# lucagem29/mcmc_clv_model

Measured on AMD Instinct MI355X. Metric: MCMC sweeps/sec x N_customers (customer-sweeps/s), higher is better.
Workload: dtype f64

## Files before the change

### include/clvmcmc.h

```cpp
#ifndef CLVMCMC_H
#define CLVMCMC_H

#include <stdint.h>

#ifdef __cplusplus
extern "C" {
#endif

#define CLV_ABI_VERSION 2

#define CLV_BLOCK 256
#define CLV_MAX_K 9
#define CLV_MAX_D 3

enum { CLV_OK = 0, CLV_EINVAL = -1, CLV_EHIP = -2, CLV_ESTATE = -3, CLV_ENOMEM = -4 };
enum { CLV_RNG_PHILOX = 0, CLV_RNG_REPLAY = 1 };
enum { CLV_SINK_FULL = 0, CLV_SINK_SUMMARY = 1, CLV_SINK_NONE = 2, CLV_SINK_SUMMARY_PCT = 3 };

#define CLV_SUMMARY_MU_CAP 0.05
enum {
  CLV_SUM_LAMBDA = 0, CLV_SUM_MU, CLV_SUM_Z, CLV_SUM_LOG_LAMBDA, CLV_SUM_LOG_MU,
  CLV_SUM_LAMBDA2, CLV_SUM_MU2, CLV_SUM_ETA, CLV_SUM_LOG_ETA, CLV_SUM_MU_CAPPED, CLV_SUM_TAU,
  CLV_N_SUM_STATS
};

typedef struct clv_config {
  int32_t abi_version;
  int32_t D;
  int32_t K;
  int32_t n_mh_steps;
  int32_t burnin, mcmc, thin;
  int32_t n_chains;
  int32_t chain_first;
  int32_t rng_mode;
  int32_t draw_sink;
  int32_t device;
  uint64_t seed;
  int64_t n_global;
  int64_t shard_begin;
  int32_t world_size;
  int32_t rank;
  int32_t blocks_per_rank;
  int32_t blocks_per_unit;
  uint64_t stream;
} clv_config;

typedef struct clv_data {
  int64_t n;
  const int32_t* x;
  const double* t_x;
  const double* T_cal;
  const double* covariates;
  const double* log_s;
} clv_data;

typedef struct clv_prior {
  double lam_init;
  double V[CLV_MAX_K * CLV_MAX_K];
  double chol_V[CLV_MAX_K * CLV_MAX_K];
  double A0B0[CLV_MAX_K * CLV_MAX_D];
  double S0_B0A0B0[CLV_MAX_D * CLV_MAX_D];
  double nu_n;
  double beta_init[CLV_MAX_K * CLV_MAX_D];
  double sigma_init[CLV_MAX_D * CLV_MAX_D];
  double omega2;
} clv_prior;

typedef struct clv_sampler clv_sampler;

int32_t clv_abi_version(void);
int32_t clv_default_blocks_per_unit(int64_t n_global);
int64_t clv_sizeof(int32_t which);
const char* clv_last_error(void);
int clv_device_count(int32_t* count);

int clv_create(const clv_config* cfg, const clv_data* data, const clv_prior* prior,
               clv_sampler** out);
void clv_destroy(clv_sampler* s);

int clv_set_replay_tape(clv_sampler* s, const double* tape, int64_t n_sweeps);
int64_t clv_replay_sweep_stride(const clv_sampler* s);

int clv_run(clv_sampler* s, int64_t n_sweeps);
int clv_rollback(clv_sampler* s);

int clv_sweep(clv_sampler* s);
int clv_hyper(clv_sampler* s, const double* gathered_device_ptr);
int clv_partials(clv_sampler* s, double** device_ptr, int64_t* n_doubles, int32_t* stride);
int clv_copy_partials(clv_sampler* s, void* dst_device_ptr);
int clv_synchronize(clv_sampler* s);
int64_t clv_sweeps_done(const clv_sampler* s);

int clv_clock_ghz(clv_sampler* s, double* ghz);
int clv_clock_probe(clv_sampler* s, double us, double* ghz);
int clv_launch_info(const clv_sampler* s, int64_t* out);
#define CLV_IPC_HANDLE_BYTES 64
int clv_p2p_info(const clv_sampler* s, int64_t* out);
int clv_p2p_export(clv_sampler* s, void* handle);
int clv_p2p_connect(clv_sampler* s, const void* handles, const uint64_t* ptrs);
int clv_p2p_disconnect(clv_sampler* s);
int clv_p2p_set_persistent(clv_sampler* s, int32_t on);
int clv_set_wait_timeout(clv_sampler* s, double ms);
int clv_set_stream(clv_sampler* s, uint64_t stream);
int clv_note_sweeps(clv_sampler* s, int64_t n);

int clv_read_draws(clv_sampler* s, double* level1, double* level2, double* loglik);
int clv_stream_draws(clv_sampler* s, double* level1);
int clv_read_summary(clv_sampler* s, double* sums, int64_t* n_stored);

int clv_get_state(clv_sampler* s, double* lambdas, double* mus, double* hyper);
int clv_set_state(clv_sampler* s, const double* lambdas, const double* mus, const double* hyper,
                  int64_t sweeps_done);

int clv_set_timing(clv_sampler* s, int32_t enable);
int clv_kernel_time(clv_sampler* s, double* sweep_kernel_ms_total, int64_t* sweep_launches,
                    double* hyper_kernel_ms_total, int64_t* hyper_launches);

int clv_debug_host_times(const clv_sampler* s, int64_t* out);
int clv_debug_philox(uint32_t k0, uint32_t k1, const uint32_t* ctr, int64_t n, uint32_t* out);
int clv_debug_variates(uint64_t seed, int32_t chain, uint32_t sweep, int64_t n, int32_t n_steps,
                       float* t_l, float* t_m, float* u_acc, double* u_z, double* u_tau,
                       double* e_alive, double* eta_z, float* log2_u_acc);
int clv_debug_log2u_scan(uint64_t w_begin, uint64_t w_end, double* out);
int clv_debug_t3(const uint32_t* words, int64_t n, int32_t packed, float* t_l, float* t_m);
int clv_debug_level2(int32_t D, int32_t K, const clv_prior* prior, const double* xty,
                     const double* yty, const double* iw_normal, const double* iw_chi2,
                     const double* z, double* beta, double* sigma);
int clv_debug_stamps(clv_sampler* s, uint64_t* out);
int clv_debug_wg_stamps(clv_sampler* s, uint64_t* out);
int clv_debug_hyper_variates(uint64_t seed, int32_t chain, uint32_t sweep, double df, int64_t n,
                             double* chi2, double* normals);
int clv_debug_exp(const double* x, int64_t n, double* out);
int clv_debug_log(const double* x, int64_t n, double* out);
int clv_debug_mh_step(int64_t n, const int32_t* x, const uint8_t* z, const double* T_cal, const double* tau,
                      const double* mean, const double* prec3, const double* cur_pt, const float* t3,
                      const double* scale2, const float* log_u, double* out);
int clv_debug_wg_map(int32_t n_chains, int32_t nb, int32_t n_cu, int32_t* out);
int clv_debug_persist_fits(int64_t grid_wgs, int32_t blocks_per_cu, int32_t n_cu);
int clv_debug_persist_choice(int32_t D, int32_t K, int32_t n_chains, int64_t grid_wgs, int32_t blocks_per_cu,
                             int32_t n_cu);

enum { CLV_EXCHANGE_AUTO = 0, CLV_EXCHANGE_P2P = 1, CLV_EXCHANGE_COPY = 2 };
typedef struct clv_group clv_group;
int clv_group_create(clv_sampler* const* shards, int32_t n, int32_t exchange, clv_group** out);
int clv_group_run(clv_group* g, int64_t n_sweeps);
int32_t clv_group_exchange(const clv_group* g);
void clv_group_destroy(clv_group* g);

enum {
  CLV_L1_MEAN_LAMBDA = 0, CLV_L1_LAMBDA_P025, CLV_L1_LAMBDA_P975, CLV_L1_MEAN_MU, CLV_L1_MEAN_MU_CAPPED,
  CLV_L1_MU_P025, CLV_L1_MU_P975, CLV_L1_MEAN_Z, CLV_L1_MEAN_TAU, CLV_L1_MEAN_ETA, CLV_N_L1_STATS
};
int clv_predict(int32_t device, const double* level1, int64_t n_draws, int64_t n, int32_t width,
                const double* T_cal, double T_star, uint64_t seed, int32_t simulate_spend, double sigma_s,
                int64_t* x_future, double* spend_future);
int clv_predict_sampler(clv_sampler* s, double T_star, uint64_t seed, int32_t simulate_spend,
                        double sigma_s, int64_t* x_future, double* spend_future);
int clv_track(int32_t device, const double* level1, int64_t n_draws, int64_t n, int32_t width,
              const double* birth_week, const double* times, int32_t n_times, uint64_t seed,
              double* inc_weekly);
int clv_track_sampler(clv_sampler* s, const double* birth_week, const double* times, int32_t n_times,
                      uint64_t seed, double* inc_weekly);
int clv_level1_summary(int32_t device, const double* level1, int64_t n_draws, int64_t n, int32_t width,
                       double mu_cap, double* out);
int clv_level1_summary_sampler(clv_sampler* s, double mu_cap, double* out);
int clv_chain_total_loglik(int32_t device, const double* level1, int64_t n_draws, int64_t n, int32_t width,
                           const int32_t* x, const double* T_cal, double* mean_total);
int clv_chain_total_loglik_sampler(clv_sampler* s, double* mean_total);

enum {
  CLV_LTV_VALUE_MEAN = 0, CLV_LTV_VALUE_SD, CLV_LTV_VALUE_P025, CLV_LTV_VALUE_P50, CLV_LTV_VALUE_P975,
  CLV_LTV_RESIDUAL_MEAN, CLV_LTV_RESIDUAL_SD, CLV_LTV_RESIDUAL_P025, CLV_LTV_RESIDUAL_P50, CLV_LTV_RESIDUAL_P975,
  CLV_LTV_P_ALIVE, CLV_LTV_LIFETIME_YRS, CLV_LTV_SURVIVAL_1YR, CLV_N_LTV_STATS
};
enum {
  CLV_LTV_DRAW_EQUITY = 0, CLV_LTV_DRAW_VALUE_TOTAL, CLV_LTV_DRAW_N_ALIVE, CLV_LTV_DRAW_MU_SHARE,
  CLV_N_LTV_DRAW_STATS
};
int clv_lifetime_value(int32_t device, const double* level1, int64_t n_draws, int64_t n, int32_t width,
                       const double* monetary , double delta, double horizon ,
                       double value_scale, double periods_per_year, double* out_customers, double* out_draws);
int clv_lifetime_value_sampler(clv_sampler* s, const double* monetary, double delta, double horizon,
                               double value_scale, double periods_per_year, double* out_customers,
                               double* out_draws);
int clv_ltv_info(int64_t* out);

enum {
  CLV_DIAG_MEAN = 0, CLV_DIAG_SD, CLV_DIAG_MCSE, CLV_DIAG_ESS, CLV_DIAG_RHAT, CLV_DIAG_LAG, CLV_N_DIAG_STATS
};
int clv_diagnostics(int32_t device, const double* series, int32_t n_chains, int64_t n_draws, int64_t n_series,
                    int32_t period, uint32_t log_mask, double* out);
int clv_diagnostics_sampler(clv_sampler* s, uint32_t log_mask, double* level1_out, double* level2_out);
int clv_autocorr(int32_t device, const double* series, int32_t n_chains, int64_t n_draws, int64_t n_series,
                 int32_t max_lag, double* out);

#define CLV_RANK_LDS_ELEMS 4080
enum {
  CLV_RANK_RHAT = 0, CLV_RANK_RHAT_BULK, CLV_RANK_RHAT_FOLDED, CLV_RANK_ESS_BULK, CLV_RANK_ESS_TAIL,
  CLV_RANK_ESS_Q05, CLV_RANK_ESS_Q95, CLV_RANK_ESS_SD, CLV_RANK_MCSE_SD, CLV_RANK_HDI_LO, CLV_RANK_HDI_HI,
  CLV_RANK_MEDIAN, CLV_RANK_LAG_BULK, CLV_N_RANK_STATS
};
int clv_rank_diagnostics(int32_t device, const double* series, int32_t n_chains, int64_t n_draws, int64_t n_series,
                         int32_t period, uint32_t log_mask, double hdi_prob, double* out);
int clv_rank_diagnostics_sampler(clv_sampler* s, uint32_t log_mask, double hdi_prob, double* level1_out,
                                 double* level2_out);
int clv_debug_zscale(int32_t device, const double* series, int32_t n_chains, int64_t n_draws, int64_t n_series,
                     int32_t folded, double* ranks_out, double* z_out);

int clv_elog2cbs(int32_t device, int64_t n_events, const int64_t* cust, const int64_t* date_ns, const double* sales,
                 int64_t unit_ns, int64_t T_cal_ns, int64_t T_tot_ns, int64_t* n_customers, int64_t* cust_out,
                 int64_t* x, double* t_x, double* litt, double* sales_out, double* sales_x, int64_t* first_ns,
                 double* T_cal, double* T_star, int64_t* x_star, double* sales_star);
int clv_generate_pareto_abe(int32_t device, int64_t n, int32_t K, const double* beta, const double* gamma,
                            const double* covars, const double* T_cal, int32_t n_star, const double* T_star,
                            uint64_t seed, int64_t* x, double* t_x, double* lambda_true, double* mu_true,
                            double* tau_true, uint8_t* alive_true, int64_t* x_star, double* covars_out,
                            int64_t* n_events, const int64_t* elog_offsets, int64_t elog_rows, int64_t* elog_cust,
                            double* elog_t);

typedef struct clv_pnbd clv_pnbd;
int clv_pnbd_create(int32_t device, int64_t n, const int32_t* x, const double* t_x, const double* T,
                    const double* weights, clv_pnbd** out);
void clv_pnbd_destroy(clv_pnbd* h);
int clv_pnbd_eval(clv_pnbd* h, const double* params, double* sums, int64_t* n_unconverged);
int clv_pnbd_customers(clv_pnbd* h, const double* params, double t_star, double* out);
int clv_pnbd_track(int32_t device, int64_t n, const double* birth_week, const double* times, int32_t n_times,
                   const double* params, double* cum);

#ifdef __cplusplus
}
#endif
#endif
```

### mcmc_clv_model_amd/csrc/capi.hip

```cpp
#include <hip/hip_runtime.h>

#include <algorithm>
#include <chrono>
#include <cstdlib>
#include <cstdio>
#include <cstring>
#include <string>
#include <vector>

#include "internal.h"
#include "kernels.h"
#include "philox.h"

using namespace clv;

namespace {

thread_local std::string g_err;

constexpr int PRIOR_DOUBLES = 81 + 81 + 27 + 9;
constexpr int GRAPH_CHUNK = 64;
constexpr int TIMING_EVENTS = 256;

}
// ... 135 lines not shown
    s->ev.resize(4 * TIMING_EVENTS);
    for (auto& e : s->ev) CLV_HIP(hipEventCreate(&e));
  }
  return CLV_OK;
}

int build_graph(clv_sampler* s, int n) {
  if (s->graph_exec && s->graph_sweeps == n) return CLV_OK;
  if (s->graph_exec) {
    CLV_HIP(hipGraphExecDestroy(s->graph_exec));
    s->graph_exec = nullptr;
  }
  hipGraph_t graph;
  CLV_HIP(hipStreamBeginCapture(s->stream, hipStreamCaptureModeThreadLocal));
  for (int k = 0; k < n; ++k) {
    int rc = enqueue_fused(s, nullptr, nullptr);
    if (rc != CLV_OK) {
      hipGraph_t dummy;
      (void)hipStreamEndCapture(s->stream, &dummy);
      return rc;
    }
  }
  CLV_HIP(hipStreamEndCapture(s->stream, &graph));
  CLV_HIP(hipGraphInstantiate(&s->graph_exec, graph, nullptr, nullptr, 0));
  CLV_HIP(hipGraphDestroy(graph));
  s->graph_sweeps = n;
  return CLV_OK;
}

bool is_pow2(int v) { return v > 0 && (v & (v - 1)) == 0; }

int64_t stored_count(const clv_sampler* s, int64_t sweeps) {
  const Geometry& g = s->g;
  if (sweeps <= g.burnin || g.n_draws <= 0) return 0;
  return std::min<int64_t>((sweeps - 1 - g.burnin) / g.thin + 1, g.n_draws);
}

void stream_enqueue(clv_sampler* s) {
  if (!s->ds_dest || !s->d_level1) return;
  const Geometry& g = s->g;
  const int64_t k = stored_count(s, s->sweeps_done);
  if (k <= s->ds_next) return;
  const int64_t row = g.n * (g.D + 2);
  for (int c = 0; c < g.n_chains; ++c) {
    const int64_t off = ((int64_t)c * g.n_draws + s->ds_next) * row;
    stream_copy(s->ds, s->device, s->d_level1 + off, s->ds_dest + off, sizeof(double) * (size_t)((k - s->ds_next) * row));
  }
  s->ds_next = k;
}

void stream_rewind(clv_sampler* s) {
  if (!s->ds_dest) return;
  stream_wait(s->ds);
  s->ds_next = std::min(s->ds_next, stored_count(s, s->sweeps_done));
}

std::string take_wait_diag(clv_sampler* s) {
  if (!s->d_diag) return "";
  unsigned long long d[DIAG_WORDS] = {};
  if (hipMemcpy(d, s->d_diag, sizeof(d), hipMemcpyDeviceToHost) != hipSuccess) return "";
  (void)hipMemset(s->d_diag, 0, sizeof(d));
  if (!d[0]) return "";
  const Geometry& g = s->g;
  const char* what = d[1] == WAIT_HYPER ? "(beta, Sigma) hand-off slot"
                     : d[1] == WAIT_BLOCKS ? "block partial"
                     : d[1] == WAIT_P2P_MAIL ? "peer unit partial (persistent)" : "peer unit partial (fused)";
  std::string m = std::string(" [wait record: sweep ") + std::to_string((long long)d[2]) + ", chain " +
                  std::to_string(d[3]) + ", rank " + std::to_string(d[4]) + ": " + what + " ";
  const long long unit = (long long)d[5];
  if ((d[1] == WAIT_P2P_MAIL || d[1] == WAIT_FX_MAIL) && g.units_per_rank > 0 && unit >= 0)
    m += "unit " + std::to_string(unit) + " (rank " + std::to_string(unit / g.units_per_rank) + ", local unit " +
         std::to_string(unit % g.units_per_rank) + ")";
  else
    m += (d[1] == WAIT_HYPER ? "of block " : "") + std::to_string(unit);
  char bits[32];
  std::snprintf(bits, sizeof(bits), "%016llx", d[7]);
  m += " statistic " + std::to_string((long long)d[6]) + " still empty (bits " + bits + ") after " +
       std::to_string(d[8]) + " polls, " + std::to_string(d[9] / 100000.0) + " ms; " + std::to_string(d[10]) +
       " lanes of the wave missing";
  if (d[1] == WAIT_P2P_MAIL || d[1] == WAIT_FX_MAIL) {
    m += "; progress (sweep each rank's level-2 side last polled for):";
    for (int q = 0; q < std::min(g.world_size, 5); ++q)
      m += " " + std::to_string(q) + ":" + (d[11 + q] == ~0ull ? std::string("none") : std::to_string((long long)d[11 + q]));
  }
  return m + "]";
}

bool parse_wait_ms(const char* txt, double* ms) {
  for (const char* c = txt; *c; ++c)
    if (*c == 'x' || *c == 'X' || *c == 'n' || *c == 'N' || *c == 'i' || *c == 'I') return false;
  char* end = nullptr;
  const double v = std::strtod(txt, &end);
  if (end == txt) return false;
  while (*end == ' ' || *end == '\t' || *end == '\n') ++end;
  if (*end || !(v == v) || v > 1e300 || v < -1e300) return false;
  *ms = std::min(3.6e6, std::max(1.0, v));
  return true;
}

}

extern "C" {

int32_t clv_abi_version(void) { return CLV_ABI_VERSION; }

int32_t clv_default_blocks_per_unit(int64_t n_global) {
  const int64_t nb = (n_global + BLOCK - 1) / BLOCK;
  int32_t g = 1;
  while ((nb + g - 1) / g > 512) g *= 2;
  return g;
}

const char* clv_last_error(void) { return g_err.c_str(); }

int64_t clv_sizeof(int32_t which) {
  switch (which) {
    case 0: return (int64_t)sizeof(clv_config);
    case 1: return (int64_t)sizeof(clv_data);
    case 2: return (int64_t)sizeof(clv_prior);
    default: return -1;
  }
}

int clv_device_count(int32_t* count) {
  int n = 0;
  CLV_HIP(hipGetDeviceCount(&n));
  *count = n;
  return CLV_OK;
}

int64_t clv_replay_sweep_stride(const clv_sampler* s) {
  const int64_t n = s->g.n;
  return n * (2 + 3 * (int64_t)s->g.S + (s->g.D == 3 ? 1 : 0)) + TAPE_HYPER;
}

}

bool clv::persist_grid_fits(int64_t grid_wgs, int blocks_per_cu, int n_cu) {
  constexpr int SGPR_MAX = 102;
  const int sgpr_term = 800 / (((SGPR_MAX + 15) / 16) * 16 + 16);
  const int64_t per_cu = std::min({blocks_per_cu, 8, sgpr_term});
  const int64_t slots = per_cu * n_cu;
  const int64_t margin = std::max(1, n_cu / 32);
  return grid_wgs > 0 && slots > 0 && grid_wgs <= slots - margin;
}

constexpr size_t PERSIST_SCRATCH_MAX = 64;

bool clv::persist_worth(int D, int K, int n_chains, int64_t grid_wgs, int n_cu) {
  (void)D, (void)K, (void)n_chains;
  return n_cu > 0 && grid_wgs > 0;
}

namespace {

#ifndef CLV_L2_ALONE_MIN_NB
#define CLV_L2_ALONE_MIN_NB 256
#endif
std::vector<int32_t> persist_wg_map(int C, int nb, int n_cu) {
  const int per = nb + 1;
  const int T = C * per;
  std::vector<int32_t> map(T);
  for (int c = 0; c < C; ++c)
    for (int b = 0; b < per; ++b) map[c * per + b] = (c << 16) | b;
  const int P = T - n_cu;
  if (P <= 0 || T > 2 * n_cu) return map;
  std::vector<std::vector<int>> todo(C);
  for (int c = 0; c < C; ++c)
    for (int b = nb - 1; b >= 0; --b) todo[c].push_back(b);
  std::vector<int32_t> first, second, single;
  int p = 0;
  const bool l2_alone = nb >= CLV_L2_ALONE_MIN_NB;
  for (int c = 0; !l2_alone && c < C && p < P; ++c, ++p) {
    first.push_back((c << 16) | nb);
    if (todo[c].empty()) return map;
    second.push_back((c << 16) | todo[c].back());
    todo[c].pop_back();
  }
  const int n_l2_paired = (int)first.size();
  const bool l2_paired = n_l2_paired == C;
  for (int c = 0; p < P; c = (c + 1) % C) {
    bool any = false;
    for (int k = 0; k < C && !any; ++k) any = todo[(c + k) % C].size() >= 2;
    if (!any) return map;
    if (todo[c].size() < 2) continue;
    first.push_back((c << 16) | todo[c].back());
    todo[c].pop_back();
    second.push_back((c << 16) | todo[c].back());
    todo[c].pop_back();
    ++p;
  }
  for (int c = 0; c < C; ++c) {
    if (!l2_paired && c >= n_l2_paired) single.push_back((c << 16) | nb);
    while (!todo[c].empty()) {
      single.push_back((c << 16) | todo[c].back());
      todo[c].pop_back();
    }
  }
  std::vector<int32_t> sorted_single;
  for (size_t k = 0; sorted_single.size() < single.size(); ++k)
    for (int c = 0; c < C; ++c) {
      size_t seen = 0;
      for (int32_t v : single)
        if ((v >> 16) == c && seen++ == k) sorted_single.push_back(v);
    }
  if ((int)first.size() != P || (int)sorted_single.size() != n_cu - P) return map;
  for (int i = 0; i < P; ++i) {
    map[i] = first[i];
    map[n_cu + i] = second[i];
  }
  for (int i = 0; i < n_cu - P; ++i) map[P + i] = sorted_single[i];
  return map;
}

}

extern "C" {

int clv_create(const clv_config* cfg, const clv_data* data, const clv_prior* prior, clv_sampler** out) {
  if (!cfg || !data || !prior || !out) return fail(CLV_EINVAL, "null argument");
  *out = nullptr;
  if (cfg->abi_version != CLV_ABI_VERSION) return fail(CLV_EINVAL, "ABI version mismatch");
  if (cfg->D != 2 && cfg->D != 3) return fail(CLV_EINVAL, "D must be 2 or 3");
  if (cfg->K < 1 || cfg->K > CLV_MAX_K) return fail(CLV_EINVAL, "K must be in 1..9");
  if (cfg->n_mh_steps < 0) return fail(CLV_EINVAL, "n_mh_steps must be >= 0");
  if (cfg->thin < 1) return fail(CLV_EINVAL, "thin must be >= 1");
  if (cfg->burnin < 0 || cfg->mcmc < 0) return fail(CLV_EINVAL, "burnin/mcmc must be >= 0");
  if (cfg->n_chains < 1) return fail(CLV_EINVAL, "n_chains must be >= 1");
  if (cfg->rng_mode != CLV_RNG_PHILOX && cfg->rng_mode != CLV_RNG_REPLAY) return fail(CLV_EINVAL, "bad rng_mode");
  if (cfg->draw_sink < CLV_SINK_FULL || cfg->draw_sink > CLV_SINK_SUMMARY_PCT) return fail(CLV_EINVAL, "bad draw_sink");
  if (data->n < 0) return fail(CLV_EINVAL, "n must be >= 0");
  if (cfg->n_global > 0xffffffffLL) return fail(CLV_EINVAL, "n_global must fit the 32-bit Philox customer counter");
  if (cfg->n_global < data->n || cfg->n_global < 1) return fail(CLV_EINVAL, "n_global must be >= n >= 0 and > 0");
  if (cfg->world_size < 1 || cfg->rank < 0 || cfg->rank >= cfg->world_size) return fail(CLV_EINVAL, "bad rank/world_size");
  if (cfg->D == 3 && data->n > 0 && !data->log_s) return fail(CLV_EINVAL, "D == 3 needs log_s");
  if (cfg->K > 1 && data->n > 0 && !data->covariates) return fail(CLV_EINVAL, "K > 1 needs covariates");
  if (data->n > 0 && (!data->x || !data->t_x || !data->T_cal)) return fail(CLV_EINVAL, "missing CBS column");
  if (cfg->rng_mode == CLV_RNG_REPLAY && cfg->world_size != 1) return fail(CLV_EINVAL, "replay needs world_size 1");

  const int32_t bpu = cfg->blocks_per_unit ? cfg->blocks_per_unit : clv_default_blocks_per_unit(cfg->n_global);
  if (!is_pow2(bpu)) return fail(CLV_EINVAL, "blocks_per_unit must be a power of two");
  const int nb_local = (int)((data->n + BLOCK - 1) / BLOCK);
  int32_t bpr = cfg->blocks_per_rank;
  if (bpr == 0) {
    if (cfg->world_size != 1) return fail(CLV_EINVAL, "blocks_per_rank required when sharded");
    bpr = ((std::max(nb_local, 1) + bpu - 1) / bpu) * bpu;
  }
  if (bpr % bpu) return fail(CLV_EINVAL, "blocks_per_rank must be a multiple of blocks_per_unit");
  if (nb_local > bpr) return fail(CLV_EINVAL, "shard larger than blocks_per_rank * CLV_BLOCK");
  if (cfg->shard_begin != (int64_t)cfg->rank * bpr * BLOCK) return fail(CLV_EINVAL, "shard_begin != rank * blocks_per_rank * CLV_BLOCK");
  const int64_t nb_global = (cfg->n_global + BLOCK - 1) / BLOCK;
  if ((int64_t)bpr * cfg->world_size < nb_global) return fail(CLV_EINVAL, "shards do not cover n_global");

  auto* s = new clv_sampler();
  s->cfg = *cfg;
  s->cfg.blocks_per_rank = bpr;
  s->cfg.blocks_per_unit = bpu;
  s->prior = *prior;
  s->replay = cfg->rng_mode == CLV_RNG_REPLAY;

  Geometry& g = s->g;
  g.D = cfg->D;
  g.K = cfg->K;
  g.S = cfg->n_mh_steps;
  g.n_chains = cfg->n_chains;
  g.n = data->n;
  g.n_global = cfg->n_global;
  g.shard_begin = cfg->shard_begin;
  g.nb_local = nb_local;
  g.blocks_per_rank = bpr;
  g.blocks_per_unit = bpu;
  g.units_per_rank = bpr / bpu;
  g.n_units_global = (nb_global + bpu - 1) / bpu;
  g.world_size = cfg->world_size;
  g.stride = cfg->K * cfg->D + cfg->D * (cfg->D + 1) / 2 + 1;
  g.burnin = cfg->burnin;
  g.mcmc = cfg->mcmc;
  g.thin = cfg->thin;
  g.n_draws = cfg->mcmc >= 1 ? (cfg->mcmc - 1) / cfg->thin + 1 : 0;
  g.l2w = cfg->D * cfg->K + cfg->D * (cfg->D + 1) / 2;

  auto cleanup_fail = [&](int rc) {
    clv_destroy(s);
    return rc;
  };
#define CLV_HIPC(expr)                                                                            \
  do {                                                                                            \
    hipError_t e_ = (expr);                                                                       \
    if (e_ != hipSuccess)                                                                         \
      return cleanup_fail(fail(CLV_EHIP, std::string(#expr) + ": " + hipGetErrorString(e_)));    \
  } while (0)

  if (cfg->device >= 0) CLV_HIPC(hipSetDevice(cfg->device));
  CLV_HIPC(hipGetDevice(&s->device));
  if (cfg->stream) {
    s->stream = (hipStream_t)(uintptr_t)cfg->stream;
  } else {
    CLV_HIPC(hipStreamCreateWithFlags(&s->stream, hipStreamNonBlocking));
    s->own = s->stream;
    s->own_stream = true;
  }

  const int64_t n = g.n, C = g.n_chains;
  CLV_HIPC(dalloc(&s->d_x, std::max<int64_t>(n, 1)));
  CLV_HIPC(dalloc(&s->d_tx, std::max<int64_t>(n, 1)));
  CLV_HIPC(dalloc(&s->d_T, std::max<int64_t>(n, 1)));
  if (g.K > 1) CLV_HIPC(dalloc(&s->d_cov, (size_t)(g.K - 1) * std::max<int64_t>(n, 1)));
  if (g.D == 3) CLV_HIPC(dalloc(&s->d_logs, std::max<int64_t>(n, 1)));
  CLV_HIPC(dalloc(&s->d_clk, 2 * CLK_RING));
  CLV_HIPC(hipMemsetAsync(s->d_clk, 0, sizeof(unsigned long long) * 2 * CLK_RING, s->stream));
  CLV_HIPC(dalloc(&s->d_lam, C * std::max<int64_t>(n, 1)));
  CLV_HIPC(dalloc(&s->d_mu, C * std::max<int64_t>(n, 1)));
  CLV_HIPC(dalloc(&s->d_hyper, C * HS));
  CLV_HIPC(dalloc(&s->d_block, (size_t)C * bpr * g.stride));
  if (bpu > 1) CLV_HIPC(dalloc(&s->d_unit, (size_t)C * g.units_per_rank * g.stride));
  else s->d_unit = s->d_block;
  CLV_HIPC(dalloc(&s->d_prior, PRIOR_DOUBLES));
  CLV_HIPC(dalloc(&s->d_ctrl, 1));
  CLV_HIPC(dalloc(&s->d_arrive, C + C * (int64_t)g.units_per_rank));
  CLV_HIPC(dalloc(&s->d_hvar, 2 * C * HV));
  CLV_HIPC(dalloc(&s->d_hyp2, 2 * C * HS));
  if (!s->replay && cfg->world_size == 1 && nb_local > 0 && bpu == 1 && nb_local <= 2 * BLOCK) {
    const char* env = std::getenv("CLV_PERSISTENT");
    hipDeviceProp_t prop{};
    size_t scratch = SIZE_MAX;
    if (persist_occupancy(g.D, g.K, false, &s->persist_bpc) == hipSuccess &&
        persist_scratch_bytes(g.D, g.K, false, &scratch) == hipSuccess &&
        hipGetDeviceProperties(&prop, s->device) == hipSuccess)
      s->n_cu = prop.multiProcessorCount;
    const int64_t grid = (int64_t)(nb_local + 1) * C;
    const bool force = env && std::string(env) == "1";
    if ((!env || std::string(env) != "0") && (force || scratch <= PERSIST_SCRATCH_MAX) && persist_grid_fits(grid, s->persist_bpc, s->n_cu) &&
        (force || persist_worth(g.D, g.K, (int)C, grid, s->n_cu)))
      s->persistent = true;
  }
  if (!s->replay && cfg->world_size > 1 && cfg->world_size <= MAX_WORLD && nb_local > 0 && nb_local <= 2 * BLOCK && g.n_units_global <= 2 * BLOCK &&
      bpu <= 64 && (int64_t)g.stride * ((nb_local + bpu - 1) / bpu) <= UMAIL) {
    hipDeviceProp_t prop{};
    size_t scratch = SIZE_MAX;
    if (persist_occupancy(g.D, g.K, true, &s->persist_bpc) == hipSuccess &&
        persist_scratch_bytes(g.D, g.K, true, &scratch) == hipSuccess &&
        hipGetDeviceProperties(&prop, s->device) == hipSuccess)
      s->n_cu = prop.multiProcessorCount;
    const char* env = std::getenv("CLV_PERSISTENT");
    const int64_t grid = (int64_t)(nb_local + 1) * C;
    const bool force = env && std::string(env) == "1";
    if ((!env || std::string(env) != "0") && (force || scratch <= PERSIST_SCRATCH_MAX) && persist_grid_fits(grid, s->persist_bpc, s->n_cu) &&
        (force || persist_worth(g.D, g.K, (int)C, grid, s->n_cu)))
      s->p2p_capable = s->p2p_persist_fits = true;
  }
  if (!s->replay && cfg->world_size > 1 && cfg->world_size <= MAX_WORLD && g.n_units_global <= 2 * BLOCK)
    s->fx_capable = true;
  if (s->p2p_capable || s->fx_capable) {
    const int64_t nm = mail_slots(g.world_size, (int)C, g.stride, g.units_per_rank) + MAIL_TAIL;
    {
      const char* env = std::getenv("CLV_MAIL_ALLOC");
      const std::string want = env ? env : "uncached";
      const unsigned flags[3] = {hipDeviceMallocUncached, hipDeviceMallocFinegrained, hipDeviceMallocDefault};
      const int first = want == "fine" ? 1 : want == "default" ? 2 : 0;
      for (int k = first; k < 3 && !s->d_mail; ++k) {
        void* p = nullptr;
        if (hipExtMallocWithFlags(&p, sizeof(double) * (size_t)nm, flags[k]) == hipSuccess && p) {
          s->d_mail = (double*)p;
          s->mail_kind = k;
        } else {
          (void)hipGetLastError();
        }
      }
      if (!s->d_mail) return cleanup_fail(fail(CLV_ENOMEM, "peer mail buffer"));
    }
    CLV_HIPC(hipMemsetAsync(s->d_mail, 0xFF, sizeof(double) * nm, s->stream));
    CLV_HIPC(dalloc(&s->d_peers, g.world_size));
  }
  if (s->persistent || s->p2p_capable || s->fx_capable) {
    CLV_HIPC(dalloc(&s->d_pblock, (size_t)C * std::max(nb_local, 1) * g.stride));
    if (s->persistent) {
      const char* env = std::getenv("CLV_DEFER");
      s->defer = !(env && std::string(env) == "0");
      if (s->defer) CLV_HIPC(dalloc(&s->d_pend, (size_t)2 * C * g.stride));
    }
    CLV_HIPC(dalloc(&s->d_lam_alt, C * std::max<int64_t>(n, 1)));
    CLV_HIPC(dalloc(&s->d_mu_alt, C * std::max<int64_t>(n, 1)));
    CLV_HIPC(dalloc(&s->d_hyper_alt, C * HS));
    if ((cfg->draw_sink == CLV_SINK_SUMMARY || cfg->draw_sink == CLV_SINK_SUMMARY_PCT) && n > 0)
      CLV_HIPC(dalloc(&s->d_sums_prev, (size_t)C * CLV_N_SUM_STATS * n));
    CLV_HIPC(dalloc(&s->d_diag, DIAG_WORDS));
    CLV_HIPC(hipMemsetAsync(s->d_diag, 0, sizeof(unsigned long long) * DIAG_WORDS, s->stream));
    CLV_HIPC(hipHostMalloc((void**)&s->h_abort, sizeof(uint32_t), hipHostMallocMapped));
    *s->h_abort = 0;
    CLV_HIPC(hipHostGetDevicePointer((void**)&s->d_h_abort, s->h_abort, 0));
    double ms = cfg->world_size > 1 ? 10000.0 : 2000.0;
    if (const char* env = std::getenv("CLV_WAIT_TIMEOUT_MS")) {
      if (!parse_wait_ms(env, &ms))
        return cleanup_fail(fail(CLV_EINVAL, "CLV_WAIT_TIMEOUT_MS must be a finite decimal number of ms"));
    }
    s->wait_ticks = (uint64_t)(ms * 1e5);
  }
  if ((s->persistent || s->p2p_capable) && s->n_cu > 0) {
    {
      std::vector<int32_t> map = persist_wg_map((int)C, (int)nb_local, s->n_cu);
      CLV_HIPC(dalloc(&s->d_wgmap, map.size()));
      CLV_HIPC(hipMemcpy(s->d_wgmap, map.data(), sizeof(int32_t) * map.size(), hipMemcpyHostToDevice));
    }
  }
#ifdef CLV_STAMPS
  {
    std::vector<unsigned long long> st(1024 * 8 + 12 * (size_t)C * (std::max(nb_local, 1) + 1), 0ull);
    for (int i = 0; i < 1024; ++i) st[i * 8 + 0] = st[i * 8 + 4] = ~0ull;
    CLV_HIPC(dalloc(&s->d_stamps, st.size()));
    CLV_HIPC(hipMemcpy(s->d_stamps, st.data(), st.size() * sizeof(unsigned long long), hipMemcpyHostToDevice));
  }
#endif
  CLV_HIPC(hipMemsetAsync(s->d_hvar, 0, sizeof(double) * 2 * C * HV, s->stream));
  CLV_HIPC(hipMemsetAsync(s->d_arrive, 0, sizeof(uint32_t) * (C + C * (int64_t)g.units_per_rank), s->stream));
  CLV_HIPC(dalloc(&s->d_bs, C * (CLV_MAX_K * CLV_MAX_D + CLV_MAX_D * CLV_MAX_D)));
  if (g.n_draws > 0) {
    CLV_HIPC(dalloc(&s->d_level2, (size_t)C * g.n_draws * g.l2w));
    CLV_HIPC(dalloc(&s->d_loglik, (size_t)C * g.n_draws));
    CLV_HIPC(hipMemsetAsync(s->d_level2, 0, sizeof(double) * C * g.n_draws * g.l2w, s->stream));
    CLV_HIPC(hipMemsetAsync(s->d_loglik, 0, sizeof(double) * C * g.n_draws, s->stream));
    if (cfg->draw_sink == CLV_SINK_FULL && n > 0) {
      const size_t bytes = sizeof(double) * (size_t)C * g.n_draws * n * (g.D + 2);
      CLV_HIPC(dalloc(&s->d_level1, bytes / sizeof(double)));
      CLV_HIPC(hipMemsetAsync(s->d_level1, 0, bytes, s->stream));
    }
  }
  if ((cfg->draw_sink == CLV_SINK_SUMMARY || cfg->draw_sink == CLV_SINK_SUMMARY_PCT) && n > 0) {
    CLV_HIPC(dalloc(&s->d_sums, (size_t)C * CLV_N_SUM_STATS * n));
    CLV_HIPC(hipMemsetAsync(s->d_sums, 0, sizeof(double) * C * CLV_N_SUM_STATS * n, s->stream));
  }
  if (cfg->draw_sink == CLV_SINK_SUMMARY_PCT && n > 0 && g.n_draws > 0) {
    const size_t nq = (size_t)C * g.n_draws * n;
    if (hipMalloc((void**)&s->d_qstore, sizeof(float2) * nq) != hipSuccess) {
      (void)hipGetLastError();
      s->d_qstore = nullptr;
      return cleanup_fail(fail(CLV_ENOMEM, "percentile store: " + std::to_string(sizeof(float2) * nq) +
                                               " bytes of device memory not available"));
    }
    CLV_HIPC(hipMemsetAsync(s->d_qstore, 0, sizeof(float2) * nq, s->stream));
  }
  CLV_HIPC(hipMemsetAsync(s->d_block, 0, sizeof(double) * C * bpr * g.stride, s->stream));
  if (bpu > 1) CLV_HIPC(hipMemsetAsync(s->d_unit, 0, sizeof(double) * C * g.units_per_rank * g.stride, s->stream));
  CLV_HIPC(hipMemsetAsync(s->d_ctrl, 0, sizeof(Ctrl), s->stream));
  CLV_HIPC(hipMemsetAsync(s->d_hyper, 0, sizeof(double) * C * HS, s->stream));

  if (n > 0) {
    CLV_HIPC(hipMemcpyAsync(s->d_x, data->x, sizeof(int32_t) * n, hipMemcpyHostToDevice, s->stream));
    CLV_HIPC(hipMemcpyAsync(s->d_tx, data->t_x, sizeof(double) * n, hipMemcpyHostToDevice, s->stream));
    CLV_HIPC(hipMemcpyAsync(s->d_T, data->T_cal, sizeof(double) * n, hipMemcpyHostToDevice, s->stream));
    if (g.K > 1)
      CLV_HIPC(hipMemcpyAsync(s->d_cov, data->covariates, sizeof(double) * (g.K - 1) * n, hipMemcpyHostToDevice, s->stream));
    if (g.D == 3)
      CLV_HIPC(hipMemcpyAsync(s->d_logs, data->log_s, sizeof(double) * n, hipMemcpyHostToDevice, s->stream));
  }
  {
    std::vector<double> pr(PRIOR_DOUBLES, 0.0);
    const int K = g.K, D = g.D;
    for (int i = 0; i < K * K; ++i) {
      pr[i] = prior->V[i];
      pr[81 + i] = prior->chol_V[i];
    }
    for (int i = 0; i < K * D; ++i) pr[162 + i] = prior->A0B0[i];
    for (int i = 0; i < D * D; ++i) pr[189 + i] = prior->S0_B0A0B0[i];
    CLV_HIPC(hipMemcpyAsync(s->d_prior, pr.data(), sizeof(double) * PRIOR_DOUBLES, hipMemcpyHostToDevice, s->stream));
    CLV_HIPC(hipStreamSynchronize(s->stream));
  }

  if (n > 0) CLV_HIPC(launch_sweep(sweep_args(s, 1), false, s->stream));
  else CLV_HIPC(hipMemsetAsync(s->d_block, 0, sizeof(double) * C * bpr * g.stride, s->stream));
  if (bpu > 1) {
    GroupArgs ga{};
    ga.g = g;
    ga.blockpart = s->d_block;
    ga.unitpart = s->d_unit;
    if (n > 0) CLV_HIPC(launch_group(ga, s->stream));
  }
  if (g.D == 3) {
    std::vector<double> bs(C * (g.K * g.D + g.D * g.D));
    for (int c = 0; c < C; ++c) {
      double* o = bs.data() + c * (g.K * g.D + g.D * g.D);
      for (int i = 0; i < g.K * g.D; ++i) o[i] = prior->beta_init[i];
      for (int i = 0; i < g.D * g.D; ++i) o[g.K * g.D + i] = prior->sigma_init[i];
    }
    CLV_HIPC(hipMemcpyAsync(s->d_bs, bs.data(), sizeof(double) * bs.size(), hipMemcpyHostToDevice, s->stream));
    CLV_HIPC(launch_set_hyper(g.D, g.K, (int)C, s->d_hyper, s->d_bs, prior->omega2, s->replay, s->stream));
  } else {
    s->pending_init_hyper = true;
  }
  CLV_HIPC(hipStreamSynchronize(s->stream));
#undef CLV_HIPC
  *out = s;
  return CLV_OK;
}

void clv_destroy(clv_sampler* s) {
  if (!s) return;
  (void)hipSetDevice(s->device);
  if (s->stream) (void)hipStreamSynchronize(s->stream);
  if (s->ds) {
    stream_wait(s->ds);
    delete s->ds;
  }
  if (s->graph_exec) (void)hipGraphExecDestroy(s->graph_exec);
  for (auto e : s->ev) (void)hipEventDestroy(e);
  if (s->done_ev) (void)hipEventDestroy(s->done_ev);
  void* ptrs[] = {s->d_x, s->d_tx, s->d_T, s->d_cov, s->d_logs, s->d_lam, s->d_mu, s->d_hyper,
                  s->d_block, s->d_prior, s->d_ctrl, s->d_level1, s->d_level2, s->d_loglik,
                  s->d_sums, s->d_tape, s->d_bs, s->d_arrive, s->d_hvar, s->d_stamps};
  for (void* p : ptrs)
    if (p) (void)hipFree(p);
  if (s->d_unit && s->d_unit != s->d_block) (void)hipFree(s->d_unit);
  if (s->d_hyp2) (void)hipFree(s->d_hyp2);
  for (void* p : {(void*)s->d_lam_alt, (void*)s->d_mu_alt, (void*)s->d_hyper_alt, (void*)s->d_sums_prev,
                  (void*)s->d_pblock, (void*)s->d_qstore, (void*)s->d_pend, (void*)s->d_diag,
                  (void*)s->d_clk})
    if (p) (void)hipFree(p);
  if (s->h_abort) (void)hipHostFree(s->h_abort);
  for (void* p : s->ipc_opened) (void)hipIpcCloseMemHandle(p);
  if (s->d_mail) (void)hipFree(s->d_mail);
  if (s->d_peers) (void)hipFree(s->d_peers);
  if (s->d_wgmap) (void)hipFree(s->d_wgmap);
  if (s->own_stream && s->own) (void)hipStreamDestroy(s->own);
  delete s;
}

int clv_set_replay_tape(clv_sampler* s, const double* tape, int64_t n_sweeps) {
  if (!s || !tape || n_sweeps < 1) return fail(CLV_EINVAL, "bad replay tape arguments");
  if (!s->replay) return fail(CLV_ESTATE, "sampler not created in replay mode");
  CLV_HIP(hipSetDevice(s->device));
  if (s->d_tape) CLV_HIP(hipFree(s->d_tape));
  s->d_tape = nullptr;
  const size_t count = (size_t)s->g.n_chains * n_sweeps * clv_replay_sweep_stride(s);
  CLV_HIP(dalloc(&s->d_tape, count));
  CLV_HIP(hipMemcpy(s->d_tape, tape, count * sizeof(double), hipMemcpyHostToDevice));
  s->tape_sweeps = n_sweeps;
  if (s->graph_exec) {
    CLV_HIP(hipGraphExecDestroy(s->graph_exec));
    s->graph_exec = nullptr;
  }
  return CLV_OK;
}

int clv_hyper(clv_sampler* s, const double* gathered) {
  if (!s) return fail(CLV_EINVAL, "null sampler");
  if (s->g.world_size > 1 && !gathered) return fail(CLV_EINVAL, "sharded hyper needs the gathered buffer");
  CLV_HIP(hipSetDevice(s->device));
  {
    int rc = persist_flush(s);
    if (rc) return rc;
  }
  if (s->pending_init_hyper) {
    int rc = check_replay_range(s, 0);
    if (rc) return rc;
    rc = enqueue_hyper(s, gathered, 1, nullptr, nullptr);
    if (rc) return rc;
    s->pending_init_hyper = false;
    return CLV_OK;
  }
  return enqueue_hyper(s, gathered, 0, nullptr, nullptr);
}

int clv_sweep(clv_sampler* s) {
  if (!s) return fail(CLV_EINVAL, "null sampler");
  if (s->pending_init_hyper) return fail(CLV_ESTATE, "bivariate: call clv_hyper once before the first sweep");
  CLV_HIP(hipSetDevice(s->device));
  int rc = persist_flush(s);
  if (rc) return rc;
  rc = check_replay_range(s, 1);
  if (rc) return rc;
  hipEvent_t e0 = nullptr, e1 = nullptr;
  if (s->timing) {
    rc = ensure_events(s);
    if (rc) return rc;
    e0 = s->ev[4 * s->ev_used];
    e1 = s->ev[4 * s->ev_used + 1];
  }
  rc = enqueue_sweep(s, e0, e1);
  if (rc) return rc;
  if (s->timing && ++s->ev_used == TIMING_EVENTS) {
    rc = harvest_timing(s);
    if (rc) return rc;
  }
  s->sweeps_done++;
  return CLV_OK;
}

int clv_partials(clv_sampler* s, double** ptr, int64_t* n_doubles, int32_t* stride) {
  if (!s) return fail(CLV_EINVAL, "null sampler");
  if (ptr) *ptr = s->d_unit;
  if (n_doubles) *n_doubles = (int64_t)s->g.n_chains * s->g.units_per_rank * s->g.stride;
  if (stride) *stride = s->g.stride;
  return CLV_OK;
}

int clv_copy_partials(clv_sampler* s, void* dst) {
  if (!s || !dst) return fail(CLV_EINVAL, "null argument");
  CLV_HIP(hipSetDevice(s->device));
  const size_t bytes = sizeof(double) * (size_t)s->g.n_chains * s->g.units_per_rank * s->g.stride;
  CLV_HIP(hipMemcpyAsync(dst, s->d_unit, bytes, hipMemcpyDeviceToDevice, s->stream));
  return CLV_OK;
}

int clv_synchronize(clv_sampler* s) {
  if (!s) return fail(CLV_EINVAL, "null sampler");
  CLV_HIP(hipSetDevice(s->device));
  CLV_HIP(hipStreamSynchronize(s->stream));
  return CLV_OK;
}

int64_t clv_sweeps_done(const clv_sampler* s) { return s ? s->sweeps_done : -1; }

int clv_clock_ghz(clv_sampler* s, double* ghz) {
  if (!s || !ghz) return fail(CLV_EINVAL, "null argument");
  *ghz = 0.0;
  const int64_t end = s->sweeps_done - 1;
  const int64_t first = std::max<int64_t>(s->clk_first, end - (CLK_RING - 1));
  if (!s->d_clk || s->clk_first < 1 || end < first) return CLV_OK;
  CLV_HIP(hipSetDevice(s->device));
  CLV_HIP(hipStreamSynchronize(s->stream));
  std::vector<unsigned long long> ring(2 * CLK_RING);
  CLV_HIP(hipMemcpy(ring.data(), s->d_clk, sizeof(unsigned long long) * ring.size(), hipMemcpyDeviceToHost));
  double dm = 0.0, dr = 0.0;
  for (int64_t q = first; q <= end; ++q) {
    dm += (double)ring[2 * (q % CLK_RING)];
    dr += (double)ring[2 * (q % CLK_RING) + 1];
  }
  if (dr > 0.0) *ghz = 0.1 * dm / dr;
  return CLV_OK;
}

int clv_launch_info(const clv_sampler* s, int64_t* out) {
  if (!s || !out) return fail(CLV_EINVAL, "null argument");
  out[0] = s->persistent ? 1 : 0;
  out[1] = s->persist_bpc;
  out[2] = s->n_cu;
  out[3] = (int64_t)(s->g.nb_local + (s->persistent ? 1 : 0)) * s->g.n_chains;
  out[4] = 0;
  out[5] = 0;
  return CLV_OK;
}

int clv_p2p_info(const clv_sampler* s, int64_t* out) {
  if (!s || !out) return fail(CLV_EINVAL, "null argument");
  out[0] = (s->p2p_capable || s->fx_capable) ? 1 : 0;
  out[4] = s->p2p_capable ? 1 : 0;
  out[1] = s->p2p_ready ? 1 : 0;
  out[2] = s->d_mail ? (int64_t)sizeof(double) * 2 * s->g.world_size * s->g.n_chains * s->g.stride * s->g.units_per_rank : 0;
  out[3] = (int64_t)(uintptr_t)s->d_mail;
  out[5] = s->d_mail ? s->mail_kind : -1;
  return CLV_OK;
}

int clv_p2p_export(clv_sampler* s, void* handle) {
  if (!s || !handle) return fail(CLV_EINVAL, "null argument");
  if (!s->p2p_capable && !s->fx_capable) return fail(CLV_ESTATE, "no peer exchange for this sampler (world size 1 or replay mode)");
  CLV_HIP(hipSetDevice(s->device));
  hipIpcMemHandle_t h;
  CLV_HIP(hipIpcGetMemHandle(&h, s->d_mail));
  std::memcpy(handle, &h, sizeof(h));
  return CLV_OK;
}

int clv_p2p_connect(clv_sampler* s, const void* handles, const uint64_t* ptrs) {
  if (!s || (!handles && !ptrs)) return fail(CLV_EINVAL, "null argument");
  if (!s->p2p_capable && !s->fx_capable) return fail(CLV_ESTATE, "no peer exchange for this sampler (world size 1 or replay mode)");
  CLV_HIP(hipSetDevice(s->device));
  CLV_HIP(hipStreamSynchronize(s->stream));
  if (s->p2p_ready || !s->ipc_opened.empty()) {
    s->p2p_ready = false;
    for (void* p : s->ipc_opened) (void)hipIpcCloseMemHandle(p);
    s->ipc_opened.clear();
  }
  {
    const int64_t nm = mail_slots(s->g.world_size, s->g.n_chains, s->g.stride, s->g.units_per_rank) + MAIL_TAIL;
    CLV_HIP(hipMemsetAsync(s->d_mail, 0xFF, sizeof(double) * nm, s->stream));
  }
  const int W = s->g.world_size, r = s->cfg.rank;
  std::vector<double*> peers(W, nullptr);
  for (int q = 0; q < W; ++q) {
    if (q == r) {
      peers[q] = s->d_mail;
    } else if (handles) {
      hipIpcMemHandle_t h;
      std::memcpy(&h, (const char*)handles + (size_t)q * sizeof(h), sizeof(h));
      void* p = nullptr;
      CLV_HIP(hipIpcOpenMemHandle(&p, h, hipIpcMemLazyEnablePeerAccess));
      s->ipc_opened.push_back(p);
      peers[q] = (double*)p;
    } else {
      peers[q] = (double*)(uintptr_t)ptrs[q];
    }
    if (!peers[q]) return fail(CLV_EINVAL, "null peer mail pointer");
  }
  CLV_HIP(hipMemcpy(s->d_peers, peers.data(), sizeof(double*) * W, hipMemcpyHostToDevice));
  CLV_HIP(hipStreamSynchronize(s->stream));
  s->p2p_ready = true;
  return CLV_OK;
}

int clv_p2p_set_persistent(clv_sampler* s, int32_t on) {
  if (!s) return fail(CLV_EINVAL, "null sampler");
  if (on && !s->p2p_persist_fits) return fail(CLV_ESTATE, "the persistent peer exchange does not fit this shard's grid");
  if (!on && !s->fx_capable) return fail(CLV_ESTATE, "no fused peer exchange for this sampler");
  CLV_HIP(hipSetDevice(s->device));
  CLV_HIP(hipStreamSynchronize(s->stream));
  s->p2p_capable = on != 0;
  s->last_persist_n = 0;
  return CLV_OK;
}

int clv_p2p_disconnect(clv_sampler* s) {
  if (!s) return fail(CLV_EINVAL, "null sampler");
  CLV_HIP(hipSetDevice(s->device));
  CLV_HIP(hipStreamSynchronize(s->stream));
  s->p2p_ready = false;
  for (void* p : s->ipc_opened) (void)hipIpcCloseMemHandle(p);
  s->ipc_opened.clear();
  if (s->d_peers) CLV_HIP(hipMemset(s->d_peers, 0, sizeof(double*) * s->g.world_size));
  return CLV_OK;
}

int clv_set_wait_timeout(clv_sampler* s, double ms) {
  if (!s || !(ms >= 1.0) || ms > 3.6e6) return fail(CLV_EINVAL, "wait timeout must be in [1 ms, 1 h]");
  s->wait_ticks = (uint64_t)(ms * 1e5);
  if (s->graph_exec) {
    CLV_HIP(hipGraphExecDestroy(s->graph_exec));
    s->graph_exec = nullptr;
  }
  return CLV_OK;
}

int clv_set_stream(clv_sampler* s, uint64_t stream) {
  if (!s || !stream) return fail(CLV_EINVAL, "bad arguments");
  if (s->graph_exec) {
    CLV_HIP(hipGraphExecDestroy(s->graph_exec));
    s->graph_exec = nullptr;
  }
  s->stream = (hipStream_t)(uintptr_t)stream;
  return CLV_OK;
}

int clv_note_sweeps(clv_sampler* s, int64_t n) {
  if (!s || s->sweeps_done + n < 0) return fail(CLV_EINVAL, "bad arguments");
  s->sweeps_done += n;
  s->last_persist_n = 0;
  return CLV_OK;
}

}

static inline int64_t host_now_ns() {
  return std::chrono::duration_cast<std::chrono::nanoseconds>(std::chrono::steady_clock::now().time_since_epoch())
      .count();
}

int clv::persist_launch(clv_sampler* s, int64_t n_sweeps) {
  const Geometry& g = s->g;
  s->last_persist_n = 0;
  s->inflight_n = 0;
  if (n_sweeps == 0) return CLV_OK;
  if (s->slots_dirty) {
    CLV_HIP(hipMemsetAsync(s->d_hyp2, 0xFF, sizeof(double) * 2 * g.n_chains * HS, s->stream));
    CLV_HIP(hipMemsetAsync(s->d_pblock, 0xFF, sizeof(double) * g.n_chains * g.nb_local * g.stride, s->stream));
    s->slots_dirty = false;
  }
  const size_t sums_bytes = sizeof(double) * (size_t)g.n_chains * CLV_N_SUM_STATS * g.n;
  if (s->d_sums_prev)
    CLV_HIP(hipMemcpyAsync(s->d_sums_prev, s->d_sums, sums_bytes, hipMemcpyDeviceToDevice, s->stream));
  SweepArgs a = sweep_args(s, 0, 1);
  const int64_t stride_c = (int64_t)g.n_chains * g.stride;
  a.pend_in = s->pend ? s->d_pend + s->pend_buf * stride_c : nullptr;
  a.pend_out = s->defer ? s->d_pend + (s->pend_buf ^ 1) * stride_c : nullptr;
  hipEvent_t e0 = nullptr, e1 = nullptr;
  if (s->timing) {
    int rc = ensure_events(s);
    if (rc) return rc;
    e0 = s->ev[4 * s->ev_used];
    e1 = s->ev[4 * s->ev_used + 1];
    if (s->ev_sweeps.size() < TIMING_EVENTS) s->ev_sweeps.assign(TIMING_EVENTS, 1);
    s->ev_sweeps[s->ev_used] = n_sweeps;
  }
  if (e0) CLV_HIP(hipEventRecord(e0, s->stream));
  s->host_ns[2] = host_now_ns();
  CLV_HIP(launch_persist(a, s->sweeps_done + 1, n_sweeps, s->stream, nullptr, nullptr));
  s->host_ns[3] = host_now_ns();
  if (e1) CLV_HIP(hipEventRecord(e1, s->stream));
  s->inflight_done = e1;
  if (s->timing) {
    if (++s->ev_used == TIMING_EVENTS) {
      int rc = harvest_timing(s);
      if (rc) return rc;
    }
  } else {
    if (!s->done_ev) CLV_HIP(hipEventCreateWithFlags(&s->done_ev, hipEventDisableTiming));
    CLV_HIP(hipEventRecord(s->done_ev, s->stream));
    s->inflight_done = s->done_ev;
  }
  s->inflight_n = n_sweeps;
  s->host_ns[4] = host_now_ns();
  return CLV_OK;
}

int clv::persist_wait(clv_sampler* s) {
  const int64_t n_sweeps = s->inflight_n;
  if (n_sweeps == 0) return CLV_OK;
  s->inflight_n = 0;
  const Geometry& g = s->g;
  const hipEvent_t done = s->inflight_done;
  if (!done) {
    CLV_HIP(hipStreamSynchronize(s->stream));
  } else {
    hipError_t q;
    while ((q = hipEventQuery(done)) == hipErrorNotReady) {
    }
    CLV_HIP(q);
  }
  s->host_ns[5] = host_now_ns();
  if (__atomic_load_n(s->h_abort, __ATOMIC_ACQUIRE)) {
    *s->h_abort = 0;
    Ctrl c{};
    c.cur = s->sweeps_done;
    CLV_HIP(hipMemcpy(s->d_ctrl, &c, sizeof(Ctrl), hipMemcpyHostToDevice));
    const size_t sums_bytes = sizeof(double) * (size_t)g.n_chains * CLV_N_SUM_STATS * g.n;
    if (s->d_sums_prev) CLV_HIP(hipMemcpy(s->d_sums, s->d_sums_prev, sums_bytes, hipMemcpyDeviceToDevice));
    s->slots_dirty = true;
    if (g.world_size > 1) s->p2p_ready = false;
    const std::string diag = take_wait_diag(s);
    return fail(CLV_EHIP, std::string(g.world_size > 1
                                          ? "persistent sweep kernel: a wait timed out (a peer rank not running, or not all "
                                            "resident?); state unchanged"
                                          : "persistent sweep kernel: a workgroup timed out waiting for its chain (not all "
                                            "resident?); state unchanged") + diag);
  }
  std::swap(s->d_lam, s->d_lam_alt);
  std::swap(s->d_mu, s->d_mu_alt);
  s->rb_pend = s->pend;
  s->rb_pend_buf = s->pend_buf;
  s->rb_hyper_swaps = 0;
  if (s->defer) {
    s->pend = true;
    s->pend_buf ^= 1;
  } else {
    std::swap(s->d_hyper, s->d_hyper_alt);
    s->rb_hyper_swaps = 1;
    s->pend = false;
  }
  if (s->graph_exec) {
    CLV_HIP(hipGraphExecDestroy(s->graph_exec));
    s->graph_exec = nullptr;
  }
  s->sweeps_done += n_sweeps;
  s->last_persist_n = n_sweeps;
  return CLV_OK;
}

int clv::persist_flush(clv_sampler* s) {
  if (!s->pend) return CLV_OK;
  CLV_HIP(hipSetDevice(s->device));
  SweepArgs a = sweep_args(s, 0, 1);
  a.pend_in = s->d_pend + s->pend_buf * (int64_t)s->g.n_chains * s->g.stride;
  a.pend_out = nullptr;
  CLV_HIP(launch_persist_flush(a, s->sweeps_done + 1, s->stream));
  CLV_HIP(hipStreamSynchronize(s->stream));
  std::swap(s->d_hyper, s->d_hyper_alt);
  s->rb_hyper_swaps++;
  s->pend = false;
  if (s->graph_exec) {
    CLV_HIP(hipGraphExecDestroy(s->graph_exec));
    s->graph_exec = nullptr;
  }
  return CLV_OK;
}

namespace {
int run_persistent(clv_sampler* s, int64_t n_sweeps) {
  int rc = persist_launch(s, n_sweeps);
  if (rc) return rc;
  return persist_wait(s);
}

int enqueue_fused_sweeps(clv_sampler* s, int64_t n_sweeps) {
  int rc = CLV_OK;
  int64_t left = n_sweeps;
  if (s->timing) {
    rc = ensure_events(s);
    if (rc) return rc;
    while (left > 0) {
      const int k = s->ev_used;
      rc = enqueue_fused(s, s->ev[4 * k], s->ev[4 * k + 1]);
      if (rc) return rc;
      s->ev_used++;
      s->sweeps_done++;
      left--;
      if (s->ev_used == TIMING_EVENTS) {
        rc = harvest_timing(s);
        if (rc) return rc;
      }
    }
    return harvest_timing(s);
  }
  if (left >= GRAPH_CHUNK) {
    rc = build_graph(s, GRAPH_CHUNK);
    if (rc) return rc;
    while (left >= GRAPH_CHUNK) {
      CLV_HIP(hipGraphLaunch(s->graph_exec, s->stream));
      s->sweeps_done += GRAPH_CHUNK;
      left -= GRAPH_CHUNK;
    }
  }
  while (left > 0) {
    rc = enqueue_fused(s, nullptr, nullptr);
    if (rc) return rc;
    s->sweeps_done++;
    left--;
  }
  return CLV_OK;
}

int run_fused_exchange(clv_sampler* s, int64_t n_sweeps) {
  s->last_persist_n = 0;
  if (n_sweeps == 0) return CLV_OK;
  const Geometry& g = s->g;
  const size_t nl = sizeof(double) * (size_t)g.n_chains * std::max<int64_t>(g.n, 1);
  const size_t sums_bytes = sizeof(double) * (size_t)g.n_chains * CLV_N_SUM_STATS * g.n;
  CLV_HIP(hipMemcpyAsync(s->d_lam_alt, s->d_lam, nl, hipMemcpyDeviceToDevice, s->stream));
  CLV_HIP(hipMemcpyAsync(s->d_mu_alt, s->d_mu, nl, hipMemcpyDeviceToDevice, s->stream));
  CLV_HIP(hipMemcpyAsync(s->d_hyper_alt, s->d_hyper, sizeof(double) * g.n_chains * HS, hipMemcpyDeviceToDevice,
                         s->stream));
  if (s->d_sums_prev) CLV_HIP(hipMemcpyAsync(s->d_sums_prev, s->d_sums, sums_bytes, hipMemcpyDeviceToDevice, s->stream));
  const int64_t before = s->sweeps_done;
  const int rc = enqueue_fused_sweeps(s, n_sweeps);
  CLV_HIP(hipStreamSynchronize(s->stream));
  const bool aborted = __atomic_load_n(s->h_abort, __ATOMIC_ACQUIRE) != 0;
  if (rc == CLV_OK && !aborted) {
    s->last_persist_n = n_sweeps;
    s->rb_pend = false;
    s->rb_hyper_swaps = 1;
    return CLV_OK;
  }
  CLV_HIP(hipMemcpy(s->d_lam, s->d_lam_alt, nl, hipMemcpyDeviceToDevice));
  CLV_HIP(hipMemcpy(s->d_mu, s->d_mu_alt, nl, hipMemcpyDeviceToDevice));
  CLV_HIP(hipMemcpy(s->d_hyper, s->d_hyper_alt, sizeof(double) * g.n_chains * HS, hipMemcpyDeviceToDevice));
  if (s->d_sums_prev) CLV_HIP(hipMemcpy(s->d_sums, s->d_sums_prev, sums_bytes, hipMemcpyDeviceToDevice));
  *s->h_abort = 0;
  s->sweeps_done = before;
  Ctrl c{};
  c.cur = before;
  CLV_HIP(hipMemcpy(s->d_ctrl, &c, sizeof(Ctrl), hipMemcpyHostToDevice));
  CLV_HIP(hipMemset(s->d_arrive, 0, sizeof(uint32_t) * (g.n_chains + (int64_t)g.n_chains * g.units_per_rank)));
  s->p2p_ready = false;
  if (rc) return rc;
  return fail(CLV_EHIP, "fused peer exchange: a wait timed out (a peer rank not running?); state unchanged" +
                            take_wait_diag(s));
}

int run_streaming(clv_sampler* s, int64_t n_sweeps) {
  const Geometry& g = s->g;
  const int64_t per_draw = (int64_t)g.n_chains * g.n * (g.D + 2) * (int64_t)sizeof(double);
  const int64_t chunk = std::max<int64_t>(256, std::max<int64_t>(1, (64LL << 20) / std::max<int64_t>(per_draw, 1)) * g.thin);
  int64_t left = n_sweeps;
  while (left > 0) {
    const int64_t k = s->sweeps_done < g.burnin ? std::min<int64_t>(left, g.burnin - s->sweeps_done)
                                                : std::min<int64_t>(left, chunk);
    int rc;
    if (s->persistent) {
      rc = run_persistent(s, k);
    } else {
      rc = enqueue_fused_sweeps(s, k);
      if (rc == CLV_OK && hipStreamSynchronize(s->stream) != hipSuccess) rc = fail(CLV_EHIP, "hipStreamSynchronize");
    }
    if (rc) return rc;
    stream_enqueue(s);
    left -= k;
  }
  return CLV_OK;
}
}

extern "C" {

// ... 224 lines not shown

int clv_debug_wg_stamps(clv_sampler* s, uint64_t* out) {
  if (!s || !out) return fail(CLV_EINVAL, "null argument");
  if (!s->d_stamps) return fail(CLV_ESTATE, "library not built with CLV_STAMPS (make STAMPS=1)");
  CLV_HIP(hipStreamSynchronize(s->stream));
  CLV_HIP(hipMemcpy(out, s->d_stamps + 1024 * 8, sizeof(uint64_t) * 12 * s->g.n_chains * (s->g.nb_local + 1),
                    hipMemcpyDeviceToHost));
  return CLV_OK;
}

int clv_debug_host_times(const clv_sampler* s, int64_t* out) {
  if (!s || !out) return fail(CLV_EINVAL, "bad arguments");
  for (int k = 0; k < 8; ++k) out[k] = s->host_ns[k];
  return CLV_OK;
}

int clv_debug_philox(uint32_t k0, uint32_t k1, const uint32_t* ctr, int64_t n, uint32_t* out) {
  if (!ctr || !out || n < 0) return fail(CLV_EINVAL, "bad arguments");
  uint32_t *dc = nullptr, *dout = nullptr;
  CLV_HIP(dalloc(&dc, 4 * std::max<int64_t>(n, 1)));
  CLV_HIP(dalloc(&dout, 4 * std::max<int64_t>(n, 1)));
  CLV_HIP(hipMemcpy(dc, ctr, 16 * n, hipMemcpyHostToDevice));
  CLV_HIP(launch_debug_philox(k0, k1, dc, n, dout, nullptr));
  CLV_HIP(hipMemcpy(out, dout, 16 * n, hipMemcpyDeviceToHost));
  CLV_HIP(hipFree(dc));
  CLV_HIP(hipFree(dout));
  return CLV_OK;
}

int clv_debug_variates(uint64_t seed, int32_t chain, uint32_t sweep, int64_t n, int32_t S, float* tl, float* tm,
                       float* ua, double* uz, double* ut, double* ea, double* ez, float* l2u) {
  if (n < 1 || S < 0) return fail(CLV_EINVAL, "bad arguments");
  const int64_t nS = std::max<int64_t>(n * S, 1);
  float *dtl, *dtm, *dua, *dl2u;
  double *duz, *dut, *dea, *dez;
  CLV_HIP(dalloc(&dtl, nS));
  CLV_HIP(dalloc(&dtm, nS));
  CLV_HIP(dalloc(&dua, nS));
  CLV_HIP(dalloc(&dl2u, nS));
  CLV_HIP(dalloc(&duz, n));
  CLV_HIP(dalloc(&dut, n));
  CLV_HIP(dalloc(&dea, n));
  CLV_HIP(dalloc(&dez, n));
  CLV_HIP(launch_debug_variates(seed, chain, sweep, n, S, dtl, dtm, dua, dl2u, duz, dut, dea, dez, nullptr));
  if (S > 0) {
    CLV_HIP(hipMemcpy(tl, dtl, sizeof(float) * n * S, hipMemcpyDeviceToHost));
    CLV_HIP(hipMemcpy(tm, dtm, sizeof(float) * n * S, hipMemcpyDeviceToHost));
    CLV_HIP(hipMemcpy(ua, dua, sizeof(float) * n * S, hipMemcpyDeviceToHost));
    if (l2u) CLV_HIP(hipMemcpy(l2u, dl2u, sizeof(float) * n * S, hipMemcpyDeviceToHost));
  }
  CLV_HIP(hipMemcpy(uz, duz, sizeof(double) * n, hipMemcpyDeviceToHost));
  CLV_HIP(hipMemcpy(ut, dut, sizeof(double) * n, hipMemcpyDeviceToHost));
  CLV_HIP(hipMemcpy(ea, dea, sizeof(double) * n, hipMemcpyDeviceToHost));
  CLV_HIP(hipMemcpy(ez, dez, sizeof(double) * n, hipMemcpyDeviceToHost));
  for (void* p : {(void*)dtl, (void*)dtm, (void*)dua, (void*)dl2u, (void*)duz, (void*)dut, (void*)dea, (void*)dez})
    CLV_HIP(hipFree(p));
  return CLV_OK;
}

int clv_debug_log2u_scan(uint64_t w_begin, uint64_t w_end, double* out) {
  if (!out || w_end > (1ull << 32) || w_begin >= w_end) return fail(CLV_EINVAL, "bad arguments");
  constexpr int NB = 4096;
  double* dres = nullptr;
  CLV_HIP(dalloc(&dres, 4 * NB));
  CLV_HIP(launch_debug_log2u_scan(w_begin, w_end, NB, dres, nullptr));
  std::vector<double> r(4 * NB);
  CLV_HIP(hipMemcpy(r.data(), dres, sizeof(double) * r.size(), hipMemcpyDeviceToHost));
  CLV_HIP(hipFree(dres));
  double mu = 0.0, ma = 0.0, wu = 0.0, mu_far = 0.0;
  for (int b = 0; b < NB; ++b) {
    if (r[4 * b] > mu) {
      mu = r[4 * b];
      wu = r[4 * b + 2];
    }
    ma = std::max(ma, r[4 * b + 1]);
    mu_far = std::max(mu_far, r[4 * b + 3]);
  }
  out[0] = mu;
  out[1] = ma;
  out[2] = wu;
  out[3] = mu_far;
  return CLV_OK;
}

int clv_debug_t3(const uint32_t* words, int64_t n, int32_t packed, float* tl, float* tm) {
  if (!words || !tl || !tm || n < 1 || (packed != 0 && packed != 1)) return fail(CLV_EINVAL, "bad arguments");
  uint32_t* dw = nullptr;
  float *dl = nullptr, *dm = nullptr;
  CLV_HIP(dalloc(&dw, 3 * n));
  CLV_HIP(dalloc(&dl, n));
  CLV_HIP(dalloc(&dm, n));
  CLV_HIP(hipMemcpy(dw, words, 12 * n, hipMemcpyHostToDevice));
  CLV_HIP(launch_debug_t3(dw, n, packed, dl, dm, nullptr));
  CLV_HIP(hipMemcpy(tl, dl, sizeof(float) * n, hipMemcpyDeviceToHost));
  CLV_HIP(hipMemcpy(tm, dm, sizeof(float) * n, hipMemcpyDeviceToHost));
  for (void* p : {(void*)dw, (void*)dl, (void*)dm}) CLV_HIP(hipFree(p));
  return CLV_OK;
}

int clv_debug_level2(int32_t D, int32_t K, const clv_prior* prior, const double* xty, const double* yty,
                     const double* iwn, const double* chi2, const double* z, double* beta, double* sigma) {
  if ((D != 2 && D != 3) || K < 1 || K > CLV_MAX_K || !prior) return fail(CLV_EINVAL, "bad arguments");
  std::vector<double> pr(PRIOR_DOUBLES, 0.0);
  for (int i = 0; i < K * K; ++i) {
    pr[i] = prior->V[i];
    pr[81 + i] = prior->chol_V[i];
  }
  for (int i = 0; i < K * D; ++i) pr[162 + i] = prior->A0B0[i];
  for (int i = 0; i < D * D; ++i) pr[189 + i] = prior->S0_B0A0B0[i];
  std::vector<double> in(K * D + D * D + 6 + D * K, 0.0);
  for (int i = 0; i < K * D; ++i) in[i] = xty[i];
  for (int i = 0; i < D * D; ++i) in[K * D + i] = yty[i];
  for (int i = 0; i < D * (D - 1) / 2; ++i) in[K * D + D * D + i] = iwn[i];
  for (int i = 0; i < D; ++i) in[K * D + D * D + 3 + i] = chi2[i];
  for (int i = 0; i < D * K; ++i) in[K * D + D * D + 6 + i] = z[i];
  double *dpr, *din, *dout;
  CLV_HIP(dalloc(&dpr, pr.size()));
  CLV_HIP(dalloc(&din, in.size()));
  CLV_HIP(dalloc(&dout, K * D + D * D));
  CLV_HIP(hipMemcpy(dpr, pr.data(), sizeof(double) * pr.size(), hipMemcpyHostToDevice));
  CLV_HIP(hipMemcpy(din, in.data(), sizeof(double) * in.size(), hipMemcpyHostToDevice));
  CLV_HIP(launch_debug_level2(D, K, dpr, din, dout, nullptr));
  std::vector<double> o(K * D + D * D);
  CLV_HIP(hipMemcpy(o.data(), dout, sizeof(double) * o.size(), hipMemcpyDeviceToHost));
  for (int i = 0; i < K * D; ++i) beta[i] = o[i];
  for (int i = 0; i < D * D; ++i) sigma[i] = o[K * D + i];
  CLV_HIP(hipFree(dpr));
  CLV_HIP(hipFree(din));
  CLV_HIP(hipFree(dout));
  return CLV_OK;
}

int clv_debug_hyper_variates(uint64_t seed, int32_t chain, uint32_t sweep, double df, int64_t n, double* chi2,
                             double* normals) {
  if (n < 1 || df < 2.0) return fail(CLV_EINVAL, "bad arguments");
  double *dc, *dn;
  CLV_HIP(dalloc(&dc, n));
  CLV_HIP(dalloc(&dn, n));
  CLV_HIP(launch_debug_hyper_variates(seed, chain, sweep, df, n, dc, dn, nullptr));
  CLV_HIP(hipMemcpy(chi2, dc, sizeof(double) * n, hipMemcpyDeviceToHost));
  CLV_HIP(hipMemcpy(normals, dn, sizeof(double) * n, hipMemcpyDeviceToHost));
  CLV_HIP(hipFree(dc));
  CLV_HIP(hipFree(dn));
  return CLV_OK;
}

int clv_debug_persist_choice(int32_t D, int32_t K, int32_t n_chains, int64_t grid_wgs, int32_t blocks_per_cu,
                             int32_t n_cu) {
  return persist_grid_fits(grid_wgs, blocks_per_cu, n_cu) && persist_worth(D, K, n_chains, grid_wgs, n_cu) ? 1 : 0;
}

int clv_debug_persist_fits(int64_t grid_wgs, int32_t blocks_per_cu, int32_t n_cu) {
  return persist_grid_fits(grid_wgs, blocks_per_cu, n_cu) ? 1 : 0;
}

int clv_debug_wg_map(int32_t n_chains, int32_t nb, int32_t n_cu, int32_t* out) {
  if (!out || n_chains < 1 || nb < 0 || n_cu < 1 || n_chains >= (1 << 15) || nb >= (1 << 16))
    return fail(CLV_EINVAL, "bad arguments");
  const std::vector<int32_t> m = persist_wg_map(n_chains, nb, n_cu);
  std::copy(m.begin(), m.end(), out);
  return CLV_OK;
}

int clv_debug_mh_step(int64_t n, const int32_t* x, const uint8_t* z, const double* T_cal, const double* tau,
                      const double* mean, const double* prec3, const double* cur_pt, const float* t3,
                      const double* scale2, const float* log_u, double* out) {
  if (!x || !z || !T_cal || !tau || !mean || !prec3 || !cur_pt || !t3 || !scale2 || !log_u || !out || n < 1)
    return fail(CLV_EINVAL, "bad arguments");
  int32_t *dx;
  uint8_t* dz;
  double *dT, *dtau, *dm, *dp, *dc, *ds, *dout;
  float *dt3, *dlu;
  CLV_HIP(hipMalloc(&dx, sizeof(int32_t) * n));
  CLV_HIP(hipMalloc(&dz, n));
  CLV_HIP(dalloc(&dT, n));
  CLV_HIP(dalloc(&dtau, n));
  CLV_HIP(dalloc(&dm, 2 * n));
  CLV_HIP(dalloc(&dp, 3));
  CLV_HIP(dalloc(&dc, 2 * n));
  CLV_HIP(dalloc(&ds, 2));
  CLV_HIP(dalloc(&dout, 7 * n));
  CLV_HIP(hipMalloc(&dt3, sizeof(float) * 2 * n));
  CLV_HIP(hipMalloc(&dlu, sizeof(float) * n));
  CLV_HIP(hipMemcpy(dx, x, sizeof(int32_t) * n, hipMemcpyHostToDevice));
  CLV_HIP(hipMemcpy(dz, z, n, hipMemcpyHostToDevice));
  CLV_HIP(hipMemcpy(dT, T_cal, sizeof(double) * n, hipMemcpyHostToDevice));
  CLV_HIP(hipMemcpy(dtau, tau, sizeof(double) * n, hipMemcpyHostToDevice));
  CLV_HIP(hipMemcpy(dm, mean, sizeof(double) * 2 * n, hipMemcpyHostToDevice));
  CLV_HIP(hipMemcpy(dp, prec3, sizeof(double) * 3, hipMemcpyHostToDevice));
  CLV_HIP(hipMemcpy(dc, cur_pt, sizeof(double) * 2 * n, hipMemcpyHostToDevice));
  CLV_HIP(hipMemcpy(ds, scale2, sizeof(double) * 2, hipMemcpyHostToDevice));
  CLV_HIP(hipMemcpy(dt3, t3, sizeof(float) * 2 * n, hipMemcpyHostToDevice));
  CLV_HIP(hipMemcpy(dlu, log_u, sizeof(float) * n, hipMemcpyHostToDevice));
  CLV_HIP(launch_debug_mh(dx, dz, dT, dtau, dm, dp, dc, dt3, ds, dlu, n, dout, nullptr));
  CLV_HIP(hipMemcpy(out, dout, sizeof(double) * 7 * n, hipMemcpyDeviceToHost));
  for (void* p : {(void*)dx, (void*)dz, (void*)dT, (void*)dtau, (void*)dm, (void*)dp, (void*)dc, (void*)ds,
                  (void*)dout, (void*)dt3, (void*)dlu})
    CLV_HIP(hipFree(p));
  return CLV_OK;
}

}
static int debug_fast_fn(const double* x, int64_t n, double* out, bool log_fn) {
  if (!x || !out || n < 1) return fail(CLV_EINVAL, "bad arguments");
  double *dx, *dout;
  CLV_HIP(dalloc(&dx, n));
  CLV_HIP(dalloc(&dout, n));
  CLV_HIP(hipMemcpy(dx, x, sizeof(double) * n, hipMemcpyHostToDevice));
  CLV_HIP(launch_debug_exp(dx, n, dout, nullptr, log_fn));
  CLV_HIP(hipMemcpy(out, dout, sizeof(double) * n, hipMemcpyDeviceToHost));
  CLV_HIP(hipFree(dx));
  CLV_HIP(hipFree(dout));
  return CLV_OK;
}
extern "C" {
int clv_debug_exp(const double* x, int64_t n, double* out) { return debug_fast_fn(x, n, out, false); }

int clv_debug_log(const double* x, int64_t n, double* out) { return debug_fast_fn(x, n, out, true); }

}
```

### mcmc_clv_model_amd/csrc/internal.h

```cpp
#pragma once
#include <hip/hip_runtime.h>

#include <atomic>
#include <condition_variable>
#include <mutex>
#include <string>
#include <vector>

#include "kernels.h"

namespace clv {

int fail(int code, const std::string& msg);

int persist_launch(clv_sampler* s, int64_t n_sweeps);
int persist_wait(clv_sampler* s);
int persist_flush(clv_sampler* s);
bool persist_grid_fits(int64_t grid_wgs, int blocks_per_cu, int n_cu);
bool persist_worth(int D, int K, int n_chains, int64_t grid_wgs, int n_cu);

struct DrawStreamState {
  std::mutex m;
  std::condition_variable cv;
  int64_t pending = 0;
  std::atomic<int> failed{0};
};
void stream_prefault(DrawStreamState* st, int device, void* dst, size_t bytes);
void stream_copy(DrawStreamState* st, int device, const void* src, void* dst, size_t bytes);
bool stream_wait(DrawStreamState* st);
void stream_clear_failed(DrawStreamState* st);

int sampler_l1(clv_sampler* s, const double** l1, int64_t* n_draws, int32_t* width);

template <class T>
hipError_t dalloc(T** p, size_t count) {
  *p = nullptr;
  if (count == 0) return hipSuccess;
  return hipMalloc((void**)p, count * sizeof(T));
}

struct DevBuf {
  void* p = nullptr;
  DevBuf() = default;
  DevBuf(const DevBuf&) = delete;
  DevBuf& operator=(const DevBuf&) = delete;
  ~DevBuf() {
    if (p) (void)hipFree(p);
  }
  template <class T>
  T* as() const {
    return (T*)p;
  }
};

struct DeviceScope {
  int prev = -1;
  explicit DeviceScope(int dev) {
    (void)hipGetDevice(&prev);
    if (dev >= 0) (void)hipSetDevice(dev);
  }
  ~DeviceScope() {
    if (prev >= 0) (void)hipSetDevice(prev);
  }
};

}

#define CLV_HIP(expr)                                                                           \
  do {                                                                                          \
    hipError_t e_ = (expr);                                                                     \
    if (e_ != hipSuccess)                                                                       \
      return ::clv::fail(CLV_EHIP, std::string(#expr) + ": " + hipGetErrorString(e_));          \
  } while (0)

struct clv_sampler {
  clv_config cfg{};
  clv_prior prior{};
  clv::Geometry g{};
  bool replay = false;
  int device = 0;
  hipStream_t stream = nullptr;
  hipStream_t own = nullptr;
  bool own_stream = false;

  int32_t* d_x = nullptr;
  double *d_tx = nullptr, *d_T = nullptr, *d_cov = nullptr, *d_logs = nullptr;
  double *d_lam = nullptr, *d_mu = nullptr, *d_hyper = nullptr;
  double *d_block = nullptr, *d_unit = nullptr;
  double* d_prior = nullptr;
  clv::Ctrl* d_ctrl = nullptr;
  uint32_t* d_arrive = nullptr;
  double* d_hyp2 = nullptr;
  double* d_pblock = nullptr;
  double *d_lam_alt = nullptr, *d_mu_alt = nullptr, *d_hyper_alt = nullptr;
  double* d_sums_prev = nullptr;
  uint32_t* h_abort = nullptr;
  uint32_t* d_h_abort = nullptr;
  unsigned long long* d_diag = nullptr;
  unsigned long long* d_clk = nullptr;
  int64_t clk_first = 0;
  uint64_t wait_ticks = 0;
  bool slots_dirty = true;
  int64_t last_persist_n = 0;
  bool defer = false;
  bool pend = false;
  int pend_buf = 0;
  double* d_pend = nullptr;
  bool rb_pend = false;
  int rb_pend_buf = 0;
  int rb_hyper_swaps = 0;
  bool persistent = false;
  int persist_bpc = 0, n_cu = 0;
  bool p2p_capable = false;
  bool p2p_persist_fits = false;
  bool fx_capable = false;
  bool p2p_ready = false;
  double* d_mail = nullptr;
  int mail_kind = -1;
  double** d_peers = nullptr;
  int32_t* d_wgmap = nullptr;
  std::vector<void*> ipc_opened;
  double* d_hvar = nullptr;
  unsigned long long* d_stamps = nullptr;
  double *d_level1 = nullptr, *d_level2 = nullptr, *d_loglik = nullptr, *d_sums = nullptr;
  float2* d_qstore = nullptr;
  double* d_tape = nullptr;
  double* d_bs = nullptr;
  int64_t tape_sweeps = 0;

  bool pending_init_hyper = false;
  int64_t sweeps_done = 0;

  hipGraphExec_t graph_exec = nullptr;
  int graph_sweeps = 0;

  hipEvent_t done_ev = nullptr;
  int64_t inflight_n = 0;
  hipEvent_t inflight_done = nullptr;

  int64_t host_ns[8] = {0, 0, 0, 0, 0, 0, 0, 0};

  clv::DrawStreamState* ds = nullptr;
  double* ds_dest = nullptr;
  int64_t ds_next = 0;

  bool timing = false;
  std::vector<hipEvent_t> ev;
  std::vector<int64_t> ev_sweeps;
  int ev_used = 0;
  double t_sweep_ms = 0.0, t_hyper_ms = 0.0;
  int64_t n_sweep_timed = 0, n_hyper_timed = 0;
};
```

### mcmc_clv_model_amd/csrc/kernels.h

```cpp
#pragma once
#include <hip/hip_runtime.h>
#include <stdint.h>

#include "../../include/clvmcmc.h"

namespace clv {

constexpr int BLOCK = CLV_BLOCK;
constexpr int HS = 64;
constexpr int H_TAG = 63;
constexpr int TAPE_HYPER = 40;
constexpr int MAX_WORLD = 64;
constexpr int UMAIL = 2048;
constexpr int HV = 40;
constexpr int MAIL_TAIL = MAX_WORLD;
constexpr int CLK_RING = 1024;
constexpr int DIAG_WORDS = 16;
enum : int { WAIT_HYPER = 1, WAIT_BLOCKS = 2, WAIT_P2P_MAIL = 3, WAIT_FX_MAIL = 4 };

__host__ __device__ inline int64_t mail_slots(int world, int chains, int stride, int units_per_rank) {
  return 2LL * world * chains * stride * units_per_rank;
}

enum : int {
  H_BETA = 0,
  H_SIGMA = 27,
  H_P00 = 36, H_P01 = 37, H_P11 = 38,
  H_S00 = 39, H_S11 = 40,
  H_S22 = 41, H_POSTVAR = 42, H_SQRT_POSTVAR = 43, H_OMEGA2 = 44,
  H_INV_OMEGA2 = 45, H_INV_S22 = 46,
};

struct Ctrl {
  int64_t cur;
  uint32_t arrive;
  uint32_t abort;
};

struct Geometry {
  int D, K, S;
  int n_chains;
  int64_t n;
  int64_t n_global;
  int64_t shard_begin;
  int nb_local;
  int blocks_per_rank;
  int blocks_per_unit;
  int units_per_rank;
  int64_t n_units_global;
  int world_size;
  int stride;
  int burnin, mcmc, thin, n_draws;
  int l2w;
};

struct Rng {
  uint64_t seed;
  int chain_first;
  const double* tape;
  int64_t tape_sweep_stride;
  int64_t tape_sweeps;
};

struct HyperArgs {
  Geometry g;
  Rng r;
  const double* units;
  double* hyper;
  Ctrl* ctrl;
  double* level2;
  double* loglik;
  const double* V;
  const double* cholV;
  const double* A0B0;
  const double* S0B;
  double nu_n;
  double omega2;
  int mode;
  const double* hvar;
  unsigned long long* stamps;
};

struct SweepArgs {
  Geometry g;
  Rng r;
  const int32_t* x;
  const double* tx;
  const double* T;
  const double* cov;
  const double* log_s;
  double* lam;
  double* mu;
  const double* hyper;
  double* blockpart;
  double* pblock;
  const Ctrl* ctrl;
  Ctrl* ctrl_rw;
  double* hyp2;
  double* level1;
  double* sums;
  float2* qstore;
  int64_t* n_stored;
  double lam_init;
  int init;
  int fuse;
  uint32_t* chain_arrive;
  uint32_t* unit_arrive;
  double* unitpart;
  double* hvar_out;
  double* mail;
  double* const* peers;
  int rank;
  const int32_t* wg_map;
  double* lam_out;
  double* mu_out;
  double* hyper_out;
  const double* pend_in;
  double* pend_out;
  uint64_t wait_ticks;
  uint32_t* abort_host;
  unsigned long long* diag;
  unsigned long long* clk;
  HyperArgs h;
  unsigned long long* stamps;
};

struct GroupArgs {
  Geometry g;
  const double* blockpart;
  double* unitpart;
};


hipError_t launch_sweep(const SweepArgs& a, bool replay, hipStream_t st, hipEvent_t e0 = nullptr,
                        hipEvent_t e1 = nullptr);
hipError_t launch_group(const GroupArgs& a, hipStream_t st);
hipError_t launch_persist(const SweepArgs& a, int64_t s_first, int64_t n_sweeps, hipStream_t st,
                          hipEvent_t e0 = nullptr, hipEvent_t e1 = nullptr);
hipError_t persist_occupancy(int D, int K, bool p2p, int* blocks_per_cu);
hipError_t persist_scratch_bytes(int D, int K, bool p2p, size_t* bytes);
hipError_t launch_persist_flush(const SweepArgs& a, int64_t s_first, hipStream_t st);
hipError_t launch_hyper(const HyperArgs& a, bool replay, hipStream_t st);
hipError_t launch_set_hyper(int D, int K, int n_chains, double* hyper, const double* beta_sigma,
                            double omega2, bool replay, hipStream_t st);
hipError_t launch_debug_philox(uint32_t k0, uint32_t k1, const uint32_t* ctr, int64_t n, uint32_t* out,
                               hipStream_t st);
hipError_t launch_debug_variates(uint64_t seed, int chain, uint32_t sweep, int64_t n, int S, float* tl,
                                 float* tm, float* ua, float* l2u, double* uz, double* ut, double* ea, double* ez,
                                 hipStream_t st);
hipError_t launch_debug_log2u_scan(uint64_t w_begin, uint64_t w_end, int n_blocks, double* out, hipStream_t st);
hipError_t launch_debug_t3(const uint32_t* w, int64_t n, int packed, float* tl, float* tm, hipStream_t st);
hipError_t launch_debug_level2(int D, int K, const double* prior_dev, const double* in, double* out,
                               hipStream_t st);
hipError_t launch_debug_hyper_variates(uint64_t seed, int chain, uint32_t sweep, double df, int64_t n,
                                       double* chi2, double* normals, hipStream_t st);
hipError_t launch_debug_exp(const double* x, int64_t n, double* out, hipStream_t st, bool log_fn = false);
hipError_t launch_debug_mh(const int32_t* x, const uint8_t* z, const double* T, const double* tau, const double* m,
                           const double* prec, const double* cur_pt, const float* t3, const double* scale,
                           const float* log_u, int64_t n, double* out, hipStream_t st);

}
```

### mcmc_clv_model_amd/csrc/kernels.hip

```cpp
#include <hip/hip_ext.h>

#include "fastmath.h"
#include "kernels.h"
#include "philox.h"

#ifndef SWEEP_MH_PIPELINE
#define SWEEP_MH_PIPELINE 1
#endif
#ifndef CLV_OPAQUE_GI
#define CLV_OPAQUE_GI(D) ((D) == 3)
#endif
#ifndef CLV_L2_OPAQUE
#define CLV_L2_OPAQUE(P) (P)
#endif
#ifndef CLV_L2_LANE0_MAX
#define CLV_L2_LANE0_MAX 6
#endif
#ifndef PERSIST_REDUCE_GEN
#define PERSIST_REDUCE_GEN 1
#endif
#ifndef SWEEP_REDUCE_CHUNK
#define SWEEP_REDUCE_CHUNK 8
#endif
template <int D, int K>
struct SweepOcc;

#ifndef SWEEP_COV_LDS_MIN_K
#define SWEEP_COV_LDS_MIN_K 6
#endif
template <int D, int K>
struct CovLds {
  static constexpr bool value = K >= SWEEP_COV_LDS_MIN_K;
};

template <int D, int K>
struct SweepOcc {
#ifdef SWEEP_MIN_BLOCKS
  static constexpr int value = SWEEP_MIN_BLOCKS;
#else
  static constexpr int value = (D == 2 && K != 6) ? 4 : 1;
#endif
};

namespace clv {


__device__ __forceinline__ double clip70(double v) {
  return __builtin_fmin(__builtin_fmax(v, -70.0), 70.0);
}
__device__ __forceinline__ double min700(double v) {
  return v > 700.0 ? 700.0 : v;
}

struct LPConst {
  double xm, omz, w, m0, m1, p00, p01, p11;
};

__device__ __forceinline__ double log_post(const LPConst& c, double ll, double lm) {
  const double dl = ll - c.m0;
  const double dm = lm - c.m1;
  const double lik = (c.xm * ll + c.omz * lm) - (exp(ll) + exp(lm)) * c.w;
  const double prior = -0.5 * ((dl * dl * c.p00 + 2.0 * dl * dm * c.p01) + dm * dm * c.p11);
  const double res = lik + prior;
  return lm > 5.0 ? -__builtin_inf() : res;
}

struct LPFast {
  double A, B, C, Dl, El, w;
};
__device__ __forceinline__ double log_post_fast(const LPFast& c, double ll, double lm, const double* tab) {
  const double t1 = __builtin_fma(c.A, ll, __builtin_fma(c.B, lm, c.Dl));
  const double t2 = __builtin_fma(c.C, lm, c.El);
  const double q = __builtin_fma(ll, t1, lm * t2);
  double el, em;
  exp_fast2(ll, lm, tab, el, em);
  return __builtin_fma(-c.w, el + em, q);
}

__device__ __forceinline__ uint64_t dbits(double x) { return __builtin_bit_cast(uint64_t, x); }
__device__ __forceinline__ double bitsd(uint64_t x) { return __builtin_bit_cast(double, x); }

__device__ __forceinline__ void swap_halves(double& a, double& b) {
  const uint64_t ua = dbits(a), ub = dbits(b);
  const auto lo = __builtin_amdgcn_permlane32_swap((uint32_t)ua, (uint32_t)ub, false, false);
  const auto hi = __builtin_amdgcn_permlane32_swap((uint32_t)(ua >> 32), (uint32_t)(ub >> 32), false, false);
  a = bitsd(((uint64_t)hi[0] << 32) | lo[0]);
  b = bitsd(((uint64_t)hi[1] << 32) | lo[1]);
}
__device__ __forceinline__ void swap_rows(double& a, double& b) {
  const uint64_t ua = dbits(a), ub = dbits(b);
  const auto lo = __builtin_amdgcn_permlane16_swap((uint32_t)ua, (uint32_t)ub, false, false);
  const auto hi = __builtin_amdgcn_permlane16_swap((uint32_t)(ua >> 32), (uint32_t)(ub >> 32), false, false);
  a = bitsd(((uint64_t)hi[0] << 32) | lo[0]);
  b = bitsd(((uint64_t)hi[1] << 32) | lo[1]);
}
template <int R>
__device__ __forceinline__ double add_row_ror(double x) {
  const uint64_t u = dbits(x);
  const uint32_t lo = __builtin_amdgcn_mov_dpp((uint32_t)u, 0x120 + R, 0xf, 0xf, true);
  const uint32_t hi = __builtin_amdgcn_mov_dpp((uint32_t)(u >> 32), 0x120 + R, 0xf, 0xf, true);
  return x + bitsd(((uint64_t)hi << 32) | lo);
}

__device__ __forceinline__ void lds_barrier() {
  __builtin_amdgcn_fence(__ATOMIC_RELEASE, "workgroup", "local");
  __builtin_amdgcn_s_barrier();
  __builtin_amdgcn_fence(__ATOMIC_ACQUIRE, "workgroup", "local");
}

template <int NS, int NT = BLOCK, bool LDS_ONLY = false>
__device__ __forceinline__ void block_reduce(double (&v)[NS], double (*red)[NS], double* out) {
  constexpr int H1 = (NS + 1) / 2;
  constexpr int H2 = (H1 + 1) / 2;
  const int lane = threadIdx.x & 63;
  const int wave = threadIdx.x >> 6;
  constexpr int NW = NT / 64;
  double w1[H1];
#pragma unroll
  for (int j = 0; j < H1; ++j) {
    double a = v[j];
    double b = (j + H1 < NS) ? v[j + H1] : 0.0;
    swap_halves(a, b);
    w1[j] = a + b;
  }
  double w2[H2];
#pragma unroll
  for (int j = 0; j < H2; ++j) {
    double a = w1[j];
    double b = (j + H2 < H1) ? w1[j + H2] : 0.0;
    swap_rows(a, b);
    w2[j] = a + b;
  }
#pragma unroll
  for (int j = 0; j < H2; ++j) {
    double x = w2[j];
    x = add_row_ror<8>(x);
    x = add_row_ror<4>(x);
    x = add_row_ror<2>(x);
    x = add_row_ror<1>(x);
    w2[j] = x;
  }
  if ((lane & 15) == 0) {
    const int row = lane >> 4;
#pragma unroll
    for (int j = 0; j < H2; ++j) {
      const int i1 = j + ((row & 1) ? H2 : 0);
      const int idx = i1 + ((row >> 1) ? H1 : 0);
      if (i1 < H1 && idx < NS) red[wave][idx] = w2[j];
    }
  }
  if constexpr (LDS_ONLY) lds_barrier(); else __syncthreads();
  if (threadIdx.x < NS) {
    double t = red[0][threadIdx.x];
#pragma unroll
    for (int w = 1; w < NW; ++w) t += red[w][threadIdx.x];
    out[threadIdx.x] = t;
  }
  if constexpr (LDS_ONLY) lds_barrier(); else __syncthreads();
}

template <int NS, int G, int NT = BLOCK, class Gen>
__device__ __forceinline__ void block_reduce_gen(const Gen& gen, double (*red)[NS], double* out) {
  const int lane = threadIdx.x & 63;
  const int wave = threadIdx.x >> 6;
  constexpr int NW = NT / 64;
#pragma unroll
  for (int base = 0; base < NS; base += G) {
    constexpr int GG = G;
    const int n = NS - base < GG ? NS - base : GG;
    const int h1 = (n + 1) / 2;
    const int h2 = (h1 + 1) / 2;
    double w1[(G + 1) / 2];
#pragma unroll
    for (int j = 0; j < (G + 1) / 2; ++j) {
      if (j < h1) {
        double a = gen(base + j);
        double b = (j + h1 < n) ? gen(base + j + h1) : 0.0;
        swap_halves(a, b);
        w1[j] = a + b;
      }
    }
    double w2[(G + 3) / 4];
#pragma unroll
    for (int j = 0; j < (G + 3) / 4; ++j) {
      if (j < h2) {
        double a = w1[j];
        double b = (j + h2 < h1) ? w1[j + h2] : 0.0;
        swap_rows(a, b);
        double x = a + b;
        x = add_row_ror<8>(x);
        x = add_row_ror<4>(x);
        x = add_row_ror<2>(x);
        x = add_row_ror<1>(x);
        w2[j] = x;
      }
    }
    if ((lane & 15) == 0) {
      const int row = lane >> 4;
#pragma unroll
      for (int j = 0; j < (G + 3) / 4; ++j) {
        const int i1 = j + ((row & 1) ? h2 : 0);
        const int idx = i1 + ((row >> 1) ? h1 : 0);
        if (j < h2 && i1 < h1 && idx < n) red[wave][base + idx] = w2[j];
      }
    }
  }
  __syncthreads();
  if (threadIdx.x < NS) {
    double t = red[0][threadIdx.x];
#pragma unroll
    for (int w = 1; w < NW; ++w) t += red[w][threadIdx.x];
    out[threadIdx.x] = t;
  }
  __syncthreads();
}

template <int D, int K>
struct StatGen {
  double xr[K];
  double Y[D];
  double lik;
  bool on;
  __device__ __forceinline__ double operator()(int j) const {
    double v;
    if (j < K * D) {
      v = xr[j / D] * Y[j % D];
    } else if (j < K * D + D * (D + 1) / 2) {
      v = 0.0;
      int t = K * D;
#pragma unroll
      for (int p = 0; p < D; ++p)
#pragma unroll
        for (int q = p; q < D; ++q, ++t)
          if (t == j) v = Y[p] * Y[q];
    } else {
      v = lik;
    }
    return v;
  }
};

#ifdef CLV_STAMPS
__device__ __forceinline__ void stamp(unsigned long long* st, int64_t s, int k, bool is_min) {
  if (!st) return;
  const unsigned long long t = __builtin_amdgcn_s_memrealtime();
  unsigned long long* p = st + (s & 1023) * 8 + k;
  if (is_min) __hip_atomic_fetch_min(p, t, __ATOMIC_RELAXED, __HIP_MEMORY_SCOPE_AGENT);
  else __hip_atomic_fetch_max(p, t, __ATOMIC_RELAXED, __HIP_MEMORY_SCOPE_AGENT);
}
#define CLV_STAMP(st, s, k, is_min) stamp(st, s, k, is_min)
__device__ __forceinline__ void wg_stamp(unsigned long long* st, int64_t wg, int k) {
  if (!st) return;
  unsigned long long v;
  if (k < 2) v = __builtin_amdgcn_s_memrealtime();
  else if (k == 2) v = __builtin_amdgcn_s_getreg((4 << 0) | (0 << 6) | (31 << 11));
  else if (k == 3) v = __builtin_amdgcn_s_getreg((20 << 0) | (0 << 6) | (15 << 11));
  else v = __builtin_amdgcn_s_memtime();
  st[1024 * 8 + wg * 12 + k] = v;
}
#define CLV_WG_STAMP(st, wg, k) wg_stamp(st, wg, k)
#define CLV_P_STAMP(st, wg, k, on) \
  do {                             \
    if ((on) && (st)) (st)[1024 * 8 + (wg) * 12 + (k)] = (k) == 8 ? __builtin_amdgcn_s_getreg((4 << 0) | (0 << 6) | (31 << 11)) : (k) == 9 ? __builtin_amdgcn_s_getreg((20 << 0) | (0 << 6) | (15 << 11)) : __builtin_amdgcn_s_memrealtime(); \
  } while (0)
#else
#define CLV_P_STAMP(st, wg, k, on) ((void)0)
#define CLV_WG_STAMP(st, wg, k) ((void)0)
#define CLV_STAMP(st, s, k, is_min) ((void)0)
#endif

__device__ __forceinline__ int64_t uniform_i64(int64_t v) {
  const uint32_t lo = __builtin_amdgcn_readfirstlane((uint32_t)v);
  const uint32_t hi = __builtin_amdgcn_readfirstlane((uint32_t)((uint64_t)v >> 32));
  return (int64_t)(((uint64_t)hi << 32) | lo);
}

__device__ __forceinline__ int64_t uniform64(int64_t x) {
  const uint32_t lo = __builtin_amdgcn_readfirstlane((uint32_t)x);
  const uint32_t hi = __builtin_amdgcn_readfirstlane((uint32_t)((uint64_t)x >> 32));
  return (int64_t)(((uint64_t)hi << 32) | lo);
}
__device__ __forceinline__ uint32_t stored_offset(int64_t s, const Geometry& g) {
  return (uint32_t)__builtin_amdgcn_readfirstlane((int32_t)(s - 1 - g.burnin));
}
__device__ __forceinline__ bool is_stored(int64_t s, const Geometry& g) {
  return s > g.burnin && s <= (int64_t)g.burnin + g.mcmc && stored_offset(s, g) % (uint32_t)g.thin == 0u;
}
__device__ __forceinline__ int64_t draw_index(int64_t s, const Geometry& g) {
  return (int64_t)(stored_offset(s, g) / (uint32_t)g.thin);
}

__global__ __launch_bounds__(64) void group_kernel(GroupArgs a) {
  const Geometry& g = a.g;
  const int u = blockIdx.x;
  const int c = blockIdx.y;
  const int j = threadIdx.x;
  if (j >= g.stride) return;
  const double* p = a.blockpart + ((int64_t)c * g.stride + j) * g.blocks_per_rank + (int64_t)u * g.blocks_per_unit;
  double t = 0.0;
  for (int bb = 0; bb < g.blocks_per_unit; ++bb) t += p[bb];
  a.unitpart[((int64_t)c * g.stride + j) * g.units_per_rank + u] = t;
}

#ifndef CLV_L2_NR
#define CLV_L2_NR 1
#endif
__device__ __forceinline__ double rsq_nr(double x) {
  double y = __builtin_amdgcn_rsq(x);
#pragma unroll
  for (int i = 0; i < 2; ++i) {
    const double h = x * y;
    const double e = __builtin_fma(-h, y, 1.0);
    y = __builtin_fma(0.5 * y, e, y);
  }
  return y;
}
__device__ __forceinline__ double rcp_nr(double x) {
  double y = __builtin_amdgcn_rcp(x);
#pragma unroll
  for (int i = 0; i < 2; ++i) y = __builtin_fma(y, __builtin_fma(-x, y, 1.0), y);
  return y;
}

template <int D, bool NR = false>
__device__ void cholesky(const double (&A)[D][D], double (&L)[D][D]) {
#pragma unroll
  for (int r = 0; r < D; ++r)
#pragma unroll
    for (int q = 0; q < D; ++q) L[r][q] = 0.0;
#pragma unroll
  for (int j = 0; j < D; ++j) {
    double sdiag = A[j][j];
#pragma unroll
    for (int k = 0; k < j; ++k) sdiag -= L[j][k] * L[j][k];
    const double rj = NR ? rsq_nr(sdiag) : 0.0;
    L[j][j] = NR ? sdiag * rj : sqrt(sdiag);
#pragma unroll
    for (int r = j + 1; r < D; ++r) {
      double sv = A[r][j];
#pragma unroll
      for (int k = 0; k < j; ++k) sv -= L[r][k] * L[j][k];
      L[r][j] = NR ? sv * rj : sv / L[j][j];
    }
  }
}

__device__ __forceinline__ void hstore(double* H, int idx, double v) {
  __hip_atomic_store(H + idx, v, __ATOMIC_RELAXED, __HIP_MEMORY_SCOPE_AGENT);
}

template <bool TO_LDS>
__device__ __forceinline__ void hput(double* H, int idx, double v) {
  if constexpr (TO_LDS) H[idx] = v;
  else hstore(H, idx, v);
}

template <int D, int K, bool TO_LDS = false, bool NR = false>
__device__ void finalize_hyper(const double* beta_flat, const double (&Sig)[D][D], double omega2, double* H) {
#pragma unroll
// ... 739 lines not shown
  const double ml = mu + lam;
  const double zz = ml * (T - tx);
  const double e = REPLAY ? exp(-zz) : exp_fast(-min700(zz), exp_tab);
  bool z;
  if constexpr (REPLAY) {
    const double p = (ml * e) / (ml * e + mu * (1.0 - e));
    z = u_z < p;
  } else {
    const double ae = ml * e;
    z = u_z * (ae + mu * (1.0 - e)) < ae;
  }
  u.z = z;

  double tau;
  if constexpr (REPLAY) {
    if (z) {
      tau = T + (1.0 / mu) * v_tau;
    } else {
      const double uu = v_tau;
      const double e_tx = exp(-min700(ml * tx));
      const double e_T = exp(-min700(ml * T));
      tau = -log((1 - uu) * e_tx + uu * e_T) / ml;
    }
  } else {
    const double uu = u53(rz, rw);
    double e_tx, e_T;
    exp_fast2(-min700(ml * tx), -min700(ml * T), exp_tab, e_tx, e_T);
    const double L = log_fast(z ? u53_open0(rz, rw) : (1 - uu) * e_tx + uu * e_T, exp_tab);
    const double q = L / (z ? mu : ml);
    tau = z ? T - q : -q;
  }
  u.tau = tau;
  u.lc.xm = u.xm;
  u.lc.omz = z ? 0.0 : 1.0;
  u.lc.w = z ? T : tau;
  if constexpr (REPLAY) {
    u.ll = log(lam);
    u.lm = log(mu);
  } else {
    u.ll = log_fast(lam, exp_tab);
    u.lm = log_fast(mu, exp_tab);
  }
}

template <int D, int K, bool REPLAY, bool CL>
__device__ __forceinline__ void cust_coeffs(Cust<D, K, CL>& u, const double* H, const double* exp_tab) {
  double m0 = 0.0, m1 = 0.0;
#pragma unroll
  for (int k = 0; k < K; ++k) {
    m0 += u.x(k) * H[H_BETA + k * D + 0];
    m1 += u.x(k) * H[H_BETA + k * D + 1];
  }
  LPConst& lc = u.lc;
  lc.m0 = m0;
  lc.m1 = m1;
  lc.p00 = H[H_P00];
  lc.p01 = H[H_P01];
  lc.p11 = H[H_P11];
  if constexpr (REPLAY) {
    u.cur = log_post(lc, u.ll, u.lm);
  } else {
    LPFast& fc = u.fc;
    fc.A = -0.5 * lc.p00;
    fc.B = -lc.p01;
    fc.C = -0.5 * lc.p11;
    fc.Dl = lc.xm + lc.p00 * lc.m0 + lc.p01 * lc.m1;
    fc.El = lc.omz + lc.p01 * lc.m0 + lc.p11 * lc.m1;
    fc.w = lc.w;
    u.cur = u.lm > 5.0 ? -__builtin_inf() : log_post_fast(fc, u.ll, u.lm, exp_tab);
  }
}

template <int D, int K, bool REPLAY, bool CL>
__device__ __forceinline__ void cust_prepare(Cust<D, K, CL>& u, const SweepArgs& a, int c, int64_t s, const double* H,
                                             uint32_t k0, uint32_t k1, const double* tape, const double* exp_tab) {
  (void)c;
  cust_ztau<D, K, REPLAY>(u, a, s, k0, k1, tape, exp_tab);
  cust_coeffs<D, K, REPLAY>(u, H, exp_tab);
}

__device__ __forceinline__ double clip70_fma(double a, double b, double c) {
  double r, lo = -70.0, hi = 70.0;
  asm("v_fma_f64 %0, %1, %2, %3" : "=v"(r) : "v"(a), "v"(b), "v"(c));
  asm("v_max_f64 %0, %1, %2" : "=v"(r) : "v"(r), "s"(lo));
  asm("v_min_f64 %0, %1, %2" : "=v"(r) : "v"(r), "s"(hi));
  return r;
}

__device__ __forceinline__ double prop_lm(double a, double b, double c) {
  double r, lo = -70.0;
  asm("v_fma_f64 %0, %1, %2, %3" : "=v"(r) : "v"(a), "v"(b), "v"(c));
  asm("v_max_f64 %0, %1, %2" : "=v"(r) : "v"(r), "s"(lo));
  return r;
}

template <int D, int K, bool CL>
__device__ __forceinline__ void mh_step(Cust<D, K, CL>& u, double s00, double s11, float t_l, float t_m, float l2u,
                                        const double* exp_tab) {
  const double thr = __builtin_fma((double)l2u, 0x1.62e42fefa39efp-1, u.cur);
  const double pl = clip70_fma(s00, (double)t_l, u.ll);
  const double pm = prop_lm(s11, (double)t_m, u.lm);
  const double plp = log_post_fast(u.fc, pl, pm, exp_tab);
  uint64_t m0, m1, sv;
  const double five = 5.0;
  asm volatile(
      "v_cmp_ge_f64_e64 %[m0], %[five], %[pm]\n\t"
      "v_cmp_gt_f64_e64 %[m1], %[plp], %[thr]\n\t"
      "s_and_saveexec_b64 %[sv], %[m0]\n\t"
      "s_and_b64 exec, exec, %[m1]\n\t"
      "v_mov_b64 %[ll], %[pl]\n\t"
      "v_mov_b64 %[lm], %[pm]\n\t"
      "v_mov_b64 %[cur], %[plp]\n\t"
      "s_mov_b64 exec, %[sv]"
      : [ll] "+v"(u.ll), [lm] "+v"(u.lm), [cur] "+v"(u.cur), [m0] "=&s"(m0), [m1] "=&s"(m1), [sv] "=&s"(sv)
      : [pl] "v"(pl), [pm] "v"(pm), [plp] "v"(plp), [thr] "v"(thr), [five] "s"(five)
      : "scc");
}

template <bool PIPE = (SWEEP_MH_PIPELINE != 0), int D, int K, bool CL>
__device__ __forceinline__ void mh_run(Cust<D, K, CL>& cu, const SlotPhilox& ph, double s00, double s11, int S,
                                       const double* exp_tab, int q0 = 0) {
  constexpr int MC = MH_CHUNK_STEPS;
  const int n_chunks = (S + MC - 1) / MC;
  if (n_chunks <= q0) return;
  float tl[MC], tm[MC], lu[MC];
  constexpr bool PK = D == 3;
  if constexpr (!PIPE) {
  for (int ch = q0; ch < n_chunks; ++ch) {
    mh_chunk_variates<PK>(ph, (uint32_t)ch, tl, tm, lu);
    const int rem = S - ch * MC;
#pragma unroll
    for (int st = 0; st < MC; ++st) mh_step(cu, s00, s11, tl[st], tm[st], st < rem ? lu[st] : __builtin_inff(), exp_tab);
  }
  return;
  }
  mh_chunk_variates<PK>(ph, (uint32_t)q0, tl, tm, lu);
  for (int ch = q0; ch + 1 < n_chunks; ++ch) {
    float ntl[MC], ntm[MC], nlu[MC];
    mh_chunk_variates<PK>(ph, (uint32_t)(ch + 1), ntl, ntm, nlu);
#pragma unroll
    for (int st = 0; st < MC; ++st) mh_step(cu, s00, s11, tl[st], tm[st], lu[st], exp_tab);
#pragma unroll
    for (int st = 0; st < MC; ++st) {
      tl[st] = ntl[st];
      tm[st] = ntm[st];
      lu[st] = nlu[st];
    }
  }
  const int rem = S - (n_chunks - 1) * MC;
#pragma unroll
  for (int st = 0; st < MC; ++st) mh_step(cu, s00, s11, tl[st], tm[st], st < rem ? lu[st] : __builtin_inff(), exp_tab);
}

constexpr int PRE_STEPS = 20;
constexpr int PRE_LDS_BYTES = PRE_STEPS * BLOCK * 12;
struct PreVariates {
  float2* t;
  float* u;
  int lane;
};

__device__ __forceinline__ int opaque_uniform(int x) {
  x = __builtin_amdgcn_readfirstlane(x);
  asm volatile("" : "+s"(x));
  return x;
}

template <int NQ = PRE_STEPS / MH_CHUNK_STEPS>
__device__ __forceinline__ void mh_pre_variates(const SlotPhilox& ph, int S_, const PreVariates& v) {
  constexpr int MC = MH_CHUNK_STEPS;
  const int S = opaque_uniform(S_);
#pragma unroll
  for (int q = 0; q < NQ; ++q) {
    if (q * MC < S) {
      float tl[MC], tm[MC], lu[MC];
      mh_chunk_variates(ph, (uint32_t)q, tl, tm, lu);
      if (q * MC + MC <= S) {
#pragma unroll
        for (int st = 0; st < MC; ++st) {
          const int k = q * MC + st;
          v.t[k * BLOCK + v.lane] = make_float2(tl[st], tm[st]);
          v.u[k * BLOCK + v.lane] = lu[st];
        }
      } else {
#pragma unroll
        for (int st = 0; st < MC; ++st) {
          const int k = q * MC + st;
          v.t[k * BLOCK + v.lane] = make_float2(tl[st], tm[st]);
          v.u[k * BLOCK + v.lane] = k < S ? lu[st] : __builtin_inff();
        }
      }
    }
  }
}

template <int NQ = PRE_STEPS / MH_CHUNK_STEPS, int D, int K, bool CL>
__device__ __forceinline__ void mh_run_pre(Cust<D, K, CL>& cu, const PreVariates& v, double s00, double s11, int S,
                                           const double* exp_tab) {
  constexpr int MC = MH_CHUNK_STEPS;
  S = opaque_uniform(S);
#pragma unroll
  for (int q = 0; q < NQ; ++q) {
    if (q * MC < S) {
      float2 t[MC];
      float u[MC];
#pragma unroll
      for (int st = 0; st < MC; ++st) {
        t[st] = v.t[(q * MC + st) * BLOCK + v.lane];
        u[st] = v.u[(q * MC + st) * BLOCK + v.lane];
      }
#pragma unroll
      for (int st = 0; st < MC; ++st) mh_step(cu, s00, s11, t[st].x, t[st].y, u[st], exp_tab);
    }
  }
}

template <int D>
struct CustOut {
  double lam, mu, eta, lgl, lgm, leta;
};

__device__ __forceinline__ double eta_normal(uint32_t k0, uint32_t k1, uint32_t gi, int64_t s, const double* tab) {
  const u32x4 r = customer_block(k0, k1, gi, (uint32_t)s, SLOT_ETA);
  return sqrt(-2.0 * log_fast(u53_open0(r.x, r.y), tab)) * cos2pi_u53(r.z, r.w, tab);
}

template <int D, int K, bool REPLAY, bool CL>
__device__ __forceinline__ CustOut<D> cust_finish(Cust<D, K, CL>& u, const SweepArgs& a, int64_t s, bool stored,
                                                  const double* H, uint32_t k0, uint32_t k1, const double* tape,
                                                  const double* exp_tab, StatGen<D, K>& st,
                                                  const double* zeta_pre = nullptr) {
  const Geometry& g = a.g;
  const int64_t i = u.i;
  double lam, mu;
  if constexpr (REPLAY) {
    lam = exp(u.ll);
    mu = exp(u.lm);
  } else {
    exp_fast2(u.ll, u.lm, exp_tab, lam, mu);
  }
  double eta = 1.0, leta = 0.0, Y[D];
  if constexpr (D == 3) {
    double m2 = 0.0;
#pragma unroll
    for (int k = 0; k < K; ++k) m2 += u.x(k) * H[H_BETA + k * D + 2];
    const double post_var = H[H_POSTVAR];
    const double post_mean = REPLAY ? post_var * (a.log_s[i] / H[H_OMEGA2] + m2 / H[H_S22])
                                    : post_var * __builtin_fma(a.log_s[i], H[H_INV_OMEGA2], m2 * H[H_INV_S22]);
    double zeta;
    if constexpr (REPLAY) {
      zeta = tape[(int64_t)(2 + 3 * g.S) * g.n + i];
    } else {
      zeta = zeta_pre ? *zeta_pre : eta_normal(k0, k1, u.gi, s, exp_tab);
    }
    const double xe = post_mean + H[H_SQRT_POSTVAR] * zeta;
    if constexpr (REPLAY) {
      eta = exp(xe);
      leta = log(eta);
    } else {
      if (__builtin_fabs(xe) <= 700.0) eta = exp_fast(xe, exp_tab);
      else eta = exp(xe);
      leta = xe;
    }
    Y[0] = REPLAY ? log(lam) : u.ll;
    Y[1] = REPLAY ? log(mu) : u.lm;
    Y[2] = leta;
  }
  double lik = 0.0, lgl = 0.0, lgm = 0.0;
  if (stored) {
    if constexpr (REPLAY) {
      lam = exp(log(lam));
      mu = exp(log(mu));
    }
    lgl = REPLAY ? log(lam) : u.ll;
    lgm = REPLAY ? log(mu) : u.lm;
    lik = (u.xm * lgl + u.lc.omz * lgm) - (lam + mu) * u.lc.w;
  }
  if constexpr (D == 2) {
    Y[0] = REPLAY ? log(lam) : u.ll;
    Y[1] = REPLAY ? log(mu) : u.lm;
  }
  u.lam = lam;
  u.mu = mu;
#pragma unroll
  for (int k = 0; k < K; ++k) st.xr[k] = u.x(k);
#pragma unroll
  for (int d = 0; d < D; ++d) st.Y[d] = Y[d];
  st.lik = lik;
  st.on = true;
  return CustOut<D>{lam, mu, eta, lgl, lgm, leta};
}

template <int D>
struct SumsPre {
  static constexpr int N = D == 3 ? CLV_N_SUM_STATS : CLV_N_SUM_STATS - 2;
  static __device__ __forceinline__ constexpr int slot(int k) { return (D == 3 || k < CLV_SUM_ETA) ? k : k - 2; }
  double v[N];
};
template <int D>
__device__ __forceinline__ void prefetch_sums(const SweepArgs& a, int c, int64_t i, SumsPre<D>& p) {
  const double* sm = a.sums + (int64_t)c * CLV_N_SUM_STATS * a.g.n + i;
#pragma unroll
  for (int k = 0; k < CLV_N_SUM_STATS; ++k) {
    if (D == 2 && (k == CLV_SUM_ETA || k == CLV_SUM_LOG_ETA)) continue;
    p.v[SumsPre<D>::slot(k)] = sm[(int64_t)k * a.g.n];
  }
}

template <int D, int K, bool CL>
__device__ __forceinline__ void cust_store(const Cust<D, K, CL>& u, const CustOut<D>& o, const SweepArgs& a, int c,
                                           int64_t s, bool stored, bool store_state,
                                           const SumsPre<D>* pre = nullptr) {
  const Geometry& g = a.g;
  const int64_t i = u.i;
  if (stored) {
    const int64_t dr = draw_index(s, g);
    if (a.level1) {
      double* w = a.level1 + (((int64_t)c * g.n_draws + dr) * g.n + i) * (D + 2);
      w[0] = o.lam;
      w[1] = o.mu;
      w[2] = u.tau;
      w[3] = u.z ? 1.0 : 0.0;
      if constexpr (D == 3) w[4] = o.eta;
    }
    if (a.sums) {
      double* sm = a.sums + (int64_t)c * CLV_N_SUM_STATS * g.n + i;
      auto acc = [&](int k, double v) {
        if (pre) sm[k * g.n] = pre->v[SumsPre<D>::slot(k)] + v;
        else sm[k * g.n] += v;
      };
      acc(CLV_SUM_LAMBDA, o.lam);
      acc(CLV_SUM_MU, o.mu);
      acc(CLV_SUM_Z, u.z ? 1.0 : 0.0);
      acc(CLV_SUM_LOG_LAMBDA, o.lgl);
      acc(CLV_SUM_LOG_MU, o.lgm);
      acc(CLV_SUM_LAMBDA2, o.lam * o.lam);
      acc(CLV_SUM_MU2, o.mu * o.mu);
      if constexpr (D == 3) {
        acc(CLV_SUM_ETA, o.eta);
        acc(CLV_SUM_LOG_ETA, o.leta);
      }
      acc(CLV_SUM_MU_CAPPED, fmin(o.mu, CLV_SUMMARY_MU_CAP));
      acc(CLV_SUM_TAU, u.tau);
    }
    if (a.qstore)
      a.qstore[((int64_t)c * g.n_draws + dr) * g.n + i] = make_float2((float)o.lam, (float)o.mu);
  }
  if (store_state) {
    const int64_t ci = (int64_t)c * g.n + i;
    a.lam[ci] = o.lam;
    a.mu[ci] = o.mu;
  }
}

static_assert(BLOCK == EXP_TAB_N, "the sweep kernel stages the exp table with one entry per lane");

template <int D, int K, bool REPLAY, bool FX>
__device__ __forceinline__ void sweep_body(const SweepArgs& a) {
  constexpr int NT = BLOCK;
  constexpr int NXY = K * D;
  constexpr int NYY = D * (D + 1) / 2;
  constexpr int NS = NXY + NYY + 1;
// ... 177 lines not shown
      __syncthreads();
      __builtin_amdgcn_fence(__ATOMIC_ACQUIRE, "wavefront");
      if (!s_last) {
        finish_store();
        return;
      }
      if (threadIdx.x < NS) {
        const double* p = a.blockpart + ((int64_t)c * g.stride + threadIdx.x) * g.blocks_per_rank + (int64_t)u * bpu;
        double t = 0.0;
        int bb = 0;
        for (; bb + 8 <= bpu; bb += 8) {
          double v[8];
#pragma unroll
          for (int q = 0; q < 8; ++q) v[q] = __hip_atomic_load(p + bb + q, __ATOMIC_RELAXED, __HIP_MEMORY_SCOPE_AGENT);
#pragma unroll
          for (int q = 0; q < 8; ++q) t += v[q];
        }
        for (; bb < bpu; ++bb) t += __hip_atomic_load(p + bb, __ATOMIC_RELAXED, __HIP_MEMORY_SCOPE_AGENT);
        if (fx) {
          for (int q = 0; q < g.world_size; ++q) st_sys(a.peers[q] + mail_off + (int64_t)u * NS + threadIdx.x, t);
        } else {
          __hip_atomic_store(a.unitpart + ((int64_t)c * g.stride + threadIdx.x) * g.units_per_rank + u, t,
                             __ATOMIC_RELAXED, __HIP_MEMORY_SCOPE_AGENT);
        }
      }
      units = a.unitpart;
    }
    if (bpu > 1 || fx) {
      asm volatile("s_waitcnt vmcnt(0)" ::: "memory");
      __syncthreads();
    }
    if (threadIdx.x == 0) {
      CLV_STAMP(a.stamps, s, 1, false);
      CLV_STAMP(a.stamps, s, 4, true);
      CLV_WG_STAMP(a.stamps, (int64_t)c * g.nb_local + b, 1);
      CLV_WG_STAMP(a.stamps, (int64_t)c * g.nb_local + b, 7);
      const uint32_t n_arrivals = (uint32_t)((g.nb_local + bpu - 1) / bpu);
      const uint32_t old = __hip_atomic_fetch_add(a.chain_arrive + c, 1u, __ATOMIC_RELAXED, __HIP_MEMORY_SCOPE_AGENT);
      const uint32_t last = old == n_arrivals - 1 ? 1u : 0u;
      if (last) __hip_atomic_store(a.chain_arrive + c, 0u, __ATOMIC_RELAXED, __HIP_MEMORY_SCOPE_AGENT);
      s_last = last;
    }
    __syncthreads();
    __builtin_amdgcn_fence(__ATOMIC_ACQUIRE, "wavefront");
    finish_store();
    if (s_last) {
      if (threadIdx.x == 0) CLV_STAMP(a.stamps, s, 2, false);
      if (!fx) {
        hyper_body<D, K, REPLAY, NS, NT>(a.h, c, s, 0, units, red, tot, var_iw, var_chi, var_noise, &l2);
      } else {
        hyper_variates<D, K, REPLAY>(a.h, c, s, var_iw, var_chi, var_noise, &l2);
        const int64_t u0 = threadIdx.x, u1 = threadIdx.x + NT;
        const bool h0 = u0 < g.n_units_global, h1 = u1 < g.n_units_global;
        const double* mb = a.mail + (int64_t)(s & 1) * g.world_size * mail_rank + (int64_t)c * g.units_per_rank * NS;
        double* p0 = (double*)mb + (u0 / g.units_per_rank) * mail_rank + (u0 % g.units_per_rank) * NS;
        double* p1 = (double*)mb + (u1 / g.units_per_rank) * mail_rank + (u1 % g.units_per_rank) * NS;
        const double* q0 = h0 ? p0 : mb;
        const double* q1 = h1 ? p1 : mb;
        __shared__ uint32_t s_fx_abort;
        if (threadIdx.x == 0) {
          s_fx_abort = 0;
          post_progress(a, a.peers, s);
        }
        __syncthreads();
        constexpr int FXC = NS <= 16 ? NS : 12;
        double acc[NS];
        bool timed_out = false;
#pragma unroll
        for (int j0 = 0; j0 < NS; j0 += FXC) {
          double v0[FXC], v1[FXC];
          const uint64_t t0 = __builtin_amdgcn_s_memrealtime();
          for (uint32_t poll = 0; !timed_out; ++poll) {
            bool ok = true;
#pragma unroll
            for (int q = 0; q < FXC; ++q) {
              if (j0 + q < NS) {
                v0[q] = ld_sys(q0 + j0 + q);
                v1[q] = ld_sys(q1 + j0 + q);
                ok = ok & (!h0 | slot_full(v0[q])) & (!h1 | slot_full(v1[q]));
              }
            }
            if (__all(ok)) break;
            const int ws = wait_state(a, t0, poll, a.wait_ticks);
            if (ws == WAIT_OBSERVED) {
              timed_out = true;
            } else if (ws == WAIT_EXPIRED) {
              timed_out = true;
              int64_t mu_ = -1;
              int mj = -1;
              uint64_t mb = 0;
#pragma unroll
              for (int q = FXC - 1; q >= 0; --q) {
                if (j0 + q < NS) {
                  if (h1 && !slot_full(v1[q])) { mu_ = u1; mj = j0 + q; mb = dbits(v1[q]); }
                  if (h0 && !slot_full(v0[q])) { mu_ = u0; mj = j0 + q; mb = dbits(v0[q]); }
                }
              }
              report_wait(a, WAIT_FX_MAIL, s, c, ok, mu_, mj, mb, poll, t0);
              raise_abort(a);
            } else {
              __builtin_amdgcn_s_sleep(1);
            }
          }
#pragma unroll
          for (int q = 0; q < FXC; ++q) {
            if (j0 + q < NS) {
              acc[j0 + q] = 0.0;
              if (h0) acc[j0 + q] += v0[q];
              if (h1) acc[j0 + q] += v1[q];
            }
          }
        }
        if (timed_out) s_fx_abort = 1;
        __syncthreads();
        if (!s_fx_abort) {
          const int nrun = g.units_per_rank * NS;
          hyper_finish<D, K, REPLAY, NS, NT>(a.h, c, s, 0, acc, red, tot, var_iw, var_chi, var_noise, &l2, [&] {
            for (int e = (int)threadIdx.x - 64; e >= 0 && e < g.world_size * nrun; e += NT - 64) {
              const int q = e / nrun;
              st_sys((double*)mb + (int64_t)q * mail_rank + (e - q * nrun), slot_empty());
            }
          });
        }
      }
      if (threadIdx.x == 0) CLV_STAMP(a.stamps, s, 3, false);
    }
  }
}


template <int D, int K, bool REPLAY, bool FX>
__global__ __launch_bounds__(BLOCK) void sweep_kernel(SweepArgs a) {
  sweep_body<D, K, REPLAY, FX>(a);
}
template <int D, int K, bool REPLAY, bool FX>
__global__ __launch_bounds__(BLOCK, 4) void sweep_kernel_occ4(SweepArgs a) {
  sweep_body<D, K, REPLAY, FX>(a);
}

template <int D, int K, bool REPLAY, bool FX>
hipError_t launch_sweep_t(const SweepArgs& a, hipStream_t st, hipEvent_t e0, hipEvent_t e1) {
  const dim3 grid(a.g.nb_local, a.g.n_chains);
  const dim3 block(BLOCK);
  if constexpr (SweepOcc<D, K>::value >= 4) {
    if (e0) hipExtLaunchKernelGGL((sweep_kernel_occ4<D, K, REPLAY, FX>), grid, block, 0, st, e0, e1, 0, a);
    else hipLaunchKernelGGL((sweep_kernel_occ4<D, K, REPLAY, FX>), grid, block, 0, st, a);
  } else {
    if (e0) hipExtLaunchKernelGGL((sweep_kernel<D, K, REPLAY, FX>), grid, block, 0, st, e0, e1, 0, a);
    else hipLaunchKernelGGL((sweep_kernel<D, K, REPLAY, FX>), grid, block, 0, st, a);
  }
  return hipGetLastError();
}

template <int D, int K, bool P2P>
__device__ __forceinline__ void persist_level2(const SweepArgs& a, int64_t s_first, int64_t n_sweeps, int c, uint32_t k0,
                                            uint32_t k1, int64_t wgi, int64_t it_stamp, double* pool) {
  constexpr int NT = BLOCK;
  constexpr int NXY = K * D;
  constexpr int NYY = D * (D + 1) / 2;
  constexpr int NS = NXY + NYY + 1;
  constexpr int NTRIL = D * (D - 1) / 2;
  (void)NXY;
  __shared__ double red[BLOCK / 64][NS];
  __shared__ double tot[NS];
  __shared__ double Hs[HS];
  __shared__ uint32_t s_abort;
  __shared__ double var_iw[4], var_chi[4], var_noise[32];
  __shared__ L2Scratch l2;
  __shared__ double* s_peers[P2P ? MAX_WORLD : 1];
  const Geometry& g = a.g;
  const int tid0 = threadIdx.x;
  (void)wgi;
  double* parts0 = a.pblock + (int64_t)c * g.nb_local * NS;
  if (tid0 == 0) s_abort = 0;
  if constexpr (P2P) {
    if (tid0 < g.world_size) s_peers[tid0] = a.peers[tid0];
  }
  __syncthreads();
  __builtin_amdgcn_s_setprio(3);
  stage_prior(a.h.V, &l2);
  const double* pin = P2P ? nullptr : a.pend_in;
  double* pout = P2P ? nullptr : a.pend_out;
  ClockMark clk_prev = CLV_CLOCK_RECORD && a.clk && c == 0 ? ClockMark::now() : ClockMark{0, 0};
  for (int64_t it = pin ? -1 : 0; it < n_sweeps; ++it) {
    int tid = tid0;
    double* parts = parts0;
    if constexpr (CLV_L2_OPAQUE(P2P)) {
      asm volatile("" : "+v"(tid));
      asm volatile("" : "+s"(parts));
    }
    const int64_t s = s_first + it;
    const bool stp = tid == 0 && it == it_stamp;
    (void)stp;
    const int64_t hs = (D == 2) ? s + 1 : s;
    const bool from_pend = it < 0;
    const bool defer_now = pout && it == n_sweeps - 1;
    CLV_P_STAMP(a.stamps, wgi, 0, stp);
    if (!defer_now) {
      if (tid < NTRIL) var_iw[tid] = hyper_normal(k0, k1, HSLOT_NORMAL0 + tid, (uint32_t)hs);
      if (tid >= 32 && tid < 32 + D * K) var_noise[tid - 32] = hyper_normal(k0, k1, HSLOT_BETA_NORMAL0 + (tid - 32), (uint32_t)hs);
      if (tid >= 64 && tid < 64 + D) var_chi[tid - 64] = chi2_draw(k0, k1, (uint32_t)hs, tid - 64, a.h.nu_n - D + 1 + (tid - 64));
    }
    if (from_pend && tid < NS) tot[tid] = pin[(int64_t)c * NS + tid];
    __syncthreads();
    if (!defer_now && tid == 0) bartlett_inverse<D>(var_iw, var_chi, l2.Ai);
    CLV_P_STAMP(a.stamps, wgi, 1, stp);
    if (!from_pend) {
    double v0[NS], v1[NS];
    const int b0 = tid, b1 = tid + NT;
    const bool hb0 = b0 < g.nb_local, hb1 = b1 < g.nb_local;
    double* pb0 = parts + (int64_t)b0 * NS;
    double* pb1 = parts + (int64_t)b1 * NS;
    const double* qb0 = hb0 ? pb0 : parts;
    const double* qb1 = hb1 ? pb1 : parts;
    const int64_t per_rank = (int64_t)g.n_chains * NS * g.units_per_rank;
    const double* mb = a.mail + (int64_t)(s & 1) * g.world_size * per_rank + (int64_t)c * NS * g.units_per_rank;
    const int64_t u0 = tid, u1 = tid + NT;
    const int r0 = (int)(u0 / g.units_per_rank), r1 = (int)(u1 / g.units_per_rank);
    const int l0 = (int)(u0 % g.units_per_rank), l1 = (int)(u1 % g.units_per_rank);
    const double* p0 = mb + r0 * per_rank + (int64_t)l0 * NS;
    const double* p1 = mb + r1 * per_rank + (int64_t)l1 * NS;
    const bool h0 = u0 < g.n_units_global, h1 = u1 < g.n_units_global;
    const bool m0 = P2P && h0 && r0 != a.rank, m1 = P2P && h1 && r1 != a.rank;
    const double* q0 = m0 ? p0 : mb;
    const double* q1 = m1 ? p1 : mb;
    double w0[NS], w1[NS];
    bool mdone = !(m0 || m1);
    if constexpr (P2P) {
      if (tid == 0) post_progress(a, s_peers, s);
    }
    const uint64_t t0 = __builtin_amdgcn_s_memrealtime();
    {
      bool done = false;
      for (uint32_t poll = 0;; ++poll) {
        if (!done) {
          bool ok = true;
#pragma unroll
          for (int j = 0; j < NS; ++j) {
            v0[j] = ld_wt(qb0 + j);
            v1[j] = ld_wt(qb1 + j);
          }
#pragma unroll
          for (int j = 0; j < NS; ++j) ok = ok & (!hb0 | slot_full(v0[j])) & (!hb1 | slot_full(v1[j]));
          done = ok;
        }
        if constexpr (P2P) {
          if (!mdone) {
            bool ok = true;
#pragma unroll
            for (int j = 0; j < NS; ++j) {
              w0[j] = ld_sys(q0 + j);
              w1[j] = ld_sys(q1 + j);
            }
#pragma unroll
            for (int j = 0; j < NS; ++j) ok = ok & (!m0 | slot_full(w0[j])) & (!m1 | slot_full(w1[j]));
            mdone = ok;
          }
        }
        if (__all(done)) break;
        const int ws = wait_state(a, t0, poll, a.wait_ticks);
        if (ws == WAIT_OBSERVED) {
          s_abort = 1;
          break;
        }
        if (ws == WAIT_EXPIRED) {
          int64_t mb_ = -1;
          int mj = -1;
          uint64_t mbits = 0;
#pragma unroll
          for (int j = NS - 1; j >= 0; --j) {
            if (hb1 && !slot_full(v1[j])) { mb_ = b1; mj = j; mbits = dbits(v1[j]); }
            if (hb0 && !slot_full(v0[j])) { mb_ = b0; mj = j; mbits = dbits(v0[j]); }
          }
          report_wait(a, WAIT_BLOCKS, s, c, done, mb_, mj, mbits, poll, t0);
          raise_abort(a);
          s_abort = 1;
          break;
        }
        __builtin_amdgcn_s_sleep(1);
      }
    }
    __syncthreads();
    if (s_abort) return;
#pragma unroll
    for (int j = 0; j < NS; ++j) {
      v0[j] = hb0 ? v0[j] : 0.0;
      v1[j] = hb1 ? v1[j] : 0.0;
    }
    CLV_P_STAMP(a.stamps, wgi, 2, stp);
    double acc[NS];
    if constexpr (!P2P) {
#pragma unroll
      for (int j = 0; j < NS; ++j) {
        acc[j] = 0.0;
        if (hb0) acc[j] += v0[j];
        if (hb1) acc[j] += v1[j];
      }
    } else {
      double* umail = pool;
      const int bpu = g.blocks_per_unit;
      const int ul = (g.nb_local + bpu - 1) / bpu;
      const int lane = tid & 63;
#pragma unroll
      for (int half = 0; half < 2; ++half) {
        const double* v = half ? v1 : v0;
        const int ub = (tid + half * NT) / bpu;
        double t[NS];
        if (bpu == 1) {
#pragma unroll
          for (int j = 0; j < NS; ++j) t[j] = v[j];
        } else {
#pragma unroll
          for (int j = 0; j < NS; ++j) t[j] = 0.0 + v[j];
          for (int k = 1; k < bpu; ++k) {
#pragma unroll
            for (int j = 0; j < NS; ++j) t[j] += __shfl(v[j], lane + k, 64);
          }
        }
        if (tid % bpu == 0 && ub < ul) {
#pragma unroll
          for (int j = 0; j < NS; ++j) umail[ub * NS + j] = t[j];
        }
      }
      lds_barrier();
      CLV_P_STAMP(a.stamps, wgi, 10, stp);
      const int64_t dst = ((int64_t)(s & 1) * g.world_size + a.rank) * per_rank + (int64_t)c * NS * g.units_per_rank;
      for (int e = tid; e < NS * ul; e += NT) {
        const double v = umail[e];
        for (int q = 0; q < g.world_size; ++q)
          if (q != a.rank) st_sys(s_peers[q] + dst + e, v);
      }
      const uint64_t tw = t0;
      for (uint32_t poll = 0; !__all(mdone); ++poll) {
        if (!mdone) {
          bool ok = true;
#pragma unroll
          for (int j = 0; j < NS; ++j) {
            w0[j] = ld_sys(q0 + j);
            w1[j] = ld_sys(q1 + j);
          }
#pragma unroll
          for (int j = 0; j < NS; ++j) ok = ok & (!m0 | slot_full(w0[j])) & (!m1 | slot_full(w1[j]));
          mdone = ok;
        }
        if (__all(mdone)) break;
        const int ws = wait_state(a, tw, poll, a.wait_ticks);
        if (ws == WAIT_OBSERVED) {
          s_abort = 1;
          break;
        }
        if (ws == WAIT_EXPIRED) {
          int64_t mu_ = -1;
          int mj = -1;
          uint64_t mbits = 0;
#pragma unroll
          for (int j = NS - 1; j >= 0; --j) {
            if (m1 && !slot_full(w1[j])) { mu_ = u1; mj = j; mbits = dbits(w1[j]); }
            if (m0 && !slot_full(w0[j])) { mu_ = u0; mj = j; mbits = dbits(w0[j]); }
          }
          report_wait(a, WAIT_P2P_MAIL, s, c, mdone, mu_, mj, mbits, poll, tw);
          raise_abort(a);
          s_abort = 1;
          break;
        }
        __builtin_amdgcn_s_sleep(1);
      }
      CLV_P_STAMP(a.stamps, wgi, 11, stp);
      lds_barrier();
      if (s_abort) return;
#pragma unroll
      for (int j = 0; j < NS; ++j) {
        const double x0 = m0 ? w0[j] : (h0 ? umail[l0 * NS + j] : 0.0);
        const double x1 = m1 ? w1[j] : (h1 ? umail[l1 * NS + j] : 0.0);
        acc[j] = 0.0;
        if (h0) acc[j] += x0;
        if (h1) acc[j] += x1;
      }
    }
    block_reduce<NS, NT, P2P>(acc, red, tot);
    CLV_P_STAMP(a.stamps, wgi, 6, stp);
    const int rt = tid - 64;
    if (rt >= 0) {
      const int nrec = g.nb_local * NS;
      for (int e = rt; e < nrec; e += NT - 64) st_wt(parts + e, slot_empty());
      if ((it > 0 || pin) && rt < HS) st_wt(a.hyp2 + ((int64_t)(s & 1) * g.n_chains + c) * HS + rt, slot_empty());
    }
    if constexpr (P2P) {
      const int nrun = g.units_per_rank * NS;
      for (int e = rt; rt >= 0 && e < g.world_size * nrun; e += NT - 64) {
        const int q = e / nrun;
        if (q != a.rank) st_sys((double*)mb + (int64_t)q * per_rank + (e - q * nrun), slot_empty());
      }
    }
    }
    if (defer_now) {
      if (tid < NS) pout[(int64_t)c * NS + tid] = tot[tid];
      if (tid == 0) {
        if (is_stored(s, g)) a.h.loglik[(int64_t)c * g.n_draws + draw_index(s, g)] = tot[NS - 1] / (double)g.n_global;
        a.ctrl_rw->cur = s;
      }
      return;
    }
    if (tid < HS) Hs[tid] = 0.0;
    level2_draw<D, K, P2P ? 6 : CLV_L2_LANE0_MAX>(tot, var_iw, var_chi, var_noise, false, &l2, l2.Ai);
    CLV_P_STAMP(a.stamps, wgi, 7, stp);
    if (tid == 0) {
      double Sig[D][D];
#pragma unroll
      for (int p = 0; p < D; ++p)
#pragma unroll
        for (int q = 0; q < D; ++q) Sig[p][q] = l2.Sig[p * D + q];
      finalize_hyper<D, K, true, CLV_L2_NR != 0>(l2.beta, Sig, a.h.omega2, Hs);
    }
    CLV_P_STAMP(a.stamps, wgi, 3, stp);
    asm volatile("s_waitcnt vmcnt(0)" ::: "memory");
    __syncthreads();
    const bool last = it == n_sweeps - 1;
    if (tid < HS) {
      if (last) a.hyper_out[(int64_t)c * HS + tid] = Hs[tid];
      else st_wt(a.hyp2 + ((int64_t)((s + 1) & 1) * g.n_chains + c) * HS + tid, Hs[tid]);
    }
    CLV_P_STAMP(a.stamps, wgi, 4, stp);
    CLV_P_STAMP(a.stamps, wgi, 5, tid == 0 && it + 1 == it_stamp);
    if (CLV_CLOCK_RECORD && a.clk && c == 0 && tid == 0) clk_prev = clock_mark(a.clk, s, clk_prev);
#ifdef CLV_STAMPS
    if (tid == 0 && a.stamps && c < 8 && it % 4 == 0 && it / 4 < 1024)
      a.stamps[(it / 4) * 8 + c] = __builtin_amdgcn_s_memrealtime();
#endif
    const bool store_l2 = hs >= 1 && is_stored(hs, g);
    double* o = store_l2 ? a.h.level2 + ((int64_t)c * g.n_draws + draw_index(hs, g)) * g.l2w : nullptr;
    if (tid < K * D && store_l2) o[(tid % D) * K + tid / D] = l2.beta[tid];
    if (tid == 0) {
      if (store_l2) {
        int q = K * D;
#pragma unroll
        for (int p = 0; p < D; ++p)
#pragma unroll
          for (int r = p; r < D; ++r) o[q++] = l2.Sig[p * D + r];
      }
      if (!from_pend && is_stored(s, g)) a.h.loglik[(int64_t)c * g.n_draws + draw_index(s, g)] = tot[NS - 1] / (double)g.n_global;
      if (last) a.ctrl_rw->cur = s;
    }
    __syncthreads();
  }
  return;
}

__device__ __forceinline__ const SweepArgs& kernargs_fresh() {
  auto p4 = (const __attribute__((address_space(4))) SweepArgs*)__builtin_amdgcn_kernarg_segment_ptr();
  asm volatile("" : "+s"(p4));
  return *(const SweepArgs*)p4;
}

#ifndef CLV_PERSIST_FRESH_ARGS
#define CLV_PERSIST_FRESH_ARGS 1
#endif
template <bool FRESH>
__device__ __forceinline__ const SweepArgs& loop_args(const SweepArgs& a) {
  if constexpr (FRESH) return kernargs_fresh();
  else return a;
}

template <int D, int K, bool P2P>
__global__ __launch_bounds__(BLOCK, 2) void persist_kernel(SweepArgs a, int64_t s_first, int64_t n_sweeps) {
  constexpr int NXY = K * D;
  constexpr int NYY = D * (D + 1) / 2;
  constexpr int NS = NXY + NYY + 1;
  __shared__ double red[BLOCK / 64][NS];
  __shared__ double tot[NS];
  __shared__ __attribute__((aligned(16))) double exp_tab[D == 3 ? FAST_TAB_N3 : FAST_TAB_N];
  __shared__ double Hs[HS];
  __shared__ uint32_t s_abort;
  __shared__ __attribute__((aligned(16))) char pool[PRE_LDS_BYTES];
  static_assert(UMAIL * sizeof(double) <= PRE_LDS_BYTES, "the level-2 unit partials share the variates' LDS");
  __shared__ double zeta_lds[D == 3 ? BLOCK : 1];
  const Geometry& g = a.g;
  int c = blockIdx.y, b = blockIdx.x;
  if (a.wg_map) {
    const int32_t m = a.wg_map[blockIdx.y * gridDim.x + blockIdx.x];
    c = m >> 16;
    b = m & 0xFFFF;
  }
  const int tid = threadIdx.x;
  const int64_t wgi = (int64_t)c * (g.nb_local + 1) + b;
  const int64_t it_stamp = n_sweeps >= 2 ? n_sweeps - 2 : 0;
  (void)wgi;
  (void)it_stamp;
  uint32_t k0, k1;
  chain_key(a.r.seed, (int64_t)a.r.chain_first + c, &k0, &k1);
  double* parts = a.pblock + (int64_t)c * g.nb_local * NS;
  if (tid == 0) s_abort = 0;

  if (b == g.nb_local) {
    persist_level2<D, K, P2P>(a, s_first, n_sweeps, c, k0, k1, wgi, it_stamp, (double*)pool);
    return;
  }

  CLV_P_STAMP(a.stamps, wgi, 7, tid == 0);
  Cust<D, K> cu;
  {
    const int64_t i = (int64_t)b * BLOCK + tid;
    cu.active = i < g.n;
    cu.i = cu.active ? i : (g.n > 0 ? g.n - 1 : 0);
  }
  cust_load(cu, a, c);
  fast_tab_fill(exp_tab, tid, BLOCK, D == 3);
  if (tid < HS) Hs[tid] = a.hyper[(int64_t)c * HS + tid];
  __syncthreads();
  if (cu.active) cust_ztau<D, K, false>(cu, a, s_first, k0, k1, nullptr, exp_tab);
  const bool pre = g.S <= PRE_STEPS;
  const PreVariates pv{(float2*)pool, (float*)(pool + PRE_STEPS * BLOCK * 8), tid};
  if (cu.active && pre) mh_pre_variates(SlotPhilox(k0, k1, cu.gi, (uint32_t)s_first), g.S, pv);
  if constexpr (D == 3) {
    if (cu.active && pre) zeta_lds[tid] = eta_normal(k0, k1, cu.gi, s_first, exp_tab);
  }
  CLV_P_STAMP(a.stamps, wgi, 10, tid == 0);
  const SweepArgs& a_launch = a;
  for (int64_t it = 0; it < n_sweeps; ++it) {
    const SweepArgs& a = loop_args<CLV_PERSIST_FRESH_ARGS && D == 2>(a_launch);
    const Geometry& g = a.g;
    const double* hyp_c = a.hyp2 + (int64_t)c * HS;
    if constexpr (CLV_OPAQUE_GI(D)) asm volatile("" : "+v"(cu.gi));
    const int64_t s = uniform64(s_first + it);
    const bool stored = is_stored(s, g);
    const bool stp = tid == 0 && it == it_stamp;
    (void)stp;
    CLV_P_STAMP(a.stamps, wgi, 0, stp);
    if (it > 0 || (!P2P && a.pend_in)) {
      if (tid < 64) {
        const double* src = hyp_c + (int64_t)(s & 1) * g.n_chains * HS;
        const uint64_t t0 = __builtin_amdgcn_s_memrealtime();
        for (uint32_t poll = 0;; ++poll) {
          const double v = ld_wt(src + tid);
          if (__all(slot_full(v))) {
            Hs[tid] = v;
            break;
          }
          const int ws = wait_state(a, t0, poll, hyper_wait_ticks(a));
          if (ws != WAIT_GOING) {
            if (ws == WAIT_EXPIRED) {
              report_wait(a, WAIT_HYPER, s, c, slot_full(v), b, tid, dbits(v), poll, t0);
              raise_abort(a);
            }
            if (tid == 0) s_abort = 1;
            break;
          }
          __builtin_amdgcn_s_sleep(1);
        }
      }
      __syncthreads();
      if (s_abort) return;
    }
    CLV_P_STAMP(a.stamps, wgi, 1, stp);
    StatGen<D, K> st{};
    CustOut<D> out{};
    __builtin_amdgcn_s_setprio(2);
    if (cu.active) {
      cust_coeffs<D, K, false>(cu, Hs, exp_tab);
      CLV_P_STAMP(a.stamps, wgi, 2, stp);
      const double s00 = Hs[H_S00];
      const double s11 = Hs[H_S11];
      if (pre) mh_run_pre(cu, pv, s00, s11, g.S, exp_tab);
      else mh_run(cu, SlotPhilox(k0, k1, cu.gi, (uint32_t)s), s00, s11, g.S, exp_tab);
      CLV_P_STAMP(a.stamps, wgi, 3, stp);
      if constexpr (D == 3) {
        if (!pre) zeta_lds[tid] = eta_normal(k0, k1, cu.gi, s, exp_tab);
      }
      out = cust_finish<D, K, false>(cu, a, s, stored, Hs, k0, k1, nullptr, exp_tab, st,
                                     D == 3 ? &zeta_lds[tid] : nullptr);
    }
    CLV_P_STAMP(a.stamps, wgi, 4, stp);
#if PERSIST_REDUCE_GEN
    block_reduce_gen<NS, SWEEP_REDUCE_CHUNK>(st, red, tot);
#else
    {
      double acc[NS];
#pragma unroll
      for (int j = 0; j < NS; ++j) acc[j] = st(j);
      block_reduce<NS>(acc, red, tot);
    }
#endif
    if (tid < NS) st_wt(parts + (int64_t)b * NS + tid, tot[tid]);
    __builtin_amdgcn_s_setprio(0);
    CLV_P_STAMP(a.stamps, wgi, 5, stp);
    CLV_P_STAMP(a.stamps, wgi, 8, stp);
    CLV_P_STAMP(a.stamps, wgi, 9, stp);
#ifdef CLV_STAMPS
    if (stp && a.stamps) a.stamps[1024 * 8 + wgi * 12 + 11] = blockIdx.y * gridDim.x + blockIdx.x;
#endif
    if (cu.active) {
      cust_store<D, K>(cu, out, a, c, s, stored, false);
      if (it + 1 < n_sweeps) {
        cust_ztau<D, K, false>(cu, a, s + 1, k0, k1, nullptr, exp_tab);
        if (pre) mh_pre_variates(SlotPhilox(k0, k1, cu.gi, (uint32_t)(s + 1)), g.S, pv);
        if constexpr (D == 3) {
          if (pre) zeta_lds[tid] = eta_normal(k0, k1, cu.gi, s + 1, exp_tab);
        }
      }
    }
    CLV_P_STAMP(a.stamps, wgi, 6, stp);
  }
  if (cu.active) {
    const int64_t ci = (int64_t)c * g.n + cu.i;
    a.lam_out[ci] = cu.lam;
    a.mu_out[ci] = cu.mu;
  }
}

template <int D, int K>
__global__ __launch_bounds__(BLOCK) void persist_flush_kernel(SweepArgs a, int64_t s_first) {
  __shared__ double pool[1];
  const int c = blockIdx.y;
  uint32_t k0, k1;
  chain_key(a.r.seed, (int64_t)a.r.chain_first + c, &k0, &k1);
  persist_level2<D, K, false>(a, s_first, 0, c, k0, k1, 0, -2, pool);
}

template <int D, int K, bool NR>
__global__ void set_hyper_kernel(int n_chains, double* hyper, const double* bs, double omega2) {
  const int c = threadIdx.x;
  if (c >= n_chains) return;
  const double* in = bs + (int64_t)c * (K * D + D * D);
  double Sig[D][D];
  for (int p = 0; p < D; ++p)
    for (int q = 0; q < D; ++q) Sig[p][q] = in[K * D + p * D + q];
  finalize_hyper<D, K, false, NR>(in, Sig, omega2, hyper + (int64_t)c * HS);
}

__global__ void debug_philox_kernel(uint32_t k0, uint32_t k1, const uint32_t* ctr, int64_t n, uint32_t* out) {
  const int64_t i = (int64_t)blockIdx.x * blockDim.x + threadIdx.x;
  if (i >= n) return;
  const u32x4 r = philox4x32_10(u32x4{ctr[4 * i], ctr[4 * i + 1], ctr[4 * i + 2], ctr[4 * i + 3]}, k0, k1);
  out[4 * i] = r.x;
  out[4 * i + 1] = r.y;
  out[4 * i + 2] = r.z;
  out[4 * i + 3] = r.w;
}

__global__ void debug_variates_kernel(uint64_t seed, int chain, uint32_t sweep, int64_t n, int S, float* tl,
                                      float* tm, float* ua, float* l2u, double* uz, double* ut, double* ea,
                                      double* ez) {
  __shared__ __attribute__((aligned(16))) double tab[FAST_TAB_N3];
  fast_tab_fill(tab, threadIdx.x, blockDim.x, true);
  __syncthreads();
  const int64_t i = (int64_t)blockIdx.x * blockDim.x + threadIdx.x;
  if (i >= n) return;
  uint32_t k0, k1;
  chain_key(seed, chain, &k0, &k1);
  const u32x4 r = customer_block(k0, k1, (uint32_t)i, sweep, SLOT_ZTAU);
  uz[i] = u53(r.x, r.y);
  ut[i] = u53(r.z, r.w);
  ea[i] = -log_fast(u53_open0(r.z, r.w), tab);
  ez[i] = eta_normal(k0, k1, (uint32_t)i, sweep, tab);
  const SlotPhilox ph(k0, k1, (uint32_t)i, sweep);
  for (int j = 0; j < S; ++j) {
    const u32x4 r = ph(SLOT_MH0 + (uint32_t)j);
    tl[(int64_t)j * n + i] = t3_f32(uf32(r.x), angle_hi(r.z));
    tm[(int64_t)j * n + i] = t3_f32(uf32(r.y), angle_lo(r.z));
    ua[(int64_t)j * n + i] = uf32(r.w);
    l2u[(int64_t)j * n + i] = log2_f32(uf32(r.w));
  }
}

__global__ void debug_log2u_scan_kernel(uint64_t w_begin, uint64_t w_end, double* out) {
  double mu = 0.0, ma = 0.0, wu = 0.0, mf = 0.0;
  const uint64_t stride = (uint64_t)gridDim.x * blockDim.x;
  for (uint64_t w = w_begin + (uint64_t)blockIdx.x * blockDim.x + threadIdx.x; w < w_end; w += stride) {
    const float u = uf32((uint32_t)w);
    const float y = log2_f32(u);
    const double e = log2((double)u);
    double err_ulp;
    if (e == 0.0) {
      err_ulp = y == 0.0f ? 0.0 : 1e30;
    } else {
      const double ulp = ldexp(1.0, ilogb(e) - 23);
      err_ulp = fabs((double)y - e) / ulp;
    }
    const double ae = fabs((double)y - e);
    if (err_ulp > mu) {
      mu = err_ulp;
      wu = (double)w;
    }
    ma = fmax(ma, ae);
    if (u <= 0.5f) mf = fmax(mf, err_ulp);
  }
  __shared__ double red[4][256];
  red[0][threadIdx.x] = mu;
  red[1][threadIdx.x] = ma;
  red[2][threadIdx.x] = wu;
  red[3][threadIdx.x] = mf;
  __syncthreads();
  if (threadIdx.x == 0) {
    double bm = 0.0, ba = 0.0, bw = 0.0, bf = 0.0;
    for (int t = 0; t < 256; ++t) {
      if (red[0][t] > bm) {
        bm = red[0][t];
        bw = red[2][t];
      }
      ba = fmax(ba, red[1][t]);
      bf = fmax(bf, red[3][t]);
    }
    out[4 * blockIdx.x] = bm;
    out[4 * blockIdx.x + 1] = ba;
    out[4 * blockIdx.x + 2] = bw;
    out[4 * blockIdx.x + 3] = bf;
  }
}

__global__ void debug_t3_kernel(const uint32_t* w, int64_t n, int packed, float* tl, float* tm) {
  const int64_t i = (int64_t)blockIdx.x * blockDim.x + threadIdx.x;
  if (i >= n) return;
  const uint32_t x = w[3 * i], y = w[3 * i + 1], z = w[3 * i + 2];
  if (packed) {
    const f32x2 t = t3_pair(x, y, z);
    tl[i] = t.x;
    tm[i] = t.y;
  } else {
    tl[i] = t3_f32(uf32(x), angle_hi(z));
    tm[i] = t3_f32(uf32(y), angle_lo(z));
  }
}

template <int D, int K>
__global__ void debug_level2_kernel(const double* prior, const double* in, double* out) {
  constexpr int NXY = K * D;
  __shared__ double tot[NXY + D * (D + 1) / 2 + 1];
  __shared__ L2Scratch sc;
  if (threadIdx.x == 0) {
    for (int q = 0; q < NXY; ++q) tot[q] = in[q];
    int t = NXY;
    for (int p = 0; p < D; ++p)
      for (int q = p; q < D; ++q) tot[t++] = in[NXY + p * D + q];
  }
  __syncthreads();
  const double* iwn = in + NXY + D * D;
  const double* chi = iwn + 3;
  const double* z = chi + 3;
  stage_prior(prior, &sc);
  __syncthreads();
  level2_draw<D, K>(tot, iwn, chi, z, false, &sc);
  if (threadIdx.x == 0) {
    for (int q = 0; q < K * D; ++q) out[q] = sc.beta[q];
    for (int q = 0; q < D * D; ++q) out[K * D + q] = sc.Sig[q];
  }
}

__global__ void debug_hyper_variates_kernel(uint64_t seed, int chain, uint32_t sweep, double df, int64_t n,
                                            double* chi2, double* normals) {
  const int64_t i = (int64_t)blockIdx.x * blockDim.x + threadIdx.x;
  if (i >= n) return;
  uint32_t k0, k1;
  chain_key(seed, chain, &k0, &k1);
  chi2[i] = chi2_draw(k0, k1, sweep + (uint32_t)i, 0, df);
  normals[i] = hyper_normal(k0, k1, HSLOT_NORMAL0, sweep + (uint32_t)i);
}

template <bool LOG>
__global__ void debug_exp_kernel(const double* x, int64_t n, double* out) {
  __shared__ __attribute__((aligned(16))) double tab[FAST_TAB_N];
  fast_tab_fill(tab, threadIdx.x, blockDim.x);
  __syncthreads();
  const int64_t i = (int64_t)blockIdx.x * blockDim.x + threadIdx.x;
  if (i < n) out[i] = LOG ? log_fast(x[i], tab) : exp_fast(x[i], tab);
}

__global__ void debug_mh_kernel(const int32_t* x, const uint8_t* z, const double* T, const double* tau,
                                const double* m, const double* prec, const double* cur_pt, const float* t3,
                                const double* scale, const float* log_u, int64_t n, double* out) {
  __shared__ __attribute__((aligned(16))) double tab[FAST_TAB_N];
  fast_tab_fill(tab, threadIdx.x, blockDim.x);
  __syncthreads();
  const int64_t i = (int64_t)blockIdx.x * blockDim.x + threadIdx.x;
  if (i >= n) return;
  double H[HS];
  for (int j = 0; j < HS; ++j) H[j] = 0.0;
  H[H_BETA + 0] = m[2 * i];
  H[H_BETA + 1] = m[2 * i + 1];
  H[H_P00] = prec[0];
  H[H_P01] = prec[1];
  H[H_P11] = prec[2];
  Cust<2, 1> u;
  u.xr_[0] = 1.0;
  u.xm = (double)x[i];
  u.z = z[i] != 0;
  u.lc.xm = u.xm;
  u.lc.omz = u.z ? 0.0 : 1.0;
  u.lc.w = u.z ? T[i] : tau[i];
  u.ll = cur_pt[2 * i];
  u.lm = cur_pt[2 * i + 1];
  cust_coeffs<2, 1, false>(u, H, tab);
  const double cur0 = u.cur;
  const double pl = clip70_fma(scale[0], (double)t3[2 * i], u.ll);
  const double pm = prop_lm(scale[1], (double)t3[2 * i + 1], u.lm);
  const double plp = log_post_fast(u.fc, pl, pm, tab);
  mh_step(u, scale[0], scale[1], t3[2 * i], t3[2 * i + 1], log_u[i], tab);
  double* o = out + 7 * i;
  o[0] = cur0;
  o[1] = plp;
  o[2] = pl;
  o[3] = pm;
  o[4] = u.ll;
  o[5] = u.lm;
  o[6] = u.cur;
}

#ifdef CLV_ONLY_K
#define CLV_FOR_K(M, D, R) M(D, CLV_ONLY_K, R)
#else
#define CLV_FOR_K(M, D, R) \
  M(D, 1, R) M(D, 2, R) M(D, 3, R) M(D, 4, R) M(D, 5, R) M(D, 6, R) M(D, 7, R) M(D, 8, R) M(D, 9, R)
#endif

hipError_t launch_sweep(const SweepArgs& a, bool replay, hipStream_t st, hipEvent_t e0, hipEvent_t e1) {
  const bool fx = a.fuse && a.g.world_size > 1;
#define CLV_CASE(DD, KK, RR)                                                      \
  if (a.g.D == DD && a.g.K == KK && replay == RR) {                               \
    if constexpr (!RR) {                                                          \
      if (fx) return launch_sweep_t<DD, KK, RR, true>(a, st, e0, e1);             \
    }                                                                             \
    return launch_sweep_t<DD, KK, RR, false>(a, st, e0, e1);                      \
  }
  CLV_FOR_K(CLV_CASE, 2, false)
  CLV_FOR_K(CLV_CASE, 3, false)
  CLV_FOR_K(CLV_CASE, 2, true)
  CLV_FOR_K(CLV_CASE, 3, true)
#undef CLV_CASE
  return hipErrorInvalidValue;
}

hipError_t launch_persist_flush(const SweepArgs& a, int64_t s_first, hipStream_t st) {
  const dim3 grid(1, a.g.n_chains);
#define CLV_CASE(DD, KK, PP)                                                                     \
  if (a.g.D == DD && a.g.K == KK) {                                                              \
    hipLaunchKernelGGL((persist_flush_kernel<DD, KK>), grid, dim3(BLOCK), 0, st, a, s_first);  \
    return hipGetLastError();                                                                  \
  }
  CLV_FOR_K(CLV_CASE, 2, false)
  CLV_FOR_K(CLV_CASE, 3, false)
#undef CLV_CASE
  return hipErrorInvalidValue;
}

hipError_t launch_persist(const SweepArgs& a, int64_t s_first, int64_t n_sweeps, hipStream_t st, hipEvent_t e0,
                          hipEvent_t e1) {
  const dim3 grid(a.g.nb_local + 1, a.g.n_chains);
  const dim3 block(BLOCK);
#define CLV_CASE(DD, KK, PP)                                                                                         \
  if (a.g.D == DD && a.g.K == KK && (a.g.world_size > 1) == PP) {                                                \
    if (e0) hipExtLaunchKernelGGL((persist_kernel<DD, KK, PP>), grid, block, 0, st, e0, e1, 0, a, s_first, n_sweeps); \
    else hipLaunchKernelGGL((persist_kernel<DD, KK, PP>), grid, block, 0, st, a, s_first, n_sweeps);                  \
    return hipGetLastError();                                                                                      \
  }
  CLV_FOR_K(CLV_CASE, 2, false)
  CLV_FOR_K(CLV_CASE, 3, false)
  CLV_FOR_K(CLV_CASE, 2, true)
  CLV_FOR_K(CLV_CASE, 3, true)
#undef CLV_CASE
  return hipErrorInvalidValue;
}

hipError_t persist_occupancy(int D, int K, bool p2p, int* blocks_per_cu) {
#define CLV_CASE(DD, KK, PP) \
  if (D == DD && K == KK && p2p == PP) return hipOccupancyMaxActiveBlocksPerMultiprocessor(blocks_per_cu, persist_kernel<DD, KK, PP>, BLOCK, 0);
  CLV_FOR_K(CLV_CASE, 2, false)
  CLV_FOR_K(CLV_CASE, 3, false)
  CLV_FOR_K(CLV_CASE, 2, true)
  CLV_FOR_K(CLV_CASE, 3, true)
#undef CLV_CASE
  return hipErrorInvalidValue;
}

hipError_t persist_scratch_bytes(int D, int K, bool p2p, size_t* bytes) {
  hipFuncAttributes fa{};
#define CLV_CASE(DD, KK, PP)                                                                     \
  if (D == DD && K == KK && p2p == PP) {                                                         \
    const hipError_t e = hipFuncGetAttributes(&fa, reinterpret_cast<const void*>(&persist_kernel<DD, KK, PP>)); \
    *bytes = fa.localSizeBytes;                                                                  \
    return e;                                                                                    \
  }
  CLV_FOR_K(CLV_CASE, 2, false)
  CLV_FOR_K(CLV_CASE, 3, false)
  CLV_FOR_K(CLV_CASE, 2, true)
  CLV_FOR_K(CLV_CASE, 3, true)
#undef CLV_CASE
  return hipErrorInvalidValue;
}

hipError_t launch_group(const GroupArgs& a, hipStream_t st) {
  const int units_local = (a.g.nb_local + a.g.blocks_per_unit - 1) / a.g.blocks_per_unit;
  hipLaunchKernelGGL(group_kernel, dim3(units_local, a.g.n_chains), dim3(64), 0, st, a);
  return hipGetLastError();
}

hipError_t launch_hyper(const HyperArgs& a, bool replay, hipStream_t st) {
#define CLV_CASE(DD, KK, RR) \
  if (a.g.D == DD && a.g.K == KK && replay == RR) { hipLaunchKernelGGL((hyper_kernel<DD, KK, RR>), dim3(a.g.n_chains), dim3(256), 0, st, a); return hipGetLastError(); }
  CLV_FOR_K(CLV_CASE, 2, false)
  CLV_FOR_K(CLV_CASE, 3, false)
  CLV_FOR_K(CLV_CASE, 2, true)
  CLV_FOR_K(CLV_CASE, 3, true)
#undef CLV_CASE
  return hipErrorInvalidValue;
}

hipError_t launch_set_hyper(int D, int K, int n_chains, double* hyper, const double* bs, double omega2,
                            bool replay, hipStream_t st) {
#define CLV_CASE(DD, KK, RR) \
  if (D == DD && K == KK && replay == RR) { hipLaunchKernelGGL((set_hyper_kernel<DD, KK, !RR && CLV_L2_NR != 0>), dim3(1), dim3(64), 0, st, n_chains, hyper, bs, omega2); return hipGetLastError(); }
  CLV_FOR_K(CLV_CASE, 2, false)
  CLV_FOR_K(CLV_CASE, 3, false)
  CLV_FOR_K(CLV_CASE, 2, true)
  CLV_FOR_K(CLV_CASE, 3, true)
#undef CLV_CASE
  return hipErrorInvalidValue;
}

hipError_t launch_debug_philox(uint32_t k0, uint32_t k1, const uint32_t* ctr, int64_t n, uint32_t* out,
                               hipStream_t st) {
  hipLaunchKernelGGL(debug_philox_kernel, dim3((unsigned)((n + 255) / 256)), dim3(256), 0, st, k0, k1, ctr, n, out);
  return hipGetLastError();
}

hipError_t launch_debug_variates(uint64_t seed, int chain, uint32_t sweep, int64_t n, int S, float* tl,
                                 float* tm, float* ua, float* l2u, double* uz, double* ut, double* ea, double* ez,
                                 hipStream_t st) {
  hipLaunchKernelGGL(debug_variates_kernel, dim3((unsigned)((n + 255) / 256)), dim3(256), 0, st, seed, chain,
                     sweep, n, S, tl, tm, ua, l2u, uz, ut, ea, ez);
  return hipGetLastError();
}

hipError_t launch_debug_log2u_scan(uint64_t w_begin, uint64_t w_end, int n_blocks, double* out, hipStream_t st) {
  hipLaunchKernelGGL(debug_log2u_scan_kernel, dim3((unsigned)n_blocks), dim3(256), 0, st, w_begin, w_end, out);
  return hipGetLastError();
}

hipError_t launch_debug_t3(const uint32_t* w, int64_t n, int packed, float* tl, float* tm, hipStream_t st) {
  hipLaunchKernelGGL(debug_t3_kernel, dim3((unsigned)((n + 255) / 256)), dim3(256), 0, st, w, n, packed, tl, tm);
  return hipGetLastError();
}

hipError_t launch_debug_level2(int D, int K, const double* prior_dev, const double* in, double* out,
                               hipStream_t st) {
#define CLV_CASE(DD, KK, RR) \
  if (D == DD && K == KK) { hipLaunchKernelGGL((debug_level2_kernel<DD, KK>), dim3(1), dim3(256), 0, st, prior_dev, in, out); return hipGetLastError(); }
  CLV_FOR_K(CLV_CASE, 2, 0)
  CLV_FOR_K(CLV_CASE, 3, 0)
#undef CLV_CASE
  return hipErrorInvalidValue;
}

hipError_t launch_debug_hyper_variates(uint64_t seed, int chain, uint32_t sweep, double df, int64_t n,
                                       double* chi2, double* normals, hipStream_t st) {
  hipLaunchKernelGGL(debug_hyper_variates_kernel, dim3((unsigned)((n + 255) / 256)), dim3(256), 0, st, seed,
                     chain, sweep, df, n, chi2, normals);
  return hipGetLastError();
}

hipError_t launch_debug_exp(const double* x, int64_t n, double* out, hipStream_t st, bool log_fn) {
  if (log_fn) hipLaunchKernelGGL(debug_exp_kernel<true>, dim3((unsigned)((n + 255) / 256)), dim3(256), 0, st, x, n, out);
  else hipLaunchKernelGGL(debug_exp_kernel<false>, dim3((unsigned)((n + 255) / 256)), dim3(256), 0, st, x, n, out);
  return hipGetLastError();
}

hipError_t launch_debug_mh(const int32_t* x, const uint8_t* z, const double* T, const double* tau, const double* m,
                           const double* prec, const double* cur_pt, const float* t3, const double* scale,
                           const float* log_u, int64_t n, double* out, hipStream_t st) {
  hipLaunchKernelGGL(debug_mh_kernel, dim3((unsigned)((n + 255) / 256)), dim3(256), 0, st, x, z, T, tau, m, prec,
                     cur_pt, t3, scale, log_u, n, out);
  return hipGetLastError();
}

}
```

### mcmc_clv_model_amd/sampler.py

```python
from __future__ import annotations

import ctypes
import weakref
import math
from dataclasses import dataclass, field
from typing import List, Optional, Sequence

import numpy as np

from . import _lib
from ._lib import check, dptr

BLOCK_SIZE = _lib.BLOCK


@dataclass
class Problem:
    D: int
    K: int
    x: np.ndarray
    t_x: np.ndarray
    T_cal: np.ndarray
    cov: np.ndarray
    log_s: Optional[np.ndarray]
# ... 59 lines not shown
        pr.V[i] = v
    for i, v in enumerate(cholV.ravel()):
        pr.chol_V[i] = v
    for i, v in enumerate(A0B0.ravel()):
        pr.A0B0[i] = v
    for i, v in enumerate(S0B.ravel()):
        pr.S0_B0A0B0[i] = v
    pr.nu_n = p.nu_00 + (p.N if n_global is None else n_global)
    for i, v in enumerate(p.beta_0.ravel()):
        pr.beta_init[i] = v
    for i, v in enumerate(p.gamma_00.ravel()):
        pr.sigma_init[i] = v
    pr.omega2 = p.omega2
    return pr


def resolve_seed(seed: Optional[int]) -> int:
    if seed is None:
        return int(np.random.SeedSequence().entropy) & ((1 << 63) - 1)
    seed = int(seed)
    if seed < 0:
        raise ValueError("expected non-negative integer")
    if seed >= 1 << 63:
        w = np.random.SeedSequence(seed).generate_state(2, np.uint32)
        return (int(w[0]) | (int(w[1]) << 32)) & ((1 << 63) - 1)
    return seed


_SINKS = {"full": _lib.SINK_FULL, "summary": _lib.SINK_SUMMARY, "summary+pct": _lib.SINK_SUMMARY_PCT,
          "none": _lib.SINK_NONE}
_RNGS = {"philox": _lib.RNG_PHILOX, "replay": _lib.RNG_REPLAY}


class HipSampler:

    def __init__(self, p: Problem, *, mcmc: int, burnin: int, thin: int, chains: int, seed: int,
                 n_mh_steps: int = 20, draw_sink: str = "full", rng: str = "philox", device: int = -1,
                 chain_first: int = 0, n_global: Optional[int] = None, shard_begin: int = 0,
                 world_size: int = 1, rank: int = 0, blocks_per_rank: int = 0, blocks_per_unit: int = 0,
                 stream: int = 0, prior: Optional[_lib.ClvPrior] = None):
        L = _lib.lib()
        if draw_sink not in _SINKS:
            raise ValueError(f"draw_sink must be one of {sorted(_SINKS)}")
        if rng not in _RNGS:
            raise ValueError(f"rng must be one of {sorted(_RNGS)}")
        if _lib.device_count() < 1:
            raise _lib.ClvError("no HIP device visible; the sampler has no CPU fallback")
        self.p = p
        self.D, self.K, self.n = p.D, p.K, p.N
        self.chains = int(chains)
        self.mcmc, self.burnin, self.thin = int(mcmc), int(burnin), int(thin)
        self.n_draws = (self.mcmc - 1) // self.thin + 1 if self.mcmc >= 1 else 0
        self.draw_sink = draw_sink
        cfg = _lib.ClvConfig()
        cfg.abi_version = _lib.ABI_VERSION
        cfg.D, cfg.K, cfg.n_mh_steps = p.D, p.K, int(n_mh_steps)
        cfg.burnin, cfg.mcmc, cfg.thin = self.burnin, self.mcmc, self.thin
        cfg.n_chains, cfg.chain_first = self.chains, int(chain_first)
        cfg.rng_mode, cfg.draw_sink, cfg.device = _RNGS[rng], _SINKS[draw_sink], int(device)
        cfg.seed = int(seed)
        cfg.n_global = int(p.N if n_global is None else n_global)
        cfg.shard_begin = int(shard_begin)
        cfg.world_size, cfg.rank = int(world_size), int(rank)
        cfg.blocks_per_rank, cfg.blocks_per_unit = int(blocks_per_rank), int(blocks_per_unit)
        cfg.stream = int(stream)
        self.cfg = cfg
        data = _lib.ClvData()
        data.n = p.N
        self._keep = [p.x, p.t_x, p.T_cal, p.cov, p.log_s]
        data.x = p.x.ctypes.data if p.N else None
        data.t_x = p.t_x.ctypes.data if p.N else None
        data.T_cal = p.T_cal.ctypes.data if p.N else None
        data.covariates = p.cov.ctypes.data if (p.K > 1 and p.N) else None
        data.log_s = p.log_s.ctypes.data if (p.D == 3 and p.N) else None
        self.prior = prior if prior is not None else make_prior(p, cfg.n_global)
        h = ctypes.c_void_p()
        check(L.clv_create(ctypes.byref(cfg), ctypes.byref(data), ctypes.byref(self.prior), ctypes.byref(h)))
        self.h = h
        self._L = L

    def close(self) -> None:
        for grp in list(getattr(self, "_groups", ())):
            grp.close()
        if getattr(self, "h", None):
            self._L.clv_destroy(self.h)
            self.h = None

    def __del__(self):
        try:
            self.close()
        except Exception:
            pass

    def __enter__(self):
        return self

    def __exit__(self, *exc):
        self.close()

    def run(self, n_sweeps: int) -> None:
        check(self._L.clv_run(self.h, int(n_sweeps)))

    def rollback(self) -> None:
        check(self._L.clv_rollback(self.h))

    def sweep(self) -> None:
        check(self._L.clv_sweep(self.h))

    def hyper(self, gathered_ptr: Optional[int] = None) -> None:
        check(self._L.clv_hyper(self.h, gathered_ptr))

    def partials(self):
        ptr = ctypes.c_void_p()
        nd = ctypes.c_int64()
        st = ctypes.c_int32()
        check(self._L.clv_partials(self.h, ctypes.byref(ptr), ctypes.byref(nd), ctypes.byref(st)))
        return ptr.value, nd.value, st.value

    def set_stream(self, stream: int) -> None:
        check(self._L.clv_set_stream(self.h, int(stream)))

    def note_sweeps(self, n: int) -> None:
        check(self._L.clv_note_sweeps(self.h, int(n)))

    def copy_partials(self, dst_ptr: int) -> None:
        check(self._L.clv_copy_partials(self.h, ctypes.c_void_p(dst_ptr)))

    def synchronize(self) -> None:
        check(self._L.clv_synchronize(self.h))

    def host_times(self) -> dict:
        hn = (ctypes.c_int64 * 8)()
        check(self._L.clv_debug_host_times(self.h, hn))
        h = [x / 1e3 for x in hn]
        if not h[0] or not h[6]:
            return {}
        names = ("set_device", "start_event", "launch_call", "end_event", "wait", "return")
        return {k: round(h[i + 1] - h[i], 3) for i, k in enumerate(names)}

    def clock_ghz(self) -> float:
        v = ctypes.c_double(0.0)
        check(self._L.clv_clock_ghz(self.h, ctypes.byref(v)))
        return float(v.value)

    def clock_probe(self, us: float = 50.0) -> float:
        v = ctypes.c_double(0.0)
        check(self._L.clv_clock_probe(self.h, float(us), ctypes.byref(v)))
        return float(v.value)

    def launch_info(self) -> dict:
        out = (ctypes.c_int64 * 6)()
        check(self._L.clv_launch_info(self.h, out))
        return dict(persistent=bool(out[0]), persist_blocks_per_cu=int(out[1]), n_cu=int(out[2]),
                    workgroups=int(out[3]))

    IPC_HANDLE_BYTES = 64

    def p2p_info(self) -> dict:
        out = (ctypes.c_int64 * 6)()
        check(self._L.clv_p2p_info(self.h, out))
        return dict(capable=bool(out[0]), connected=bool(out[1]), mail_bytes=int(out[2]), mail_ptr=int(out[3]),
                    persistent=bool(out[4]), mail_memory={0: "uncached", 1: "fine-grained", 2: "device"}.get(int(out[5])))

    def p2p_export(self) -> bytes:
        buf = ctypes.create_string_buffer(self.IPC_HANDLE_BYTES)
        check(self._L.clv_p2p_export(self.h, buf))
        return buf.raw

    def p2p_connect(self, handles: Optional[Sequence[bytes]] = None, ptrs: Optional[Sequence[int]] = None) -> None:
        if handles is not None:
            blob = ctypes.create_string_buffer(b"".join(handles), self.IPC_HANDLE_BYTES * len(handles))
            check(self._L.clv_p2p_connect(self.h, blob, None))
        else:
            arr = (ctypes.c_uint64 * len(ptrs))(*[int(p) for p in ptrs])
            check(self._L.clv_p2p_connect(self.h, None, arr))

    def p2p_set_persistent(self, on: bool) -> None:
        check(self._L.clv_p2p_set_persistent(self.h, 1 if on else 0))

    def p2p_disconnect(self) -> None:
        check(self._L.clv_p2p_disconnect(self.h))

    def set_wait_timeout(self, ms: float) -> None:
        check(self._L.clv_set_wait_timeout(self.h, float(ms)))

    @property
    def sweeps_done(self) -> int:
        return int(self._L.clv_sweeps_done(self.h))

    def set_replay_tape(self, tape: np.ndarray, n_sweeps: int) -> None:
        tape = np.ascontiguousarray(tape, dtype=np.float64)
        stride = self.replay_sweep_stride
        if tape.size != self.chains * n_sweeps * stride:
            raise ValueError(f"tape has {tape.size} doubles, expected {self.chains * n_sweeps * stride}")
        check(self._L.clv_set_replay_tape(self.h, dptr(tape), int(n_sweeps)))

    @property
    def replay_sweep_stride(self) -> int:
        return int(self._L.clv_replay_sweep_stride(self.h))

    def level1_buffer(self) -> np.ndarray:
        return np.empty((self.chains, self.n_draws, self.n, self.D + 2))

    def stream_draws(self, level1: Optional[np.ndarray]) -> None:
        if level1 is not None:
            C, nd, n, D = self.chains, self.n_draws, self.n, self.D
            if (level1.shape != (C, nd, n, D + 2) or level1.dtype != np.float64 or not level1.flags.c_contiguous
                    or not level1.flags.writeable):
                raise ValueError("level1 must be a writeable C-contiguous float64 array of shape (chains, n_draws, n, D+2)")
        self._stream_buf = level1
        check(self._L.clv_stream_draws(self.h, dptr(level1)))

    def read_draws(self, level1: bool = True, out: Optional[np.ndarray] = None):
        C, nd, n, D, K = self.chains, self.n_draws, self.n, self.D, self.K
        l1 = None
        if level1 and self.draw_sink == "full":
            l1 = out if out is not None else self.level1_buffer()
        l2 = np.empty((C, nd, D * K + D * (D + 1) // 2))
        ll = np.empty((C, nd))
        check(self._L.clv_read_draws(self.h, dptr(l1), dptr(l2), dptr(ll)))
        return l1, l2, ll

    def flush(self) -> None:
        hyp = np.empty((self.chains, self.K * self.D + self.D * self.D))
        check(self._L.clv_get_state(self.h, None, None, dptr(hyp)))

    def read_summary(self):
        sums = np.empty((self.chains, _lib.N_SUM_STATS, self.n))
        k = ctypes.c_int64()
        check(self._L.clv_read_summary(self.h, dptr(sums), ctypes.byref(k)))
        return sums, int(k.value)

    def get_state(self):
        C, n, D, K = self.chains, self.n, self.D, self.K
        lam, mu = np.empty((C, n)), np.empty((C, n))
        hyp = np.empty((C, K * D + D * D))
        check(self._L.clv_get_state(self.h, dptr(lam), dptr(mu), dptr(hyp)))
        beta = hyp[:, : K * D].reshape(C, K, D)
        sigma = hyp[:, K * D:].reshape(C, D, D)
        return lam, mu, beta, sigma

    def set_state(self, lam, mu, beta, sigma, sweeps_done: int) -> None:
        C, n, D, K = self.chains, self.n, self.D, self.K
        lam = np.ascontiguousarray(np.broadcast_to(lam, (C, n)), dtype=np.float64)
        mu = np.ascontiguousarray(np.broadcast_to(mu, (C, n)), dtype=np.float64)
        hyp = np.concatenate([np.broadcast_to(beta, (C, K, D)).reshape(C, K * D),
                              np.broadcast_to(sigma, (C, D, D)).reshape(C, D * D)], axis=1)
        hyp = np.ascontiguousarray(hyp, dtype=np.float64)
        check(self._L.clv_set_state(self.h, dptr(lam), dptr(mu), dptr(hyp), int(sweeps_done)))

    def predict(self, T_star: float = 39.0, seed: Optional[int] = None, simulate_spend: bool = False,
                sigma_s: float = 0.5):
        nd = self.chains * self.n_draws
        x = np.empty((nd, self.n), np.int64)
        spend = np.empty((nd, self.n), np.float64) if simulate_spend else None
        check(self._L.clv_predict_sampler(self.h, float(T_star), resolve_seed(seed), 1 if simulate_spend else 0,
                                          float(sigma_s), x.ctypes.data_as(ctypes.POINTER(ctypes.c_int64)),
                                          dptr(spend)))
        return (x, spend) if simulate_spend else x

    def level1_summary(self, mu_cap: float = 0.05) -> np.ndarray:
        out = np.empty((self.n, len(_lib.L1_STATS)), np.float64)
        check(self._L.clv_level1_summary_sampler(self.h, float(mu_cap), dptr(out)))
        return out

    def diagnostics(self, log_columns=("lambda", "mu"), level1: bool = True, level2: bool = True,
                    param_names=None, rank: bool = False, hdi_prob: float = 0.94) -> dict:
        from . import analysis as A
        if rank:
            hdi_prob = A._check_hdi_prob(hdi_prob)
        w = self.D + 2
        mask = A.level1_log_mask(log_columns, w)
        o1 = np.empty((self.n * w, len(_lib.DIAG_STATS)), np.float64) if level1 else None
        o2 = np.empty((self.D * self.K + self.D * (self.D + 1) // 2, len(_lib.DIAG_STATS)), np.float64) if level2 else None
        check(self._L.clv_diagnostics_sampler(self.h, mask, dptr(o1), dptr(o2)))
        out = {}
        if level1:
            out["level_1"] = A.level1_diagnostics_frame(o1, self.n, w, mask)
        if level2:
            out["level_2"] = A.level2_diagnostics_frame(o2, param_names)
        if rank:
            r1 = np.empty((self.n * w, len(_lib.RANK_STATS)), np.float64) if level1 else None
            r2 = np.empty((len(o2), len(_lib.RANK_STATS)), np.float64) if level2 else None
            check(self._L.clv_rank_diagnostics_sampler(self.h, mask, hdi_prob, dptr(r1), dptr(r2)))
            if level1:
                out["level_1_rank"] = A.level1_rank_diagnostics_frame(r1, self.n, w, mask)
            if level2:
                out["level_2_rank"] = A.level2_rank_diagnostics_frame(r2, param_names)
                out["level_2_summary"] = A.level2_summary_frame(o2, r2, param_names, hdi_prob)
        return out

    def lifetime_value(self, *, discount_rate: float = 0.15, periods_per_year: float = 52.0, horizon=None,
                       monetary=None, omega2: float = 0.0) -> dict:
        from . import analysis as A
        par = A.ltv_params(discount_rate, periods_per_year, horizon, omega2)
        m = A.ltv_monetary(monetary, self.n, self.D + 2)
        cust = np.empty((self.n, len(_lib.LTV_STATS)), np.float64)
        per_draw = np.empty((self.chains * self.n_draws, len(_lib.LTV_DRAW_STATS)), np.float64)
        check(self._L.clv_lifetime_value_sampler(self.h, dptr(m), par["delta"], par["horizon"], par["value_scale"],
                                                 par["periods_per_year"], dptr(cust), dptr(per_draw)))
        return A.ltv_frames(cust, per_draw, par)

    def chain_total_loglik(self) -> float:
        out = ctypes.c_double()
        check(self._L.clv_chain_total_loglik_sampler(self.h, ctypes.byref(out)))
        return float(out.value)

# ... 284 lines not shown
```

Measured before the change: 9.722 billion.

## Add split persistent layout packing 1.5 blocks per 512-thread workgroup with helper waves

Adds a new persistent kernel layout for D=2 in which each 512-thread workgroup runs six customer waves (1.5 logical blocks) plus two helper waves. The helper waves generate the next sweep's MH variates ahead of time into LDS. Partial sums are written to extra records, and the level-2 reducer recombines the split blocks with a shuffle. The aim is to fit more chains' blocks on the CUs with fewer workgroups when the block layout oversubscribes, and to overlap RNG generation with compute. In exchange it brings a more complex reduction mapping, a fallback path if the launch aborts, and an env override.

```diff
diff --git a/include/clvmcmc.h b/include/clvmcmc.h
--- a/include/clvmcmc.h
+++ b/include/clvmcmc.h
@@ -139,6 +139,9 @@
 int clv_debug_persist_fits(int64_t grid_wgs, int32_t blocks_per_cu, int32_t n_cu);
 int clv_debug_persist_choice(int32_t D, int32_t K, int32_t n_chains, int64_t grid_wgs, int32_t blocks_per_cu,
                              int32_t n_cu);
+int clv_debug_split_fits(int32_t n_chains, int32_t nb, int32_t blocks_per_cu, int32_t n_cu);
+int clv_debug_split_choice(int32_t n_chains, int32_t nb, int32_t blocks_per_cu, int32_t n_cu);
+int clv_debug_split_layout(int32_t n_chains, int32_t nb, int32_t* out);
 
 enum { CLV_EXCHANGE_AUTO = 0, CLV_EXCHANGE_P2P = 1, CLV_EXCHANGE_COPY = 2 };
 typedef struct clv_group clv_group;
diff --git a/mcmc_clv_model_amd/csrc/capi.hip b/mcmc_clv_model_amd/csrc/capi.hip
--- a/mcmc_clv_model_amd/csrc/capi.hip
+++ b/mcmc_clv_model_amd/csrc/capi.hip
@@ -311,6 +311,23 @@
   return n_cu > 0 && grid_wgs > 0;
 }
 
+bool clv::persist_split_fits(int n_chains, int nb, int blocks_per_cu, int n_cu) {
+  if (n_chains < 1 || nb < 1 || nb > SPLIT_MAX_NB || blocks_per_cu < 1 || n_cu < 1) return false;
+  const int64_t grid = (int64_t)n_chains * (split_wgs(nb) + 1);
+  const int64_t margin = std::max(1, n_cu / 64);
+  return grid <= n_cu - margin;
+}
+
+bool clv::persist_split_pays(int n_chains, int nb, int n_cu) { return (int64_t)n_chains * (nb + 1) > n_cu; }
+
+std::vector<int32_t> clv::persist_split_layout(int n_chains, int nb) {
+  const int per = split_wgs(nb) + 1;
+  std::vector<int32_t> map((size_t)n_chains * per);
+  for (int c = 0; c < n_chains; ++c)
+    for (int p = 0; p < per; ++p) map[(size_t)c * per + p] = (c << 16) | p;
+  return map;
+}
+
 namespace {
 
 #ifndef CLV_L2_ALONE_MIN_NB
@@ -492,6 +509,20 @@
     if ((!env || std::string(env) != "0") && (force || scratch <= PERSIST_SCRATCH_MAX) && persist_grid_fits(grid, s->persist_bpc, s->n_cu) &&
         (force || persist_worth(g.D, g.K, (int)C, grid, s->n_cu)))
       s->persistent = true;
+    if (s->persistent && g.D == 2 && g.S <= PRE_STEPS && nb_local <= SPLIT_MAX_NB) {
+      const char* lay = std::getenv("CLV_PERSIST_LAYOUT");
+      const std::string want = lay ? lay : "";
+      if (lay && want != "block" && want != "split")
+        return cleanup_fail(fail(CLV_EINVAL, "CLV_PERSIST_LAYOUT must be block or split"));
+      int bpc = 0;
+      size_t sscratch = SIZE_MAX;
+      if (want != "block" && persist_split_resources(g.D, g.K, &bpc, &sscratch) == hipSuccess && sscratch == 0 &&
+          persist_split_fits((int)C, (int)nb_local, bpc, s->n_cu) &&
+          (want == "split" || persist_split_pays((int)C, (int)nb_local, s->n_cu)))
+        s->split = true;
+      else
+        (void)hipGetLastError();
+    }
   }
   if (!s->replay && cfg->world_size > 1 && cfg->world_size <= MAX_WORLD && nb_local > 0 && nb_local <= 2 * BLOCK && g.n_units_global <= 2 * BLOCK &&
       bpu <= 64 && (int64_t)g.stride * ((nb_local + bpu - 1) / bpu) <= UMAIL) {
@@ -532,7 +563,7 @@
     CLV_HIPC(dalloc(&s->d_peers, g.world_size));
   }
   if (s->persistent || s->p2p_capable || s->fx_capable) {
-    CLV_HIPC(dalloc(&s->d_pblock, (size_t)C * std::max(nb_local, 1) * g.stride));
+    CLV_HIPC(dalloc(&s->d_pblock, (size_t)C * split_records(std::max((int)nb_local, 1)) * g.stride));
     if (s->persistent) {
       const char* env = std::getenv("CLV_DEFER");
       s->defer = !(env && std::string(env) == "0");
@@ -560,6 +591,11 @@
       std::vector<int32_t> map = persist_wg_map((int)C, (int)nb_local, s->n_cu);
       CLV_HIPC(dalloc(&s->d_wgmap, map.size()));
       CLV_HIPC(hipMemcpy(s->d_wgmap, map.data(), sizeof(int32_t) * map.size(), hipMemcpyHostToDevice));
+    }
+    if (s->split) {
+      std::vector<int32_t> map = persist_split_layout((int)C, (int)nb_local);
+      CLV_HIPC(dalloc(&s->d_wgmap_split, map.size()));
+      CLV_HIPC(hipMemcpy(s->d_wgmap_split, map.data(), sizeof(int32_t) * map.size(), hipMemcpyHostToDevice));
     }
   }
 #ifdef CLV_STAMPS
@@ -679,6 +715,7 @@
   if (s->d_mail) (void)hipFree(s->d_mail);
   if (s->d_peers) (void)hipFree(s->d_peers);
   if (s->d_wgmap) (void)hipFree(s->d_wgmap);
+  if (s->d_wgmap_split) (void)hipFree(s->d_wgmap_split);
   if (s->own_stream && s->own) (void)hipStreamDestroy(s->own);
   delete s;
 }
@@ -794,8 +831,8 @@
   out[1] = s->persist_bpc;
   out[2] = s->n_cu;
   out[3] = (int64_t)(s->g.nb_local + (s->persistent ? 1 : 0)) * s->g.n_chains;
-  out[4] = 0;
-  out[5] = 0;
+  out[4] = s->split ? (int64_t)(split_wgs(s->g.nb_local) + 1) * s->g.n_chains : out[3];
+  out[5] = !s->persistent ? LAYOUT_NONE : s->split ? LAYOUT_SPLIT : s->split_reverted ? -LAYOUT_BLOCK : LAYOUT_BLOCK;
   return CLV_OK;
 }
 
@@ -920,7 +957,7 @@
   if (n_sweeps == 0) return CLV_OK;
   if (s->slots_dirty) {
     CLV_HIP(hipMemsetAsync(s->d_hyp2, 0xFF, sizeof(double) * 2 * g.n_chains * HS, s->stream));
-    CLV_HIP(hipMemsetAsync(s->d_pblock, 0xFF, sizeof(double) * g.n_chains * g.nb_local * g.stride, s->stream));
+    CLV_HIP(hipMemsetAsync(s->d_pblock, 0xFF, sizeof(double) * g.n_chains * split_records(g.nb_local) * g.stride, s->stream));
     s->slots_dirty = false;
   }
   const size_t sums_bytes = sizeof(double) * (size_t)g.n_chains * CLV_N_SUM_STATS * g.n;
@@ -941,7 +978,12 @@
   }
   if (e0) CLV_HIP(hipEventRecord(e0, s->stream));
   s->host_ns[2] = host_now_ns();
-  CLV_HIP(launch_persist(a, s->sweeps_done + 1, n_sweeps, s->stream, nullptr, nullptr));
+  if (s->split) {
+    a.wg_map = s->d_wgmap_split;
+    CLV_HIP(launch_persist_split(a, s->sweeps_done + 1, n_sweeps, s->stream));
+  } else {
+    CLV_HIP(launch_persist(a, s->sweeps_done + 1, n_sweeps, s->stream, nullptr, nullptr));
+  }
   s->host_ns[3] = host_now_ns();
   if (e1) CLV_HIP(hipEventRecord(e1, s->stream));
   s->inflight_done = e1;
@@ -984,7 +1026,12 @@
     if (s->d_sums_prev) CLV_HIP(hipMemcpy(s->d_sums, s->d_sums_prev, sums_bytes, hipMemcpyDeviceToDevice));
     s->slots_dirty = true;
     if (g.world_size > 1) s->p2p_ready = false;
-    const std::string diag = take_wait_diag(s);
+    std::string diag = take_wait_diag(s);
+    if (s->split) {
+      s->split = false;
+      s->split_reverted = true;
+      diag += "; the split layout's launch aborted: this handle uses the block layout from now on";
+    }
     return fail(CLV_EHIP, std::string(g.world_size > 1
                                           ? "persistent sweep kernel: a wait timed out (a peer rank not running, or not all "
                                             "resident?); state unchanged"
@@ -1515,6 +1562,39 @@
 
 int clv_debug_persist_fits(int64_t grid_wgs, int32_t blocks_per_cu, int32_t n_cu) {
   return persist_grid_fits(grid_wgs, blocks_per_cu, n_cu) ? 1 : 0;
+}
+
+int clv_debug_split_fits(int32_t n_chains, int32_t nb, int32_t blocks_per_cu, int32_t n_cu) {
+  return persist_split_fits(n_chains, nb, blocks_per_cu, n_cu) ? 1 : 0;
+}
+
+int clv_debug_split_choice(int32_t n_chains, int32_t nb, int32_t blocks_per_cu, int32_t n_cu) {
+  return persist_split_fits(n_chains, nb, blocks_per_cu, n_cu) && persist_split_pays(n_chains, nb, n_cu) ? 1 : 0;
+}
+
+int clv_debug_split_layout(int32_t n_chains, int32_t nb, int32_t* out) {
+  if (!out || n_chains < 1 || nb < 1 || nb > SPLIT_MAX_NB || n_chains >= (1 << 15)) return fail(CLV_EINVAL, "bad arguments");
+  const std::vector<int32_t> m = persist_split_layout(n_chains, nb);
+  const int nwg = split_wgs(nb);
+  for (size_t i = 0; i < m.size(); ++i) {
+    int32_t* o = out + 8 * i;
+    const int p = m[i] & 0xFFFF;
+    o[0] = m[i] >> 16;
+    for (int k = 1; k < 8; ++k) o[k] = -1;
+    if (p == nwg) continue;
+    const int r0 = SPLIT_CW * p;
+    o[1] = r0;
+    o[2] = std::min(SPLIT_CW, 4 * nb - r0);
+    const int b0 = (p & 1) ? (r0 - 2) / 4 : r0 / 4, b1 = (p & 1) ? (r0 + 2) / 4 : r0 / 4 + 1;
+    o[3] = (p & 1) ? 3 : 1;
+    o[4] = b0;
+    if (b1 < nb) {
+      o[5] = (p & 1) ? 1 : 2;
+      o[6] = b1;
+    }
+    o[7] = (p & 1) ? nb + 2 * (b0 / 3) : -1;
+  }
+  return CLV_OK;
 }
 
 int clv_debug_wg_map(int32_t n_chains, int32_t nb, int32_t n_cu, int32_t* out) {
diff --git a/mcmc_clv_model_amd/csrc/internal.h b/mcmc_clv_model_amd/csrc/internal.h
--- a/mcmc_clv_model_amd/csrc/internal.h
+++ b/mcmc_clv_model_amd/csrc/internal.h
@@ -18,6 +18,9 @@
 int persist_flush(clv_sampler* s);
 bool persist_grid_fits(int64_t grid_wgs, int blocks_per_cu, int n_cu);
 bool persist_worth(int D, int K, int n_chains, int64_t grid_wgs, int n_cu);
+bool persist_split_fits(int n_chains, int nb, int blocks_per_cu, int n_cu);
+bool persist_split_pays(int n_chains, int nb, int n_cu);
+std::vector<int32_t> persist_split_layout(int n_chains, int nb);
 
 struct DrawStreamState {
   std::mutex m;
@@ -111,6 +114,9 @@
   int rb_hyper_swaps = 0;
   bool persistent = false;
   int persist_bpc = 0, n_cu = 0;
+  bool split = false;
+  bool split_reverted = false;
+  int32_t* d_wgmap_split = nullptr;
   bool p2p_capable = false;
   bool p2p_persist_fits = false;
   bool fx_capable = false;
diff --git a/mcmc_clv_model_amd/csrc/kernels.h b/mcmc_clv_model_amd/csrc/kernels.h
--- a/mcmc_clv_model_amd/csrc/kernels.h
+++ b/mcmc_clv_model_amd/csrc/kernels.h
@@ -16,6 +16,13 @@
 constexpr int MAIL_TAIL = MAX_WORLD;
 constexpr int CLK_RING = 1024;
 constexpr int DIAG_WORDS = 16;
+constexpr int PRE_STEPS = 20;
+constexpr int SPLIT_CW = 6;
+constexpr int SPLIT_NT = 512;
+constexpr int SPLIT_MAX_NB = 256;
+enum : int { LAYOUT_NONE = 0, LAYOUT_BLOCK = 1, LAYOUT_SPLIT = 2 };
+__host__ __device__ inline int split_wgs(int nb) { return (2 * nb + 2) / 3; }
+__host__ __device__ inline int split_records(int nb) { return nb + 2 * ((nb + 1) / 3); }
 enum : int { WAIT_HYPER = 1, WAIT_BLOCKS = 2, WAIT_P2P_MAIL = 3, WAIT_FX_MAIL = 4 };
 
 __host__ __device__ inline int64_t mail_slots(int world, int chains, int stride, int units_per_rank) {
@@ -137,6 +144,8 @@
 hipError_t launch_group(const GroupArgs& a, hipStream_t st);
 hipError_t launch_persist(const SweepArgs& a, int64_t s_first, int64_t n_sweeps, hipStream_t st,
                           hipEvent_t e0 = nullptr, hipEvent_t e1 = nullptr);
+hipError_t launch_persist_split(const SweepArgs& a, int64_t s_first, int64_t n_sweeps, hipStream_t st);
+hipError_t persist_split_resources(int D, int K, int* blocks_per_cu, size_t* scratch_bytes);
 hipError_t persist_occupancy(int D, int K, bool p2p, int* blocks_per_cu);
 hipError_t persist_scratch_bytes(int D, int K, bool p2p, size_t* bytes);
 hipError_t launch_persist_flush(const SweepArgs& a, int64_t s_first, hipStream_t st);
diff --git a/mcmc_clv_model_amd/csrc/kernels.hip b/mcmc_clv_model_amd/csrc/kernels.hip
--- a/mcmc_clv_model_amd/csrc/kernels.hip
+++ b/mcmc_clv_model_amd/csrc/kernels.hip
@@ -159,11 +159,10 @@
   if constexpr (LDS_ONLY) lds_barrier(); else __syncthreads();
 }
 
-template <int NS, int G, int NT = BLOCK, class Gen>
-__device__ __forceinline__ void block_reduce_gen(const Gen& gen, double (*red)[NS], double* out) {
+template <int NS, int G, class Gen>
+__device__ __forceinline__ void wave_reduce_gen(const Gen& gen, double (*red)[NS]) {
   const int lane = threadIdx.x & 63;
   const int wave = threadIdx.x >> 6;
-  constexpr int NW = NT / 64;
 #pragma unroll
   for (int base = 0; base < NS; base += G) {
     constexpr int GG = G;
@@ -205,6 +204,12 @@
       }
     }
   }
+}
+
+template <int NS, int G, int NT = BLOCK, class Gen>
+__device__ __forceinline__ void block_reduce_gen(const Gen& gen, double (*red)[NS], double* out) {
+  constexpr int NW = NT / 64;
+  wave_reduce_gen<NS, G>(gen, red);
   __syncthreads();
   if (threadIdx.x < NS) {
     double t = red[0][threadIdx.x];
@@ -1250,7 +1255,6 @@
   for (int st = 0; st < MC; ++st) mh_step(cu, s00, s11, tl[st], tm[st], st < rem ? lu[st] : __builtin_inff(), exp_tab);
 }
 
-constexpr int PRE_STEPS = 20;
 constexpr int PRE_LDS_BYTES = PRE_STEPS * BLOCK * 12;
 struct PreVariates {
   float2* t;
@@ -1264,35 +1268,35 @@
   return x;
 }
 
-template <int NQ = PRE_STEPS / MH_CHUNK_STEPS>
-__device__ __forceinline__ void mh_pre_variates(const SlotPhilox& ph, int S_, const PreVariates& v) {
+template <int NQ = PRE_STEPS / MH_CHUNK_STEPS, int NT = BLOCK>
+__device__ __forceinline__ void mh_pre_variates(const SlotPhilox& ph, int S_, const PreVariates& v, int q0 = 0) {
   constexpr int MC = MH_CHUNK_STEPS;
   const int S = opaque_uniform(S_);
 #pragma unroll
   for (int q = 0; q < NQ; ++q) {
-    if (q * MC < S) {
+    if (q >= q0 && q * MC < S) {
       float tl[MC], tm[MC], lu[MC];
       mh_chunk_variates(ph, (uint32_t)q, tl, tm, lu);
       if (q * MC + MC <= S) {
 #pragma unroll
         for (int st = 0; st < MC; ++st) {
           const int k = q * MC + st;
-          v.t[k * BLOCK + v.lane] = make_float2(tl[st], tm[st]);
-          v.u[k * BLOCK + v.lane] = lu[st];
+          v.t[k * NT + v.lane] = make_float2(tl[st], tm[st]);
+          v.u[k * NT + v.lane] = lu[st];
         }
       } else {
 #pragma unroll
         for (int st = 0; st < MC; ++st) {
           const int k = q * MC + st;
-          v.t[k * BLOCK + v.lane] = make_float2(tl[st], tm[st]);
-          v.u[k * BLOCK + v.lane] = k < S ? lu[st] : __builtin_inff();
+          v.t[k * NT + v.lane] = make_float2(tl[st], tm[st]);
+          v.u[k * NT + v.lane] = k < S ? lu[st] : __builtin_inff();
         }
       }
     }
   }
 }
 
-template <int NQ = PRE_STEPS / MH_CHUNK_STEPS, int D, int K, bool CL>
+template <int NQ = PRE_STEPS / MH_CHUNK_STEPS, int NT = BLOCK, int D, int K, bool CL>
 __device__ __forceinline__ void mh_run_pre(Cust<D, K, CL>& cu, const PreVariates& v, double s00, double s11, int S,
                                            const double* exp_tab) {
   constexpr int MC = MH_CHUNK_STEPS;
@@ -1304,8 +1308,8 @@
       float u[MC];
 #pragma unroll
       for (int st = 0; st < MC; ++st) {
-        t[st] = v.t[(q * MC + st) * BLOCK + v.lane];
-        u[st] = v.u[(q * MC + st) * BLOCK + v.lane];
+        t[st] = v.t[(q * MC + st) * NT + v.lane];
+        u[st] = v.u[(q * MC + st) * NT + v.lane];
       }
 #pragma unroll
       for (int st = 0; st < MC; ++st) mh_step(cu, s00, s11, t[st].x, t[st].y, u[st], exp_tab);
@@ -1789,7 +1793,7 @@
   return hipGetLastError();
 }
 
-template <int D, int K, bool P2P>
+template <int D, int K, bool P2P, bool SPLIT = false>
 __device__ __forceinline__ void persist_level2(const SweepArgs& a, int64_t s_first, int64_t n_sweeps, int c, uint32_t k0,
                                             uint32_t k1, int64_t wgi, int64_t it_stamp, double* pool) {
   constexpr int NT = BLOCK;
@@ -1808,7 +1812,8 @@
   const Geometry& g = a.g;
   const int tid0 = threadIdx.x;
   (void)wgi;
-  double* parts0 = a.pblock + (int64_t)c * g.nb_local * NS;
+  static_assert(!(SPLIT && P2P), "the split layout is world size 1 only");
+  double* parts0 = a.pblock + (int64_t)c * (SPLIT ? split_records(g.nb_local) : g.nb_local) * NS;
   if (tid0 == 0) s_abort = 0;
   if constexpr (P2P) {
     if (tid0 < g.world_size) s_peers[tid0] = a.peers[tid0];
@@ -1844,10 +1849,25 @@
     CLV_P_STAMP(a.stamps, wgi, 1, stp);
     if (!from_pend) {
     double v0[NS], v1[NS];
-    const int b0 = tid, b1 = tid + NT;
-    const bool hb0 = b0 < g.nb_local, hb1 = b1 < g.nb_local;
+    int eb = -1, er = 0, src = tid & 63;
+    if constexpr (SPLIT) {
+      const int bm = tid - 1, bp = tid + 1;
+      if (tid % 3 == 1 && tid < g.nb_local) {
+        eb = tid;
+        src = (tid & 63) != 63 ? src + 1 : src - 1;
+      } else if (bm >= 0 && bm % 3 == 1 && (bm & 63) != 63 && bm < g.nb_local) {
+        eb = bm;
+        er = 1;
+      } else if (bp % 3 == 1 && (bp & 63) == 63 && bp < g.nb_local) {
+        eb = bp;
+        er = 1;
+      }
+    }
+    const bool own_split = SPLIT && eb == tid;
+    const int b0 = tid, b1 = SPLIT ? eb : tid + NT;
+    const bool hb0 = b0 < g.nb_local, hb1 = SPLIT ? eb >= 0 : b1 < g.nb_local;
     double* pb0 = parts + (int64_t)b0 * NS;
-    double* pb1 = parts + (int64_t)b1 * NS;
+    double* pb1 = parts + (int64_t)(SPLIT ? g.nb_local + 2 * (eb / 3) + er : b1) * NS;
     const double* qb0 = hb0 ? pb0 : parts;
     const double* qb1 = hb1 ? pb1 : parts;
     const int64_t per_rank = (int64_t)g.n_chains * NS * g.units_per_rank;
@@ -1926,7 +1946,14 @@
     }
     CLV_P_STAMP(a.stamps, wgi, 2, stp);
     double acc[NS];
-    if constexpr (!P2P) {
+    if constexpr (SPLIT) {
+#pragma unroll
+      for (int j = 0; j < NS; ++j) {
+        const double r3 = __shfl(v1[j], src, 64);
+        acc[j] = 0.0;
+        if (hb0) acc[j] += own_split ? (v0[j] + v1[j]) + r3 : v0[j];
+      }
+    } else if constexpr (!P2P) {
 #pragma unroll
       for (int j = 0; j < NS; ++j) {
         acc[j] = 0.0;
@@ -2018,7 +2045,7 @@
     CLV_P_STAMP(a.stamps, wgi, 6, stp);
     const int rt = tid - 64;
     if (rt >= 0) {
-      const int nrec = g.nb_local * NS;
+      const int nrec = (SPLIT ? split_records(g.nb_local) : g.nb_local) * NS;
       for (int e = rt; e < nrec; e += NT - 64) st_wt(parts + e, slot_empty());
       if ((it > 0 || pin) && rt < HS) st_wt(a.hyp2 + ((int64_t)(s & 1) * g.n_chains + c) * HS + rt, slot_empty());
     }
@@ -2233,6 +2260,222 @@
         if constexpr (D == 3) {
           if (pre) zeta_lds[tid] = eta_normal(k0, k1, cu.gi, s + 1, exp_tab);
         }
+      }
+    }
+    CLV_P_STAMP(a.stamps, wgi, 6, stp);
+  }
+  if (cu.active) {
+    const int64_t ci = (int64_t)c * g.n + cu.i;
+    a.lam_out[ci] = cu.lam;
+    a.mu_out[ci] = cu.mu;
+  }
+}
+
+#ifndef CLV_SPLIT_HELP_CHUNKS
+#define CLV_SPLIT_HELP_CHUNKS 2
+#endif
+constexpr int SPLIT_NC = SPLIT_CW * 64;
+constexpr int SPLIT_PRE_LDS_BYTES = PRE_STEPS * SPLIT_NC * 12;
+
+template <int D, int K, int HC>
+__global__ __launch_bounds__(SPLIT_NT, 1) void persist_kernel_split(SweepArgs a, int64_t s_first, int64_t n_sweeps) {
+  static_assert(D == 2, "the split layout is bivariate");
+  constexpr int NXY = K * D;
+  constexpr int NYY = D * (D + 1) / 2;
+  constexpr int NS = NXY + NYY + 1;
+  constexpr int MC = MH_CHUNK_STEPS;
+  constexpr int NQ = PRE_STEPS / MC;
+  static_assert(HC >= 0 && HC <= NQ, "helper share");
+  __shared__ double red[SPLIT_CW][NS];
+  __shared__ __attribute__((aligned(16))) double exp_tab[FAST_TAB_N];
+  __shared__ double Hs[HS];
+  __shared__ uint32_t s_abort;
+  __shared__ __attribute__((aligned(16))) char pool[SPLIT_PRE_LDS_BYTES];
+  const Geometry& g = a.g;
+  const int nwg = split_wgs(g.nb_local);
+  int c = blockIdx.y, p = blockIdx.x;
+  if (a.wg_map) {
+    const int32_t m = a.wg_map[blockIdx.y * gridDim.x + blockIdx.x];
+    c = m >> 16;
+    p = m & 0xFFFF;
+  }
+  const int tid = threadIdx.x;
+  const int wave = __builtin_amdgcn_readfirstlane(tid >> 6);
+  const int64_t wgi = (int64_t)c * (nwg + 1) + p;
+  const int64_t it_stamp = n_sweeps >= 2 ? n_sweeps - 2 : 0;
+  (void)wgi;
+  (void)it_stamp;
+  uint32_t k0, k1;
+  chain_key(a.r.seed, (int64_t)a.r.chain_first + c, &k0, &k1);
+  double* parts = a.pblock + (int64_t)c * split_records(g.nb_local) * NS;
+  if (tid == 0) s_abort = 0;
+
+  if (p == nwg) {
+    if (tid >= BLOCK) return;
+    persist_level2<D, K, false, true>(a, s_first, n_sweeps, c, k0, k1, wgi, it_stamp, (double*)pool);
+    return;
+  }
+
+  const PreVariates pv{(float2*)pool, (float*)(pool + PRE_STEPS * SPLIT_NC * 8), tid};
+  fast_tab_fill(exp_tab, tid, SPLIT_NT, false);
+  if (tid < HS) Hs[tid] = a.hyper[(int64_t)c * HS + tid];
+  const bool first_wait = a.pend_in != nullptr;
+
+  if (wave >= SPLIT_CW) {
+    const int h = wave - SPLIT_CW;
+    uint32_t gi[2];
+    bool on[2];
+    int col[2];
+#pragma unroll
+    for (int t = 0; t < 2; ++t) {
+      col[t] = (h + 4 * t) * 64 + (tid & 63);
+      const int64_t i = (int64_t)p * SPLIT_NC + col[t];
+      on[t] = i < g.n;
+      gi[t] = (uint32_t)(g.shard_begin + i);
+    }
+    __syncthreads();
+    for (int64_t it = 0; it < n_sweeps; ++it) {
+      if (it > 0 || first_wait) {
+        __syncthreads();
+        if (s_abort) return;
+      }
+      const bool ahead = HC > 0 && it + 1 < n_sweeps;
+      const int S = opaque_uniform(loop_args<CLV_PERSIST_FRESH_ARGS != 0>(a).g.S);
+      float tl[2][HC > 0 ? HC : 1][MC], tm[2][HC > 0 ? HC : 1][MC], lu[2][HC > 0 ? HC : 1][MC];
+      if (ahead) {
+#pragma unroll
+        for (int t = 0; t < 2; ++t) {
+          if (on[t]) {
+            const SlotPhilox ph(k0, k1, gi[t], (uint32_t)(s_first + it + 1));
+#pragma unroll
+            for (int q = 0; q < HC; ++q)
+              if (q * MC < S) mh_chunk_variates(ph, (uint32_t)q, tl[t][q], tm[t][q], lu[t][q]);
+          }
+        }
+      }
+      __syncthreads();
+      if (ahead) {
+#pragma unroll
+        for (int t = 0; t < 2; ++t) {
+          if (on[t]) {
+#pragma unroll
+            for (int q = 0; q < HC; ++q) {
+              if (q * MC < S) {
+#pragma unroll
+                for (int st = 0; st < MC; ++st) {
+                  const int k = q * MC + st;
+                  pv.t[k * SPLIT_NC + col[t]] = make_float2(tl[t][q][st], tm[t][q][st]);
+                  pv.u[k * SPLIT_NC + col[t]] = k < S ? lu[t][q][st] : __builtin_inff();
+                }
+              }
+            }
+          }
+        }
+      }
+    }
+    return;
+  }
+
+  CLV_P_STAMP(a.stamps, wgi, 7, tid == 0);
+  Cust<D, K> cu;
+  {
+    const int64_t i = (int64_t)p * SPLIT_NC + tid;
+    cu.active = i < g.n;
+    cu.i = cu.active ? i : (g.n > 0 ? g.n - 1 : 0);
+  }
+  cust_load(cu, a, c);
+  __syncthreads();
+  if (cu.active) {
+    cust_ztau<D, K, false>(cu, a, s_first, k0, k1, nullptr, exp_tab);
+    mh_pre_variates<NQ, SPLIT_NC>(SlotPhilox(k0, k1, cu.gi, (uint32_t)s_first), g.S, pv);
+  }
+  CLV_P_STAMP(a.stamps, wgi, 10, tid == 0);
+  const SweepArgs& a_launch = a;
+  for (int64_t it = 0; it < n_sweeps; ++it) {
+    const SweepArgs& a = loop_args<CLV_PERSIST_FRESH_ARGS != 0>(a_launch);
+    const Geometry& g = a.g;
+    const double* hyp_c = a.hyp2 + (int64_t)c * HS;
+    const int64_t s = uniform64(s_first + it);
+    const bool stored = is_stored(s, g);
+    const bool stp = tid == 0 && it == it_stamp;
+    (void)stp;
+    CLV_P_STAMP(a.stamps, wgi, 0, stp);
+    if (it > 0 || first_wait) {
+      if (tid < 64) {
+        const double* src = hyp_c + (int64_t)(s & 1) * g.n_chains * HS;
+        const uint64_t t0 = __builtin_amdgcn_s_memrealtime();
+        for (uint32_t poll = 0;; ++poll) {
+          const double v = ld_wt(src + tid);
+          if (__all(slot_full(v))) {
+            Hs[tid] = v;
+            break;
+          }
+          const int ws = wait_state(a, t0, poll, hyper_wait_ticks(a));
+          if (ws != WAIT_GOING) {
+            if (ws == WAIT_EXPIRED) {
+              report_wait(a, WAIT_HYPER, s, c, slot_full(v), p, tid, dbits(v), poll, t0);
+              raise_abort(a);
+            }
+            if (tid == 0) s_abort = 1;
+            break;
+          }
+          __builtin_amdgcn_s_sleep(1);
+        }
+      }
+      __syncthreads();
+      if (s_abort) return;
+    }
+    CLV_P_STAMP(a.stamps, wgi, 1, stp);
+    StatGen<D, K> st{};
+    CustOut<D> out{};
+    __builtin_amdgcn_s_setprio(2);
+    if (cu.active) {
+      cust_coeffs<D, K, false>(cu, Hs, exp_tab);
+      CLV_P_STAMP(a.stamps, wgi, 2, stp);
+      mh_run_pre<NQ, SPLIT_NC>(cu, pv, Hs[H_S00], Hs[H_S11], g.S, exp_tab);
+      CLV_P_STAMP(a.stamps, wgi, 3, stp);
+      out = cust_finish<D, K, false>(cu, a, s, stored, Hs, k0, k1, nullptr, exp_tab, st, nullptr);
+    }
+    CLV_P_STAMP(a.stamps, wgi, 4, stp);
+    wave_reduce_gen<NS, SWEEP_REDUCE_CHUNK>(st, red);
+    __syncthreads();
+    {
+      const int j = tid & 63;
+      const int r0 = SPLIT_CW * p;
+      if (j < NS && tid < 128) {
+        if ((p & 1) == 0) {
+          if (tid < 64) {
+            st_wt(parts + (int64_t)(r0 / 4) * NS + j, ((red[0][j] + red[1][j]) + red[2][j]) + red[3][j]);
+          } else {
+            const int b = r0 / 4 + 1;
+            if (b < g.nb_local) st_wt(parts + (int64_t)b * NS + j, red[4][j] + red[5][j]);
+          }
+        } else {
+          if (tid < 64) {
+            const int b = (r0 - 2) / 4;
+            double* ext = parts + (int64_t)(g.nb_local + 2 * (b / 3)) * NS;
+            st_wt(ext + j, red[0][j]);
+            st_wt(ext + NS + j, red[1][j]);
+          } else {
+            const int b = (r0 + 2) / 4;
+            if (b < g.nb_local) st_wt(parts + (int64_t)b * NS + j, ((red[2][j] + red[3][j]) + red[4][j]) + red[5][j]);
+          }
+        }
+      }
+    }
+    __builtin_amdgcn_s_setprio(0);
+    CLV_P_STAMP(a.stamps, wgi, 5, stp);
+    CLV_P_STAMP(a.stamps, wgi, 8, stp);
+    CLV_P_STAMP(a.stamps, wgi, 9, stp);
+#ifdef CLV_STAMPS
+    if (stp && a.stamps) a.stamps[1024 * 8 + wgi * 12 + 11] = blockIdx.y * gridDim.x + blockIdx.x;
+#endif
+    if (cu.active) {
+      cust_store<D, K>(cu, out, a, c, s, stored, false);
+      if (it + 1 < n_sweeps) {
+        cust_ztau<D, K, false>(cu, a, s + 1, k0, k1, nullptr, exp_tab);
+        const int q_own = (__builtin_amdgcn_readfirstlane(tid >> 6) & 3) < 2 ? HC : 0;
+        mh_pre_variates<NQ, SPLIT_NC>(SlotPhilox(k0, k1, cu.gi, (uint32_t)(s + 1)), g.S, pv, q_own);
       }
     }
     CLV_P_STAMP(a.stamps, wgi, 6, stp);
@@ -2496,6 +2739,33 @@
   return hipErrorInvalidValue;
 }
 
+hipError_t launch_persist_split(const SweepArgs& a, int64_t s_first, int64_t n_sweeps, hipStream_t st) {
+  const dim3 grid(split_wgs(a.g.nb_local) + 1, a.g.n_chains);
+#define CLV_CASE(DD, KK, PP)                                                                                        \
+  if (a.g.D == DD && a.g.K == KK) {                                                                               \
+    hipLaunchKernelGGL((persist_kernel_split<DD, KK, CLV_SPLIT_HELP_CHUNKS>), grid, dim3(SPLIT_NT), 0, st, a, s_first, n_sweeps); \
+    return hipGetLastError();                                                                                     \
+  }
+  CLV_FOR_K(CLV_CASE, 2, false)
+#undef CLV_CASE
+  return hipErrorInvalidValue;
+}
+
+hipError_t persist_split_resources(int D, int K, int* blocks_per_cu, size_t* scratch_bytes) {
+  hipFuncAttributes fa{};
+#define CLV_CASE(DD, KK, PP)                                                                                      \
+  if (D == DD && K == KK) {                                                                                       \
+    hipError_t e = hipOccupancyMaxActiveBlocksPerMultiprocessor(blocks_per_cu, persist_kernel_split<DD, KK, CLV_SPLIT_HELP_CHUNKS>, SPLIT_NT, 0); \
+    if (e != hipSuccess) return e;                                                                                \
+    e = hipFuncGetAttributes(&fa, reinterpret_cast<const void*>(&persist_kernel_split<DD, KK, CLV_SPLIT_HELP_CHUNKS>)); \
+    *scratch_bytes = fa.localSizeBytes;                                                                           \
+    return e;                                                                                                     \
+  }
+  CLV_FOR_K(CLV_CASE, 2, false)
+#undef CLV_CASE
+  return hipErrorInvalidValue;
+}
+
 hipError_t persist_occupancy(int D, int K, bool p2p, int* blocks_per_cu) {
 #define CLV_CASE(DD, KK, PP) \
   if (D == DD && K == KK && p2p == PP) return hipOccupancyMaxActiveBlocksPerMultiprocessor(blocks_per_cu, persist_kernel<DD, KK, PP>, BLOCK, 0);
diff --git a/mcmc_clv_model_amd/sampler.py b/mcmc_clv_model_amd/sampler.py
--- a/mcmc_clv_model_amd/sampler.py
+++ b/mcmc_clv_model_amd/sampler.py
@@ -235,7 +235,8 @@
         out = (ctypes.c_int64 * 6)()
         check(self._L.clv_launch_info(self.h, out))
         return dict(persistent=bool(out[0]), persist_blocks_per_cu=int(out[1]), n_cu=int(out[2]),
-                    workgroups=int(out[3]))
+                    workgroups=int(out[3]), physical_workgroups=int(out[4]),
+                    layout={1: "block", 2: "split", -1: "block (split aborted)"}.get(int(out[5])))
 
     IPC_HANDLE_BYTES = 64
 
```

Result: faster. 10.83 billion, median of 6 (+11.4%).
